# DearCaat/RRT-MIL

Measured on AMD Instinct MI355X. Metric: slides/sec RRTEncoder fwd, N=9000 D=512 region_num=8, higher is better.
Workload: dtype f32

## Files before the change

include/rrt_hip.h:

```cpp
#ifndef RRT_HIP_H
#define RRT_HIP_H
#include <stddef.h>
#include <stdint.h>

#ifdef __cplusplus
extern "C" {
#endif

#define RRT_ABI_VERSION 28
#define RRT_MAX_RMSA_LAYERS 8
#define RRT_MAX_CRMSA_K 8

enum {
  RRT_OK = 0,
  RRT_E_INVALID = -1,
  RRT_E_UNSUPPORTED = -2,
  RRT_E_WORKSPACE = -3,
  RRT_E_HANDOVER = -4
};

enum { RRT_COMPUTE_F32 = 0, RRT_COMPUTE_BF16 = 1, RRT_COMPUTE_F16 = 2, RRT_COMPUTE_F32X3 = 3 };
enum { RRT_POS_NONE = 0, RRT_POS_PEG = 1, RRT_POS_PPEG = 2 };
enum { RRT_EPEG_ATTN = 0, RRT_EPEG_VALUE_BF = 1, RRT_EPEG_VALUE_AF = 2 };

enum { RRT_ACT_NONE = 0, RRT_ACT_RELU = 1, RRT_ACT_GELU = 2, RRT_ACT_TANH = 3, RRT_ACT_SIGMOID = 4 };

typedef struct rrt_grid {
  int64_t L;
  int32_t H;
  int32_t s;
  int32_t regions_side;
  int64_t add;
} rrt_grid;

typedef struct rrt_encoder_desc {
  int32_t dim;
  int32_t n_heads;
  int32_t n_rmsa_layers;
  int32_t region_num;
  int32_t region_size;
  int32_t min_region_num;
  float   min_region_ratio;
  int32_t epeg;
  int32_t epeg_k;
  int32_t cr_msa;
  int32_t crmsa_k;
  int32_t crmsa_heads;
  int32_t crmsa_mlp;
  int32_t all_shortcut;
  int32_t compute;
  int32_t ffn;
  int32_t ffn_act;
  int32_t ffn_hidden;
  int32_t pos;
  int32_t pos_pos;
  int32_t peg_k;
  int32_t peg_1d;
  int32_t epeg_2d;
  int32_t epeg_type;
  int32_t weights16_valid;
  int32_t solo;
} rrt_encoder_desc;

typedef struct rrt_attn_weights {
  const float *norm_w, *norm_b;
  const float *qkv_w, *qkv_b;
  const float *proj_w, *proj_b;
  const float *pe_w, *pe_b;
  const float *norm2_w, *norm2_b;
  const float *fc1_w, *fc1_b;
  const float *fc2_w, *fc2_b;
} rrt_attn_weights;

typedef struct rrt_encoder_weights {
  rrt_attn_weights rmsa[RRT_MAX_RMSA_LAYERS];
  rrt_attn_weights crmsa;
  const float *phi;
  const float *phi0_w, *phi2_w;
  const float *norm_w, *norm_b;
  const float *pos_w[3], *pos_b[3];
  uint64_t version;
} rrt_encoder_weights;

int         rrt_abi_version(void);
const char *rrt_strerror(int code);

int rrt_region_grid(int64_t L, int32_t region_num, int32_t region_size,
                    int32_t min_region_num, float min_region_ratio, rrt_grid *out);

int rrt_encoder_workspace_size(const rrt_encoder_desc *desc, int64_t n_tokens, size_t *bytes);

#define RRT_PLAN_FUSED      1
#define RRT_PLAN_FUSED_PROJ 2
#define RRT_PLAN_FUSED16    4
#define RRT_PLAN_FUSED_X3   8
#define RRT_PLAN_CRMSA_PARTS 16
#define RRT_PLAN_ATTN_HD    32
int rrt_encoder_plan(const rrt_encoder_desc *desc, int64_t n_tokens, int32_t *flags);

int rrt_encoder_forward_f32(const rrt_encoder_desc *desc, const rrt_encoder_weights *w,
                            const float *x, float *y, int64_t n_tokens,
                            void *workspace, size_t workspace_bytes, void *stream);

enum {
  RRT_EV_START = 0,
  RRT_EV_LN_PARTITION,
  RRT_EV_QKV,
  RRT_EV_ATTN,
  RRT_EV_PROJ,
  RRT_EV_CR_COMBINE,
  RRT_EV_CR_INNER,
  RRT_EV_END,
  RRT_EV_COUNT
};
int rrt_encoder_forward_events_f32(const rrt_encoder_desc *desc, const rrt_encoder_weights *w,
                                   const float *x, float *y, int64_t n_tokens,
                                   void *workspace, size_t workspace_bytes, void *stream,
                                   void **events);

typedef struct rrt_phase_gate rrt_phase_gate;
int rrt_phase_gate_create(rrt_phase_gate **out);
int rrt_phase_gate_destroy(rrt_phase_gate *gate);
int rrt_encoder_forward_gated_f32(const rrt_encoder_desc *desc, const rrt_encoder_weights *w,
                                  const float *x, float *y, int64_t n_tokens,
                                  void *workspace, size_t workspace_bytes, void *stream,
                                  rrt_phase_gate *gate, void **events);

int rrt_encoder_batch_workspace_size(const rrt_encoder_desc *desc, int32_t batch, int64_t n_tokens, size_t *bytes);
int rrt_encoder_forward_batch_f32(const rrt_encoder_desc *desc, const rrt_encoder_weights *w,
                                  const float *x, float *y, int32_t batch, int64_t n_tokens,
                                  void *workspace, size_t workspace_bytes, void *stream);


int rrt_ln_partition_f32(const float *x, const float *gamma, const float *beta, float *u,
                         int64_t L, int32_t dim, const rrt_grid *g, void *stream);

int rrt_linear_f32(const float *A, const float *B, const float *bias, float *C,
                   int64_t M, int32_t N, int32_t K, int32_t q_cols, float q_scale,
                   int32_t compute , void *stream);

int rrt_linear_unpartition_residual_f32(const float *A, const float *B, const float *bias,
                                        const float *resid, float *out, int32_t N, int32_t K,
                                        const rrt_grid *g, int32_t compute, void *stream);

int rrt_region_attention_f32(const float *qkv, const float *pe_w, float *o,
                             int32_t n_regions, int32_t P, int32_t dim, int32_t heads,
                             int32_t epeg_k, void *stream);

int rrt_region_attention_hd_supported(int32_t P, int32_t dim, int32_t heads, int32_t epeg_k);
int rrt_region_attention_hd_f32(const float *qkv, const float *pe_w, float *o,
                                int32_t n_regions, int32_t P, int32_t dim, int32_t heads,
                                int32_t epeg_k, void *stream);

int rrt_rmsa_fused_f32(const float *u, const float *qkv_w, const float *qkv_b, const float *pe_w,
                       float *o, int32_t n_regions, int32_t P, int32_t dim, int32_t heads,
                       int32_t epeg_k, int32_t compute, void *stream);

int rrt_rmsa_fused_proj_f32(const float *u, const float *qkv_w, const float *qkv_b, const float *pe_w,
                            const float *proj_w, const float *proj_b, const float *resid, float *out,
                            float *o_scratch, int32_t *counters, int32_t dim, int32_t heads, int32_t epeg_k,
                            const rrt_grid *g, void *stream);
int rrt_rmsa_fused_proj_stats_f32(const float *u, const float *qkv_w, const float *qkv_b, const float *pe_w,
                                  const float *proj_w, const float *proj_b, const float *resid, float *out,
                                  float *o_scratch, int32_t *counters, const float *ln2_gamma, const float *phi,
                                  int32_t crmsa_k, float *part, int32_t dim, int32_t heads, int32_t epeg_k,
                                  const rrt_grid *g, void *stream);
int rrt_crmsa_combine_parts_f32(const float *x1, const float *part, const float *gamma, const float *beta,
                                const float *phi, float *wdisp, float *rep, int64_t n_tokens, int32_t dim, int32_t k,
                                const rrt_grid *g8, void *stream);
int rrt_device_error(int32_t clear);
int rrt_debug_rmsa_fused_proj_f32(const float *u, const float *qkv_w, const float *qkv_b, const float *pe_w,
                                  const float *proj_w, const float *proj_b, const float *resid, float *out,
                                  float *o_scratch, int32_t *counters, int32_t dim, int32_t heads, int32_t epeg_k,
                                  const rrt_grid *g, int32_t lag, int32_t spin_limit, int32_t wait_extra, void *stream);

int rrt_cast16(const float *src, uint16_t *dst, int64_t n, int32_t compute, void *stream);
int rrt_ln_partition16(const float *x, const float *gamma, const float *beta, uint16_t *u, int64_t L,
                       int32_t dim, const rrt_grid *g, int32_t compute, void *stream);
int rrt_linear16_f32(const uint16_t *A, const uint16_t *B, const float *bias, const float *resid, float *C,
                     int64_t M, int32_t N, int32_t K, const rrt_grid *g, int32_t compute, void *stream);
int rrt_rmsa_fused16(const uint16_t *u, const uint16_t *qkv_w, const float *qkv_b, const float *pe_w,
                     uint16_t *o, int32_t n_regions, int32_t P, int32_t dim, int32_t heads, int32_t epeg_k,
                     int32_t compute, void *stream);
int rrt_rmsa_pair16_proj(const uint16_t *u, const uint16_t *qkv_w, const float *qkv_b, const float *pe_w,
                         const uint16_t *proj_w, const float *proj_b, const float *resid, float *out, uint16_t *o,
                         int32_t *cnt, int32_t dim, int32_t heads, int32_t epeg_k, const rrt_grid *g, int32_t compute,
                         void *stream);

int rrt_cast_split(const float *src, void *dst, int64_t n, void *stream);
int rrt_ln_partition_split(const float *x, const float *gamma, const float *beta, void *u, int64_t L,
                           int32_t dim, const rrt_grid *g, void *stream);
int rrt_linear_split_f32(const void *A, const void *B, const float *bias, const float *resid, float *C,
                         int64_t M, int32_t N, int32_t K, const rrt_grid *g, void *stream);
int rrt_rmsa_fused_x3(const void *u, const void *qkv_w, const float *qkv_b, const float *pe_w, void *o,
                      int32_t n_regions, int32_t P, int32_t dim, int32_t heads, int32_t epeg_k, void *stream);

int rrt_crmsa_logits_f32(const float *x1, const float *gamma, const float *beta, const float *phi,
                         float *mean_rstd, float *logits, int64_t L, int32_t dim, int32_t k,
                         const rrt_grid *g8, void *stream);
int rrt_crmsa_combine_f32(const float *x1, const float *gamma, const float *beta,
                          const float *mean_rstd, const float *logits, float *wdisp, float *rep,
                          int64_t L, int32_t dim, int32_t k, const rrt_grid *g8, void *stream);
int rrt_crmsa_region_f32(const float *x1, const float *gamma, const float *beta, const float *phi,
                         float *mean_rstd, float *logits, float *wdisp, float *rep,
                         int64_t L, int32_t dim, int32_t k, const rrt_grid *g8, void *stream);
int rrt_crmsa_region4_f32(const float *x1, const float *gamma, const float *beta, const float *phi,
                          float *mean_rstd, float *logits, float *wdisp, float *rep,
                          int64_t L, int32_t dim, int32_t k, const rrt_grid *g8,
                          void *scratch, size_t scratch_bytes, void *stream);
int rrt_crmsa_stream4_f32(const float *x1, const float *gamma, const float *beta, const float *phi,
                          float *mean_rstd, float *logits, float *wdisp, float *rep,
                          int64_t L, int32_t dim, int32_t k, const rrt_grid *g8,
                          void *scratch, size_t scratch_bytes, void *stream);
int rrt_crmsa_dispatch_ln_f32(const float *x1, const float *x0, const float *wdisp,
                              const float *rep2, const float *gamma,
                              const float *beta, float *y, int64_t L, int32_t dim, int32_t k,
                              const rrt_grid *g8, void *stream);
int rrt_crmsa_mlp_logits_f32(const float *hid, const float *w2, float *logits, int64_t rows,
                             int32_t hdim, int32_t k, void *stream);
int rrt_layernorm_f32(const float *x1, const float *x0, const float *gamma, const float *beta,
                      float *y, int64_t L, int32_t dim, void *stream);

typedef struct rrt_mil_desc {
  rrt_encoder_desc enc;
  int32_t input_dim;
  int32_t emb_act;
  int32_t n_classes;
  int32_t pool_hidden;
  int32_t pool_act;
  int32_t pool_gated;
  int32_t input16;
} rrt_mil_desc;

typedef struct rrt_mil_weights {
  rrt_encoder_weights enc;
  const float *emb_w, *emb_b;
  const float *pool_a_w, *pool_a_b;
  const float *pool_b_w, *pool_b_b;
  const float *pool_c_w, *pool_c_b;
  const float *pred_w, *pred_b;
} rrt_mil_weights;

int rrt_attn_pool_workspace_size(int64_t n_tokens, int32_t dim, int32_t hidden, size_t *bytes);
int rrt_attn_pool_f32(const float *y, const float *hid_a, const float *hid_b, const float *c_w, const float *c_b,
                      float *pooled, float *attn, float *a_raw, int64_t n_tokens, int32_t dim, int32_t hidden,
                      void *workspace, size_t workspace_bytes, void *stream);
int rrt_attn_pool_backward_f32(const float *y, const float *hid_a, const float *hid_b, const float *c_w,
                               const float *attn, const float *pooled, const float *d_pooled,
                               const float *d_attn, const float *d_raw, const float *c_ext, float *dy,
                               float *dhid_a, float *dhid_b, float *dwcb, int64_t n_tokens, int32_t dim,
                               int32_t hidden, void *workspace, size_t workspace_bytes, void *stream);

int rrt_mil_workspace_size(const rrt_mil_desc *desc, int64_t n_tokens, size_t *bytes);

int rrt_mil_forward_f32(const rrt_mil_desc *desc, const rrt_mil_weights *w, const float *x,
                        float *logits, float *attn, int32_t no_norm, float *feat, int64_t n_tokens,
                        void *workspace, size_t workspace_bytes, void *stream);

int rrt_pool_workspace_size(int64_t n_tokens, int32_t dim, int32_t hidden, int32_t gated, size_t *bytes);
int rrt_pool_predict_f32(const float *y, const float *a_w, const float *a_b, const float *b_w,
                         const float *b_b, const float *c_w, const float *c_b, const float *pred_w,
                         const float *pred_b, float *pooled, float *logits, float *attn, int32_t no_norm,
                         int64_t n_tokens, int32_t dim, int32_t hidden, int32_t act, int32_t n_classes,
                         int32_t compute, void *workspace, size_t workspace_bytes, void *stream);

int rrt_linear_act_f32(const float *A, const float *B, const float *bias, float *C, int64_t M, int32_t N,
                       int32_t K, int32_t act, int32_t compute, void *stream);

typedef struct rrt_executor rrt_executor;
typedef struct rrt_bag {
  const float *x;
  float *y;
  int64_t n_tokens;
} rrt_bag;
int rrt_executor_create(const rrt_encoder_desc *desc, int32_t n_streams, int64_t max_tokens,
                        rrt_executor **out);
int rrt_executor_create_on_streams(const rrt_encoder_desc *desc, int32_t n_streams, void *const *streams,
                                   int64_t max_tokens, rrt_executor **out);
int rrt_executor_forward(rrt_executor *ex, const rrt_encoder_weights *w, const rrt_bag *bags,
                         int32_t n_bags, void *stream);
int rrt_executor_destroy(rrt_executor *ex);

int rrt_region_attention_backward_workspace_size(int32_t n_regions, int32_t P, int32_t dim, int32_t heads,
                                                 int32_t epeg_k, size_t *bytes);
int rrt_region_attention_backward_f32(const float *qkv, const float *pe_w, const float *o, const float *d_o,
                                      float *d_qkv, float *d_pe_w, int32_t n_regions, int32_t P, int32_t dim,
                                      int32_t heads, int32_t epeg_k, void *workspace, size_t workspace_bytes,
                                      void *stream);
int rrt_layernorm_backward_f32(const float *dy, const float *x, const float *gamma, const float *add,
                               float *dx, float *dgamma_dbeta, int64_t L, int32_t dim, const rrt_grid *g,
                               void *workspace, size_t workspace_bytes, void *stream);
int rrt_reduce_partials_f32(const float *part, float *out, float *out_tr, int32_t S, int64_t n, int64_t split,
                            int32_t tr_dim, int32_t tr_k, int32_t deferred, int32_t copies, void *stream);
int rrt_linear_backward_workspace_size(int64_t M, int32_t N, int32_t K, size_t *bytes);
int rrt_linear_backward_f32(const float *dY, const float *X, const float *W, float *dX, float *dW,
                            float *db, int64_t M, int32_t N, int32_t K, int32_t compute,
                            void *workspace, size_t workspace_bytes, void *stream);

typedef struct rrt_attn_grads {
  float *norm;
  float *qkv_w, *qkv_b;
  float *proj_w, *proj_b;
  float *pe_w;
  float *pe_b;
  float *norm2;
  float *fc1_w, *fc1_b;
  float *fc2_w, *fc2_b;
} rrt_attn_grads;
typedef struct rrt_encoder_grads {
  rrt_attn_grads rmsa[RRT_MAX_RMSA_LAYERS];
  rrt_attn_grads crmsa;
  float *phi;
  float *phi0_w, *phi2_w;
  float *norm;
  float *pos_w[3], *pos_b[3];
} rrt_encoder_grads;

int rrt_encoder_train_sizes(const rrt_encoder_desc *desc, int64_t n_tokens, size_t *stash_bytes,
                            size_t *backward_workspace_bytes);
int rrt_encoder_forward_train_f32(const rrt_encoder_desc *desc, const rrt_encoder_weights *w, const float *x,
                                  float *y, int64_t n_tokens, void *stash, size_t stash_bytes,
                                  float drop_p, uint64_t drop_seed, const float *branch_scale, void *stream);
// ... 11 lines not shown
```

rrt-mil_amd/_lib.py:

```python
import ctypes as C
import os

HERE = os.path.dirname(os.path.abspath(__file__))
LIB_PATH = os.path.join(HERE, "librrt_hip.so")

RRT_MAX_RMSA_LAYERS = 8
RRT_MAX_CRMSA_K = 8
ABI_VERSION = 28

_f32p = C.POINTER(C.c_float)


class Grid(C.Structure):
    _fields_ = [("L", C.c_int64), ("H", C.c_int32), ("s", C.c_int32),
                ("regions_side", C.c_int32), ("add", C.c_int64)]


class EncoderDesc(C.Structure):
    _fields_ = [("dim", C.c_int32), ("n_heads", C.c_int32), ("n_rmsa_layers", C.c_int32),
                ("region_num", C.c_int32), ("region_size", C.c_int32), ("min_region_num", C.c_int32),
                ("min_region_ratio", C.c_float), ("epeg", C.c_int32), ("epeg_k", C.c_int32),
                ("cr_msa", C.c_int32), ("crmsa_k", C.c_int32), ("crmsa_heads", C.c_int32),
                ("crmsa_mlp", C.c_int32), ("all_shortcut", C.c_int32), ("compute", C.c_int32),
                ("ffn", C.c_int32), ("ffn_act", C.c_int32), ("ffn_hidden", C.c_int32),
                ("pos", C.c_int32), ("pos_pos", C.c_int32), ("peg_k", C.c_int32), ("peg_1d", C.c_int32),
                ("epeg_2d", C.c_int32), ("epeg_type", C.c_int32), ("weights16_valid", C.c_int32),
                ("solo", C.c_int32)]


class AttnWeights(C.Structure):
    _fields_ = [(n, C.c_void_p) for n in ("norm_w", "norm_b", "qkv_w", "qkv_b", "proj_w", "proj_b",
                                          "pe_w", "pe_b", "norm2_w", "norm2_b", "fc1_w", "fc1_b",
                                          "fc2_w", "fc2_b")]


class EncoderWeights(C.Structure):
    _fields_ = [("rmsa", AttnWeights * RRT_MAX_RMSA_LAYERS), ("crmsa", AttnWeights),
                ("phi", C.c_void_p), ("phi0_w", C.c_void_p), ("phi2_w", C.c_void_p),
                ("norm_w", C.c_void_p), ("norm_b", C.c_void_p),
                ("pos_w", C.c_void_p * 3), ("pos_b", C.c_void_p * 3), ("version", C.c_uint64)]


class AttnGrads(C.Structure):
    _fields_ = [(n, C.c_void_p) for n in ("norm", "qkv_w", "qkv_b", "proj_w", "proj_b", "pe_w", "pe_b", "norm2",
                                          "fc1_w", "fc1_b", "fc2_w", "fc2_b")]


class EncoderGrads(C.Structure):
    _fields_ = [("rmsa", AttnGrads * RRT_MAX_RMSA_LAYERS), ("crmsa", AttnGrads), ("phi", C.c_void_p),
                ("phi0_w", C.c_void_p), ("phi2_w", C.c_void_p), ("norm", C.c_void_p),
                ("pos_w", C.c_void_p * 3), ("pos_b", C.c_void_p * 3)]


class MilDesc(C.Structure):
    _fields_ = [("enc", EncoderDesc), ("input_dim", C.c_int32), ("emb_act", C.c_int32),
                ("n_classes", C.c_int32), ("pool_hidden", C.c_int32), ("pool_act", C.c_int32),
                ("pool_gated", C.c_int32), ("input16", C.c_int32)]


class MilWeights(C.Structure):
    _fields_ = [("enc", EncoderWeights)] + [(n, C.c_void_p) for n in (
        "emb_w", "emb_b", "pool_a_w", "pool_a_b", "pool_b_w", "pool_b_b", "pool_c_w", "pool_c_b",
        "pred_w", "pred_b")]


class Bag(C.Structure):
    _fields_ = [("x", C.c_void_p), ("y", C.c_void_p), ("n_tokens", C.c_int64)]


ACT_NONE, ACT_RELU, ACT_GELU, ACT_TANH, ACT_SIGMOID = 0, 1, 2, 3, 4
ACT_BY_NAME = {"relu": ACT_RELU, "gelu": ACT_GELU, "tanh": ACT_TANH}

SIGNATURES = {
    "rrt_abi_version": (C.c_int, []),
    "rrt_strerror": (C.c_char_p, [C.c_int]),
    "rrt_region_grid": (C.c_int, [C.c_int64, C.c_int32, C.c_int32, C.c_int32, C.c_float, C.POINTER(Grid)]),
    "rrt_encoder_workspace_size": (C.c_int, [C.POINTER(EncoderDesc), C.c_int64, C.POINTER(C.c_size_t)]),
    "rrt_encoder_plan": (C.c_int, [C.POINTER(EncoderDesc), C.c_int64, C.POINTER(C.c_int32)]),
    "rrt_encoder_forward_f32": (C.c_int, [C.POINTER(EncoderDesc), C.POINTER(EncoderWeights), C.c_void_p,
                                          C.c_void_p, C.c_int64, C.c_void_p, C.c_size_t, C.c_void_p]),
    "rrt_encoder_forward_events_f32": (C.c_int, [C.POINTER(EncoderDesc), C.POINTER(EncoderWeights), C.c_void_p,
                                                 C.c_void_p, C.c_int64, C.c_void_p, C.c_size_t, C.c_void_p,
                                                 C.POINTER(C.c_void_p)]),
    "rrt_encoder_batch_workspace_size": (C.c_int, [C.POINTER(EncoderDesc), C.c_int32, C.c_int64, C.POINTER(C.c_size_t)]),
    "rrt_encoder_forward_batch_f32": (C.c_int, [C.POINTER(EncoderDesc), C.POINTER(EncoderWeights), C.c_void_p, C.c_void_p,
                                                C.c_int32, C.c_int64, C.c_void_p, C.c_size_t, C.c_void_p]),
    "rrt_phase_gate_create": (C.c_int, [C.POINTER(C.c_void_p)]),
    "rrt_phase_gate_destroy": (C.c_int, [C.c_void_p]),
    "rrt_encoder_forward_gated_f32": (C.c_int, [C.POINTER(EncoderDesc), C.POINTER(EncoderWeights), C.c_void_p,
                                                C.c_void_p, C.c_int64, C.c_void_p, C.c_size_t, C.c_void_p,
                                                C.c_void_p, C.POINTER(C.c_void_p)]),
    "rrt_ln_partition_f32": (C.c_int, [C.c_void_p, C.c_void_p, C.c_void_p, C.c_void_p, C.c_int64,
                                       C.c_int32, C.POINTER(Grid), C.c_void_p]),
    "rrt_linear_f32": (C.c_int, [C.c_void_p, C.c_void_p, C.c_void_p, C.c_void_p, C.c_int64, C.c_int32,
                                 C.c_int32, C.c_int32, C.c_float, C.c_int32, C.c_void_p]),
    "rrt_linear_unpartition_residual_f32": (C.c_int, [C.c_void_p, C.c_void_p, C.c_void_p, C.c_void_p,
                                                      C.c_void_p, C.c_int32, C.c_int32, C.POINTER(Grid),
                                                      C.c_int32, C.c_void_p]),
    "rrt_region_attention_f32": (C.c_int, [C.c_void_p, C.c_void_p, C.c_void_p, C.c_int32, C.c_int32,
                                           C.c_int32, C.c_int32, C.c_int32, C.c_void_p]),
    "rrt_region_attention_hd_supported": (C.c_int, [C.c_int32] * 4),
    "rrt_region_attention_hd_f32": (C.c_int, [C.c_void_p, C.c_void_p, C.c_void_p, C.c_int32, C.c_int32,
                                              C.c_int32, C.c_int32, C.c_int32, C.c_void_p]),
    "rrt_rmsa_fused_f32": (C.c_int, [C.c_void_p] * 5 + [C.c_int32] * 6 + [C.c_void_p]),
    "rrt_rmsa_fused_proj_f32": (C.c_int, [C.c_void_p] * 10 + [C.c_int32] * 3 + [C.c_void_p] * 2),
    "rrt_device_error": (C.c_int, [C.c_int32]),
    "rrt_rmsa_fused_proj_stats_f32": (C.c_int, [C.c_void_p] * 12 + [C.c_int32, C.c_void_p] + [C.c_int32] * 3 + [C.c_void_p] * 2),
    "rrt_crmsa_combine_parts_f32": (C.c_int, [C.c_void_p] * 7 + [C.c_int64, C.c_int32, C.c_int32, C.POINTER(Grid), C.c_void_p]),
    "rrt_debug_rmsa_fused_proj_f32": (C.c_int, [C.c_void_p] * 10 + [C.c_int32] * 3 + [C.c_void_p] + [C.c_int32] * 3 + [C.c_void_p]),
    "rrt_cast16": (C.c_int, [C.c_void_p, C.c_void_p, C.c_int64, C.c_int32, C.c_void_p]),
    "rrt_ln_partition16": (C.c_int, [C.c_void_p, C.c_void_p, C.c_void_p, C.c_void_p, C.c_int64, C.c_int32,
                                     C.POINTER(Grid), C.c_int32, C.c_void_p]),
    "rrt_linear16_f32": (C.c_int, [C.c_void_p] * 5 + [C.c_int64, C.c_int32, C.c_int32, C.POINTER(Grid), C.c_int32,
                                                      C.c_void_p]),
    "rrt_rmsa_fused16": (C.c_int, [C.c_void_p] * 5 + [C.c_int32] * 6 + [C.c_void_p]),
    "rrt_rmsa_pair16_proj": (C.c_int, [C.c_void_p] * 10 + [C.c_int32] * 3 + [C.POINTER(Grid), C.c_int32, C.c_void_p]),
    "rrt_cast_split": (C.c_int, [C.c_void_p, C.c_void_p, C.c_int64, C.c_void_p]),
    "rrt_ln_partition_split": (C.c_int, [C.c_void_p, C.c_void_p, C.c_void_p, C.c_void_p, C.c_int64, C.c_int32,
                                         C.POINTER(Grid), C.c_void_p]),
    "rrt_linear_split_f32": (C.c_int, [C.c_void_p] * 5 + [C.c_int64, C.c_int32, C.c_int32, C.POINTER(Grid), C.c_void_p]),
    "rrt_rmsa_fused_x3": (C.c_int, [C.c_void_p] * 5 + [C.c_int32] * 5 + [C.c_void_p]),
    "rrt_crmsa_logits_f32": (C.c_int, [C.c_void_p] * 6 + [C.c_int64, C.c_int32, C.c_int32,
                                                         C.POINTER(Grid), C.c_void_p]),
    "rrt_crmsa_combine_f32": (C.c_int, [C.c_void_p] * 7 + [C.c_int64, C.c_int32, C.c_int32,
                                                          C.POINTER(Grid), C.c_void_p]),
    "rrt_crmsa_region_f32": (C.c_int, [C.c_void_p] * 8 + [C.c_int64, C.c_int32, C.c_int32, C.POINTER(Grid), C.c_void_p]),
    "rrt_crmsa_region4_f32": (C.c_int, [C.c_void_p] * 8 + [C.c_int64, C.c_int32, C.c_int32, C.POINTER(Grid), C.c_void_p,
                                                         C.c_size_t, C.c_void_p]),
    "rrt_crmsa_stream4_f32": (C.c_int, [C.c_void_p] * 8 + [C.c_int64, C.c_int32, C.c_int32, C.POINTER(Grid), C.c_void_p,
                                                         C.c_size_t, C.c_void_p]),
    "rrt_crmsa_dispatch_ln_f32": (C.c_int, [C.c_void_p] * 7 + [C.c_int64, C.c_int32, C.c_int32,
                                                              C.POINTER(Grid), C.c_void_p]),
    "rrt_crmsa_mlp_logits_f32": (C.c_int, [C.c_void_p] * 3 + [C.c_int64, C.c_int32, C.c_int32, C.c_void_p]),
    "rrt_layernorm_f32": (C.c_int, [C.c_void_p] * 5 + [C.c_int64, C.c_int32, C.c_void_p]),
    "rrt_mil_workspace_size": (C.c_int, [C.POINTER(MilDesc), C.c_int64, C.POINTER(C.c_size_t)]),
    "rrt_mil_forward_f32": (C.c_int, [C.POINTER(MilDesc), C.POINTER(MilWeights), C.c_void_p, C.c_void_p,
                                      C.c_void_p, C.c_int32, C.c_void_p, C.c_int64, C.c_void_p, C.c_size_t,
                                      C.c_void_p]),
    "rrt_pool_workspace_size": (C.c_int, [C.c_int64, C.c_int32, C.c_int32, C.c_int32, C.POINTER(C.c_size_t)]),
    "rrt_pool_predict_f32": (C.c_int, [C.c_void_p] * 12 + [C.c_int32, C.c_int64] + [C.c_int32] * 5 +
                             [C.c_void_p, C.c_size_t, C.c_void_p]),
    "rrt_attn_pool_workspace_size": (C.c_int, [C.c_int64, C.c_int32, C.c_int32, C.POINTER(C.c_size_t)]),
    "rrt_attn_pool_f32": (C.c_int, [C.c_void_p] * 8 + [C.c_int64, C.c_int32, C.c_int32, C.c_void_p, C.c_size_t, C.c_void_p]),
    "rrt_attn_pool_backward_f32": (C.c_int, [C.c_void_p] * 14 + [C.c_int64, C.c_int32, C.c_int32, C.c_void_p, C.c_size_t,
                                                                 C.c_void_p]),
    "rrt_executor_create": (C.c_int, [C.POINTER(EncoderDesc), C.c_int32, C.c_int64, C.POINTER(C.c_void_p)]),
    "rrt_executor_create_on_streams": (C.c_int, [C.POINTER(EncoderDesc), C.c_int32, C.POINTER(C.c_void_p), C.c_int64,
                                                 C.POINTER(C.c_void_p)]),
    "rrt_executor_forward": (C.c_int, [C.c_void_p, C.POINTER(EncoderWeights), C.POINTER(Bag), C.c_int32,
                                       C.c_void_p]),
    "rrt_executor_destroy": (C.c_int, [C.c_void_p]),
    "rrt_region_attention_backward_workspace_size": (C.c_int, [C.c_int32] * 5 + [C.POINTER(C.c_size_t)]),
    "rrt_region_attention_backward_f32": (C.c_int, [C.c_void_p] * 6 + [C.c_int32] * 5 + [C.c_void_p, C.c_size_t,
                                                                                       C.c_void_p]),
    "rrt_layernorm_backward_f32": (C.c_int, [C.c_void_p] * 6 + [C.c_int64, C.c_int32, C.POINTER(Grid), C.c_void_p,
                                                                C.c_size_t, C.c_void_p]),
    "rrt_reduce_partials_f32": (C.c_int, [C.c_void_p] * 3 + [C.c_int32, C.c_int64, C.c_int64] + [C.c_int32] * 4 + [C.c_void_p]),
    "rrt_linear_backward_workspace_size": (C.c_int, [C.c_int64, C.c_int32, C.c_int32, C.POINTER(C.c_size_t)]),
    "rrt_linear_backward_f32": (C.c_int, [C.c_void_p] * 6 + [C.c_int64, C.c_int32, C.c_int32, C.c_int32,
                                                             C.c_void_p, C.c_size_t, C.c_void_p]),
    "rrt_encoder_train_sizes": (C.c_int, [C.POINTER(EncoderDesc), C.c_int64, C.POINTER(C.c_size_t),
                                          C.POINTER(C.c_size_t)]),
    "rrt_encoder_forward_train_f32": (C.c_int, [C.POINTER(EncoderDesc), C.POINTER(EncoderWeights), C.c_void_p,
                                                C.c_void_p, C.c_int64, C.c_void_p, C.c_size_t, C.c_float,
                                                C.c_uint64, C.POINTER(C.c_float), C.c_void_p]),
    "rrt_encoder_backward_f32": (C.c_int, [C.POINTER(EncoderDesc), C.POINTER(EncoderWeights), C.c_void_p, C.c_void_p,
                                           C.c_void_p, C.c_size_t, C.POINTER(EncoderGrads), C.c_void_p, C.c_int64,
                                           C.c_void_p, C.c_size_t, C.c_float, C.c_uint64, C.POINTER(C.c_float),
                                           C.c_void_p]),
    "rrt_linear_act_f32": (C.c_int, [C.c_void_p] * 4 + [C.c_int64, C.c_int32, C.c_int32, C.c_int32, C.c_int32,
                                                        C.c_void_p]),
}

COMPUTE_F32, COMPUTE_BF16, COMPUTE_F16, COMPUTE_F32X3 = 0, 1, 2, 3
POS_NONE, POS_PEG, POS_PPEG = 0, 1, 2
EPEG_ATTN, EPEG_VALUE_BF, EPEG_VALUE_AF = 0, 1, 2

PLAN_FUSED, PLAN_FUSED_PROJ, PLAN_FUSED16, PLAN_FUSED_X3, PLAN_CRMSA_PARTS, PLAN_ATTN_HD = 1, 2, 4, 8, 16, 32
EV_START, EV_LN_PARTITION, EV_QKV, EV_ATTN, EV_PROJ, EV_CR_COMBINE, EV_CR_INNER, EV_END, EV_COUNT = range(9)

_lib = None


class RRTHipError(RuntimeError):
    pass


def load(path=None):
    global _lib
    if _lib is not None and path is None:
        return _lib
    p = path or os.environ.get("RRT_HIP_LIB") or LIB_PATH
    if not os.path.exists(p):
        raise RRTHipError(
            f"{p} is missing: the HIP extension is the only compute path. Build it with "
            "`python rrt-mil_amd/build.py` (needs /opt/rocm/bin/hipcc).")
    lib = C.CDLL(p)
    for name, (res, args) in SIGNATURES.items():
        fn = getattr(lib, name)
        fn.restype = res
        fn.argtypes = args
    if lib.rrt_abi_version() != ABI_VERSION:
        raise RRTHipError(f"librrt_hip.so ABI {lib.rrt_abi_version()} != binding {ABI_VERSION}; rebuild")
    if path is None:
        _lib = lib
    return lib


E_HANDOVER = -4


def device_error(clear=False):
    return int(load().rrt_device_error(1 if clear else 0))


def check(rc, what=""):
    if rc != 0:
        msg = load().rrt_strerror(rc).decode()
        if rc == -2:
            raise NotImplementedError(f"rrt_hip {what}: {msg}")
        if rc == E_HANDOVER:
            msg += (" -- sticky until cleared: torch.cuda.synchronize(), discard the outputs of the forwards in flight, "
                    "rrt_mil_amd.device_error(clear=True), run them again")
        raise RRTHipError(f"rrt_hip {what} failed ({rc}): {msg}")


def region_grid(L, region_num=8, region_size=0, min_region_num=0, min_region_ratio=0.0):
    g = Grid()
    check(load().rrt_region_grid(L, region_num, region_size, min_region_num, min_region_ratio, C.byref(g)),
          "rrt_region_grid")
    return g
```

rrt-mil_amd/csrc/api.hip:

```cpp
#include <math.h>
#include <stdio.h>
#include <string.h>

#include "internal.h"

namespace {

thread_local char g_detail[256] = "";

int unsupported(const char* why) {
  snprintf(g_detail, sizeof(g_detail), "%s", why);
  return RRT_E_UNSUPPORTED;
}

int64_t ceil_sqrt(int64_t n) {
  int64_t r = (int64_t)floor(sqrt((double)n));
  while (r * r > n) --r;
  while ((r + 1) * (r + 1) <= n) ++r;
  return r * r == n ? r : r + 1;
}

inline size_t align_up(size_t v, size_t a) { return (v + a - 1) / a * a; }

struct Workspace {
  float *uo, *qkv, *xa, *xb, *mean_rstd, *logits, *wdisp, *rep, *rep_qkv, *rep_o, *rep2, *v8, *hid;
  float *ffn_ln, *ffn_hid, *xp;
  float* pe_out;
  float* smap;
  uint16_t* w16;
  uint16_t* wcr16;
  uint16_t *rep16, *repo16;
  float* cr_part;
  int* cr_cnt;
  int* proj_cnt;
  float* cr_pstat;
  size_t bytes;
};

Workspace carve(const rrt_encoder_desc& d, int64_t N, const rrt_grid& g, const rrt_grid& g8, char* base) {
  Workspace w{};
  size_t off = 0;
  auto take = [&](size_t nfloat) {
    float* p = base ? (float*)(base + off) : nullptr;
    off = align_up(off + nfloat * sizeof(float), 256);
    return p;
  };
  const size_t D = d.dim;
  const size_t Np = (size_t)g.H * g.H, Np8 = (size_t)g8.H * g8.H;
  const size_t R8 = (size_t)g8.regions_side * g8.regions_side;
  if (d.n_rmsa_layers > 0) w.w16 = (uint16_t*)take((size_t)d.n_rmsa_layers * 4 * D * D);
  if (d.cr_msa) w.wcr16 = (uint16_t*)take(2 * D * D);
  if (d.n_rmsa_layers > 0) {
    w.uo = take(Np * D);
    w.qkv = take(Np * 3 * D);
    w.xa = take((size_t)N * D);
    if (d.n_rmsa_layers > 1 || d.ffn) w.xb = take((size_t)N * D);
    w.proj_cnt = (int*)take((size_t)g.regions_side * g.regions_side);
    if (d.epeg && d.epeg_type != RRT_EPEG_ATTN) w.pe_out = take(Np * D);
    if (d.epeg && d.epeg_2d && d.epeg_type == RRT_EPEG_ATTN) {
      const size_t sm = attn_scoremap_scratch_floats(g.regions_side * g.regions_side, g.s * g.s, d.n_heads, d.epeg_k, 1);
      if (sm) w.smap = take(sm);
    }
  }
  if (d.ffn) {
    if (!w.xa) w.xa = take((size_t)N * D);
    if (!w.xb) w.xb = take((size_t)N * D);
    w.ffn_ln = take((size_t)N * D);
    w.ffn_hid = take((size_t)N * d.ffn_hidden);
  }
  if (d.cr_msa) {
    const size_t k = d.crmsa_k;
    w.mean_rstd = take((size_t)N * 2);
    w.logits = take(Np8 * k);
    w.wdisp = take(Np8 * k);
    w.rep = take(k * R8 * D);
    w.rep_qkv = take(k * R8 * 3 * D);
    w.rep_o = take(k * R8 * D);
    w.rep2 = take(k * R8 * D);
    w.rep16 = (uint16_t*)take(k * R8 * D / 2);
    w.repo16 = (uint16_t*)take(k * R8 * D / 2);
    if (d.n_rmsa_layers > 0) {
      w.cr_part = take(crmsa_region4_scratch_floats(to_dev(g8), d.crmsa_k));
      w.cr_cnt = (int*)take(64);
      if (D % 64 == 0) w.cr_pstat = take(crmsa_parts_floats(N, (int)D, d.crmsa_k));
    }
    if (d.crmsa_mlp) {
      w.v8 = take(Np8 * D);
      w.hid = take(Np8 * (D / 4));
    }
  }
  if (d.pos) w.xp = take((size_t)N * D);
  w.bytes = off ? off : 256;
  return w;
}

int check_desc(const rrt_encoder_desc* d, int64_t N) {
  if (!d || N <= 0) return RRT_E_INVALID;
  if (d->dim <= 0 || d->dim % 32 != 0) return unsupported("dim must be a positive multiple of 32");
  if (d->dim > 2048) return unsupported("dim > 2048");
  if (d->n_rmsa_layers < 0 || d->n_rmsa_layers > RRT_MAX_RMSA_LAYERS) return unsupported("n_layers-1 out of range");
  if (d->n_rmsa_layers > 0) {
    if (d->n_heads <= 0 || d->dim % d->n_heads != 0) return unsupported("n_heads must divide dim");
    if (d->epeg && (d->epeg_k <= 0 || d->epeg_k % 2 == 0)) return unsupported("epeg_k must be odd");
    if (d->epeg_type < RRT_EPEG_ATTN || d->epeg_type > RRT_EPEG_VALUE_AF) return unsupported("epeg_type must be attn / value_bf / value_af");
    if (d->epeg && (d->epeg_2d || d->epeg_type != RRT_EPEG_ATTN) && d->epeg_k > 63) return unsupported("epeg ablations: epeg_k <= 63");
    if (d->region_size <= 0 && d->region_num <= 0) return unsupported("region_num must be positive");
  }
  if (d->cr_msa) {
    if (d->crmsa_k <= 0 || d->crmsa_k > RRT_MAX_CRMSA_K) return unsupported("crmsa_k must be in [1,8]");
    if (d->crmsa_heads <= 0 || d->dim % d->crmsa_heads != 0) return unsupported("crmsa_heads must divide dim");
  }
  if (d->ffn) {
    if (d->ffn_hidden <= 0 || d->ffn_hidden % 32 != 0)
      return unsupported("ffn: hidden width int(dim * mlp_ratio) must be a positive multiple of 32");
    if (d->ffn_act != RRT_ACT_GELU && d->ffn_act != RRT_ACT_RELU) return unsupported("ffn_act must be gelu or relu");
  }
  if (d->pos) {
    if (d->pos != RRT_POS_PEG && d->pos != RRT_POS_PPEG) return unsupported("pos must be none / peg / ppeg");
    if (d->peg_k <= 0 || d->peg_k % 2 == 0 || d->peg_k > 11) return unsupported("peg_k must be odd and <= 11");
    if (d->pos_pos != -1 && d->pos_pos != 0) return unsupported("pos_pos must be -1 or 0");
  }
  if (N > (int64_t)4000000) return unsupported("bag larger than 4e6 tokens");
  if (d->compute < 0 || d->compute > RRT_COMPUTE_F32X3) return unsupported("compute must be RRT_COMPUTE_F32/BF16/F16/F32X3");
  return RRT_OK;
}

hipError_t inner_attention(const float* u, int n_regions, int P, const rrt_attn_weights& w, int dim,
                           int heads, int epeg_k, float* qkv, float* o, int prec, bool solo, hipStream_t st) {
  const int M = n_regions * P;
  LinearEpilogue ep{};
  ep.prec = prec;
  ep.solo = solo;
  ep.bias = w.qkv_b;
  ep.q_cols = dim;
  ep.q_scale = 1.0f / sqrtf((float)(dim / heads));
  hipError_t e = launch_linear(u, w.qkv_w, qkv, M, 3 * dim, dim, ep, st);
  if (e != hipSuccess) return e;
  return launch_region_attention(qkv, epeg_k > 0 ? w.pe_w : nullptr, o, n_regions, P, dim, heads,
                                 epeg_k, st);
}

}

GridDev to_dev(const rrt_grid& g) {
  GridDev d;
  d.L = (int)g.L;
  d.H = g.H;
  d.s = g.s;
  d.rs = g.regions_side;
  d.P = g.s * g.s;
  d.Np = g.H * g.H;
  d.inv_H = 1.0f / (float)d.H;
  d.inv_s = 1.0f / (float)d.s;
  d.inv_rs = 1.0f / (float)d.rs;
  d.inv_P = 1.0f / (float)d.P;
  d.Rt = d.rs * d.rs;
  return d;
}

extern "C" {

int rrt_abi_version(void) { return RRT_ABI_VERSION; }

const char* rrt_strerror(int code) {
  switch (code) {
    case RRT_OK: return "ok";
    case RRT_E_INVALID: return "invalid argument (null pointer or non-positive size)";
    case RRT_E_UNSUPPORTED: return g_detail[0] ? g_detail : "unsupported configuration";
    case RRT_E_WORKSPACE: return "workspace too small (see rrt_encoder_workspace_size)";
    case RRT_E_HANDOVER: return "an earlier merged R-MSA launch gave up its in-launch hand-over wait; outputs in flight are invalid "
                                "(synchronise, then rrt_device_error(1) to clear)";
    default: return code > 0 ? hipGetErrorString((hipError_t)code) : "unknown error";
  }
}

int rrt_region_grid(int64_t L, int32_t region_num, int32_t region_size, int32_t min_region_num,
                    float min_region_ratio, rrt_grid* out) {
  if (!out || L <= 0) return RRT_E_INVALID;
  if (region_size <= 0 && region_num <= 0) return RRT_E_INVALID;
  int64_t H = ceil_sqrt(L), s;
  if (region_size > 0) {
    H += ((-H) % region_size + region_size) % region_size;
    s = region_size;
  } else {
    H += ((-H) % region_num + region_num) % region_num;
    s = H / region_num;
  }
  int64_t add = H * H - L;
  if ((double)add > (double)L / ((double)min_region_ratio + 1e-8) || L < min_region_num) {
    H = ceil_sqrt(L);
    H += H % 2;
    add = H * H - L;
    s = H;
  }
  if (H > 46340) return RRT_E_INVALID;
  out->L = L;
  out->H = (int32_t)H;
  out->s = (int32_t)s;
  out->regions_side = (int32_t)(H / s);
  out->add = add;
  return RRT_OK;
}

int rrt_encoder_workspace_size(const rrt_encoder_desc* desc, int64_t n_tokens, size_t* bytes) {
  if (!bytes) return RRT_E_INVALID;
  int rc = check_desc(desc, n_tokens);
  if (rc) return rc;
  rrt_grid g{}, g8{};
  if (desc->n_rmsa_layers > 0) {
    rc = rrt_region_grid(n_tokens, desc->region_num, desc->region_size, desc->min_region_num,
                         desc->min_region_ratio, &g);
    if (rc) return rc;
  }
  rc = rrt_region_grid(n_tokens, 8, 0, 0, 0.f, &g8);
  if (rc) return rc;
  *bytes = carve(*desc, n_tokens, g, g8, nullptr).bytes;
  return RRT_OK;
}

int rrt_encoder_plan(const rrt_encoder_desc* desc, int64_t n_tokens, int32_t* flags) {
  if (!flags) return RRT_E_INVALID;
  *flags = 0;
  int rc = check_desc(desc, n_tokens);
  if (rc) return rc;
  if (desc->n_rmsa_layers <= 0) return RRT_OK;
  rrt_grid g{};
  rc = rrt_region_grid(n_tokens, desc->region_num, desc->region_size, desc->min_region_num, desc->min_region_ratio, &g);
  if (rc) return rc;
  const GridDev gd = to_dev(g);
  const int D = desc->dim, ek = desc->epeg ? desc->epeg_k : 0;
  const bool want_x3 = desc->compute == RRT_COMPUTE_F32X3;
  const int compute = want_x3 ? RRT_COMPUTE_F32 : desc->compute;
  const bool epeg_variant = desc->epeg && (desc->epeg_2d || desc->epeg_type != RRT_EPEG_ATTN);
  if (epeg_variant) return RRT_OK;
  const bool rows_ok = rmsa_fused_supported_rows(gd.Np, D);
  if (compute != RRT_COMPUTE_F32 && D % 64 == 0 && rmsa_fused16_supported(gd.P, D, desc->n_heads, ek) && rows_ok) {
    *flags = RRT_PLAN_FUSED16;
    return RRT_OK;
  }
  if (want_x3 && D % 256 == 0 && rmsa_fused_x3_supported(gd.P, D, desc->n_heads, ek) && rows_ok) {
    *flags = RRT_PLAN_FUSED_X3;
    return RRT_OK;
  }
  if (rmsa_fused_supported(gd.P, D, desc->n_heads, ek) && rows_ok) {
    *flags = RRT_PLAN_FUSED;
    if (compute == RRT_COMPUTE_F32 && rmsa_fused_proj_supported(gd.rs * gd.rs, gd.P, D, desc->n_heads, ek, compute)) {
      *flags |= RRT_PLAN_FUSED_PROJ;
      rrt_grid g8{};
      if (rrt_region_grid(n_tokens, 8, 0, 0, 0.f, &g8) == RRT_OK && desc->solo != 0 && desc->crmsa_k <= 4 && desc->cr_msa &&
          !desc->crmsa_mlp && !desc->ffn && D % 64 == 0 &&
          crmsa_combine_parts_supported(D, desc->crmsa_k, to_dev(g8)))
        *flags |= RRT_PLAN_CRMSA_PARTS;
    }
    return RRT_OK;
  }
  if (region_attention_hd_supported(gd.P, D, desc->n_heads, ek)) *flags = RRT_PLAN_ATTN_HD;
  return RRT_OK;
}

struct rrt_phase_gate {
  hipEvent_t done;
  bool armed;
};

static int ffn_apply(const rrt_encoder_desc* desc, const rrt_attn_weights& lw, const float* xi, float* xo,
                     const Workspace& ws, int64_t N, hipStream_t st) {
  if (!lw.norm2_w || !lw.norm2_b || !lw.fc1_w || !lw.fc1_b || !lw.fc2_w || !lw.fc2_b) return RRT_E_INVALID;
  const int D = desc->dim;
  GridDev gid{};
  const int Hs = (int)ceil_sqrt(N);
  gid.L = (int)N;
  gid.H = gid.s = Hs;
  gid.rs = 1;
  gid.P = gid.Np = Hs * Hs;
  gid.inv_H = gid.inv_s = 1.0f / (float)Hs;
  gid.inv_rs = 1.0f;
  gid.inv_P = 1.0f / (float)gid.P;
  gid.Rt = 1;
  hipError_t fe = launch_layernorm(xi, nullptr, lw.norm2_w, lw.norm2_b, ws.ffn_ln, (int)N, D, st);
  if (fe != hipSuccess) return (int)fe;
  LinearEpilogue e1{};
  e1.prec = desc->compute;
  e1.bias = lw.fc1_b;
  e1.act = desc->ffn_act;
  fe = launch_linear(ws.ffn_ln, lw.fc1_w, ws.ffn_hid, (int)N, desc->ffn_hidden, D, e1, st);
  if (fe != hipSuccess) return (int)fe;
  LinearEpilogue e2{};
  e2.prec = desc->compute;
  e2.bias = lw.fc2_b;
  e2.resid = xi;
  e2.g = gid;
  return (int)launch_linear(ws.ffn_hid, lw.fc2_w, xo, (int)N, D, desc->ffn_hidden, e2, st);
}

#ifndef RRT_STREAM4_MIN_P
#define RRT_STREAM4_MIN_P 145
#endif
static bool crmsa_parts_wanted(const rrt_encoder_desc& d, const Workspace& ws, const GridDev& g8, bool stops_before_crmsa) {
  return d.solo != 0 && d.cr_msa && !d.crmsa_mlp && !d.ffn && d.crmsa_k <= 4 && !stops_before_crmsa && ws.cr_pstat != nullptr &&
         crmsa_combine_parts_supported(d.dim, d.crmsa_k, g8);
}

static int encoder_forward(const rrt_encoder_desc* desc_in, const rrt_encoder_weights* w, const float* x,
                           float* y, int64_t n_tokens, void* workspace, size_t workspace_bytes,
                           void* stream, void** events, rrt_phase_gate* gate = nullptr, float* rmsa_out = nullptr,
                           uint16_t* y16 = nullptr, bool* y16_done = nullptr) {
  if (y16_done) *y16_done = false;
  if (!desc_in || !w || !x || !y || x == y) return RRT_E_INVALID;
  int rc = check_desc(desc_in, n_tokens);
  if (rc) return rc;
  if (handover_err_peek(false)) return RRT_E_HANDOVER;
  rrt_encoder_desc dloc = *desc_in;
  const bool want_x3 = dloc.compute == RRT_COMPUTE_F32X3;
  if (want_x3) dloc.compute = RRT_COMPUTE_F32;
  const rrt_encoder_desc* const desc = &dloc;
  hipStream_t st = (hipStream_t)stream;
  const int D = desc->dim;
  const int64_t N = n_tokens;
  rrt_grid g{}, g8{};
  if (desc->n_rmsa_layers > 0) {
    rc = rrt_region_grid(N, desc->region_num, desc->region_size, desc->min_region_num,
                         desc->min_region_ratio, &g);
    if (rc) return rc;
  }
  rc = rrt_region_grid(N, 8, 0, 0, 0.f, &g8);
  if (rc) return rc;
  Workspace ws = carve(*desc, N, g, g8, nullptr);
  if (!workspace || workspace_bytes < ws.bytes) return RRT_E_WORKSPACE;
  ws = carve(*desc, N, g, g8, (char*)workspace);

  hipError_t e = hipSuccess;
#define RRT_TRY(call)            \
  do {                           \
    e = (call);                  \
    if (e != hipSuccess) return (int)e; \
  } while (0)
#define RRT_MARK(i)                                                          \
  do {                                                                       \
    if (events && events[i]) RRT_TRY(hipEventRecord((hipEvent_t)events[i], st)); \
  } while (0)
  RRT_MARK(RRT_EV_START);

  auto ffn_block = [&](const rrt_attn_weights& lw, const float* xi, float* xo) -> int {
    return ffn_apply(desc, lw, xi, xo, ws, N, st);
  };

  const float* xin = x;
  auto pos_embed = [&]() -> int {
    if (!w->pos_w[0] || (desc->pos == RRT_POS_PPEG && (!w->pos_w[1] || !w->pos_w[2]))) return RRT_E_INVALID;
    hipError_t pe = launch_peg(xin, w->pos_w, w->pos_b, ws.xp, (int)N, D, desc->peg_k, desc->peg_1d,
                               desc->pos == RRT_POS_PPEG, st);
    if (pe != hipSuccess) return (int)pe;
    xin = ws.xp;
    return RRT_OK;
  };
  if (desc->pos && desc->pos_pos == -1) {
    rc = pos_embed();
    if (rc) return rc;
  }
  const bool epeg_variant = desc->epeg && (desc->epeg_2d || desc->epeg_type != RRT_EPEG_ATTN);
  bool lowp16 = false;
  const bool inner16 = desc->cr_msa && desc->compute != RRT_COMPUTE_F32 && D % 64 == 0 &&
                       rmsa_fused16_supported(64, D, desc->crmsa_heads, 0);
  if (desc->compute != RRT_COMPUTE_F32 && D % 64 == 0) {
    Cast16Jobs jobs{};
    if (desc->n_rmsa_layers > 0 && !epeg_variant) {
      const GridDev gd = to_dev(g);
      lowp16 = rmsa_fused16_supported(gd.P, D, desc->n_heads, desc->epeg ? desc->epeg_k : 0) &&
               rmsa_fused_supported_rows(gd.Np, D);
      for (int li = 0; li < desc->n_rmsa_layers; ++li) {
        const rrt_attn_weights& lw = w->rmsa[li];
        if (!lw.qkv_w || !lw.proj_w) return RRT_E_INVALID;
        uint16_t* base = ws.w16 + (size_t)li * 4 * D * D;
        jobs.src[jobs.count] = lw.qkv_w; jobs.dst[jobs.count] = base; jobs.n4[jobs.count++] = (size_t)3 * D * D / 4;
        jobs.src[jobs.count] = lw.proj_w; jobs.dst[jobs.count] = base + (size_t)3 * D * D; jobs.n4[jobs.count++] = (size_t)D * D / 4;
      }
    }
    if (inner16) {
      if (!w->crmsa.qkv_w || !w->crmsa.proj_w) return RRT_E_INVALID;
      jobs.src[jobs.count] = w->crmsa.qkv_w; jobs.dst[jobs.count] = ws.wcr16; jobs.n4[jobs.count++] = (size_t)3 * D * D / 4;
      jobs.src[jobs.count] = w->crmsa.proj_w; jobs.dst[jobs.count] = ws.wcr16 + (size_t)3 * D * D; jobs.n4[jobs.count++] = (size_t)D * D / 4;
    }
    if (jobs.count && !desc->weights16_valid) RRT_TRY(launch_cast16(jobs, desc->compute, st));
  }
  bool x3 = false;
  if (want_x3 && desc->n_rmsa_layers > 0 && !epeg_variant) {
    const GridDev gd = to_dev(g);
    x3 = D % 256 == 0 && rmsa_fused_x3_supported(gd.P, D, desc->n_heads, desc->epeg ? desc->epeg_k : 0) &&
         rmsa_fused_supported_rows(gd.Np, D);
    Cast16Jobs jobs{};
    for (int li = 0; li < desc->n_rmsa_layers; ++li) {
      const rrt_attn_weights& lw = w->rmsa[li];
      if (!lw.qkv_w || !lw.proj_w) return RRT_E_INVALID;
      uint16_t* base = ws.w16 + (size_t)li * 8 * D * D;
      jobs.src[jobs.count] = lw.qkv_w; jobs.dst[jobs.count] = base; jobs.n4[jobs.count++] = (size_t)3 * D * D / 4;
      jobs.src[jobs.count] = lw.proj_w; jobs.dst[jobs.count] = base + (size_t)6 * D * D; jobs.n4[jobs.count++] = (size_t)D * D / 4;
    }
    if (!desc->weights16_valid) RRT_TRY(launch_cast_split(jobs, st));
  }
  bool parts_done = false;
  for (int li = 0; li < desc->n_rmsa_layers; ++li) {
    if (li == 1 && desc->pos && desc->pos_pos == 0) {
      rc = pos_embed();
      if (rc) return rc;
    }
    const rrt_attn_weights& lw = w->rmsa[li];
    if (!lw.norm_w || !lw.norm_b || !lw.qkv_w || !lw.proj_w || !lw.proj_b) return RRT_E_INVALID;
    if (desc->epeg && !lw.pe_w) return RRT_E_INVALID;
    const GridDev gd = to_dev(g);
    const bool to_out = rmsa_out != nullptr && li == desc->n_rmsa_layers - 1;
    float* xout = desc->ffn ? ws.xa : (to_out ? rmsa_out : ((li & 1) ? ws.xb : ws.xa));
    float* const fout = to_out ? rmsa_out : ws.xb;
    const int ek = desc->epeg ? desc->epeg_k : 0;
    if (lowp16) {
      uint16_t* u16 = (uint16_t*)ws.uo;
      uint16_t* o16 = (uint16_t*)ws.qkv;
      const uint16_t* wq16 = ws.w16 + (size_t)li * 4 * D * D;
      static const bool want_merged16 = rrt_tune_env("RRT_PAIR16_PROJ") != nullptr;
      const bool merged16 = want_merged16 && ws.proj_cnt != nullptr &&
                            rmsa_pair16_proj_supported(gd.rs * gd.rs, gd.P, D, desc->n_heads, ek);
      RRT_TRY(launch_ln_partition16(xin, lw.norm_w, lw.norm_b, u16, D, gd, desc->compute, st, merged16 ? ws.proj_cnt : nullptr,
                                    merged16 ? gd.rs * gd.rs / 2 : 0));
      rrt_phase_gate* const gt16 = (gate && gd.P > 112) ? gate : nullptr;
      if (gt16 && gt16->armed) RRT_TRY(hipStreamWaitEvent(st, gt16->done, 0));
      if (li == 0) RRT_MARK(RRT_EV_LN_PARTITION);
      if (merged16) {
        PairProj pj{};
        pj.Wp = wq16 + (size_t)3 * D * D;
        pj.bias = lw.proj_b;
        pj.resid = xin;
        pj.out = xout;
        pj.cnt = ws.proj_cnt;
        pj.zero64 = ws.cr_cnt;
        pj.g = gd;
        RRT_TRY(launch_rmsa_pair16_proj(u16, wq16, lw.qkv_b, desc->epeg ? lw.pe_w : nullptr, o16, gd.rs * gd.rs, gd.P, D,
                                        desc->n_heads, ek, desc->compute, pj, st));
        if (gt16) { RRT_TRY(hipEventRecord(gt16->done, st)); gt16->armed = true; }
        if (li == 0) { RRT_MARK(RRT_EV_QKV); RRT_MARK(RRT_EV_ATTN); RRT_MARK(RRT_EV_PROJ); }
        xin = xout;
        if (desc->ffn) {
          rc = ffn_block(lw, xout, fout);
          if (rc) return rc;
          xin = fout;
        }
        continue;
      }
      RRT_TRY(launch_rmsa_fused16(u16, wq16, lw.qkv_b, desc->epeg ? lw.pe_w : nullptr, o16, gd.rs * gd.rs, gd.P, D,
                                  desc->n_heads, ek, desc->compute, st));
      if (gt16) { RRT_TRY(hipEventRecord(gt16->done, st)); gt16->armed = true; }
      if (li == 0) { RRT_MARK(RRT_EV_QKV); RRT_MARK(RRT_EV_ATTN); }
      LinearEpilogue ep{};
      ep.prec = desc->compute;
      ep.bias = lw.proj_b;
      ep.resid = xin;
      ep.g = gd;
      ep.zero64 = ws.cr_cnt;
      ep.solo = desc->solo != 0;
      RRT_TRY(launch_linear16(o16, wq16 + (size_t)3 * D * D, xout, gd.Np, D, D, ep, st));
      if (li == 0) RRT_MARK(RRT_EV_PROJ);
      xin = xout;
      if (desc->ffn) {
        rc = ffn_block(lw, xout, fout);
        if (rc) return rc;
        xin = fout;
      }
      continue;
    }
    if (x3) {
      const uint16_t* wq = ws.w16 + (size_t)li * 8 * D * D;
      RRT_TRY(launch_ln_partition_split(xin, lw.norm_w, lw.norm_b, ws.uo, D, gd, st));
      rrt_phase_gate* const gt3 = (gate && gd.P > 112) ? gate : nullptr;
      if (gt3 && gt3->armed) RRT_TRY(hipStreamWaitEvent(st, gt3->done, 0));
      if (li == 0) RRT_MARK(RRT_EV_LN_PARTITION);
      RRT_TRY(launch_rmsa_fused_x3(ws.uo, wq, lw.qkv_b, desc->epeg ? lw.pe_w : nullptr, ws.qkv, gd.rs * gd.rs, gd.P, D,
                                   desc->n_heads, ek, st));
      if (gt3) { RRT_TRY(hipEventRecord(gt3->done, st)); gt3->armed = true; }
      if (li == 0) { RRT_MARK(RRT_EV_QKV); RRT_MARK(RRT_EV_ATTN); }
      LinearEpilogue ep{};
      ep.bias = lw.proj_b;
      ep.resid = xin;
      ep.g = gd;
      ep.zero64 = ws.cr_cnt;
      RRT_TRY(launch_linear_split(ws.qkv, wq + (size_t)6 * D * D, xout, gd.Np, D, D, ep, st));
      if (li == 0) RRT_MARK(RRT_EV_PROJ);
      xin = xout;
      if (desc->ffn) {
        rc = ffn_block(lw, xout, fout);
        if (rc) return rc;
        xin = fout;
      }
      continue;
    }
    const bool merged = !epeg_variant && desc->compute == RRT_COMPUTE_F32 && ws.proj_cnt != nullptr &&
                        rmsa_fused_supported_rows(gd.Np, D) &&
                        rmsa_fused_proj_supported(gd.rs * gd.rs, gd.P, D, desc->n_heads, ek, desc->compute);
    const bool parts = merged && li == desc->n_rmsa_layers - 1 && !epeg_variant &&
                       rmsa_fused_supported(gd.P, D, desc->n_heads, ek) &&
                       crmsa_parts_wanted(*desc, ws, to_dev(g8), rmsa_out != nullptr);
    if (parts && (!w->crmsa.norm_w || !w->crmsa.norm_b || !w->phi)) return RRT_E_INVALID;
    RRT_TRY(launch_ln_partition(xin, lw.norm_w, lw.norm_b, ws.uo, D, gd, st, merged ? ws.proj_cnt : nullptr,
                                merged ? gd.rs * gd.rs : 0));
    if (epeg_variant) {
      if (!lw.pe_w) return RRT_E_INVALID;
      const int nreg = gd.rs * gd.rs;
      {
        LinearEpilogue ep{};
        ep.prec = desc->compute;
        ep.bias = lw.qkv_b;
        ep.q_cols = D;
        ep.q_scale = 1.0f / sqrtf((float)(D / desc->n_heads));
        RRT_TRY(launch_linear(ws.uo, lw.qkv_w, ws.qkv, gd.Np, 3 * D, D, ep, st));
      }
      if (desc->epeg_type == RRT_EPEG_ATTN) {
        RRT_TRY(launch_attn_scoremap(ws.qkv, lw.pe_w, ws.uo, ws.smap, nreg, gd.P, D, desc->n_heads, desc->epeg_k, st));
      } else {
        RRT_TRY(launch_value_pe(ws.qkv, lw.pe_w, lw.pe_b, ws.pe_out, nreg, gd.P, gd.s, D, desc->n_heads, desc->epeg_k,
                                desc->epeg_2d, st));
        if (desc->epeg_type == RRT_EPEG_VALUE_BF)
          RRT_TRY(launch_add_cols(ws.qkv + 2 * D, ws.pe_out, (size_t)gd.Np, D, 3 * D, st));
        RRT_TRY(launch_region_attention(ws.qkv, nullptr, ws.uo, nreg, gd.P, D, desc->n_heads, 0, st));
        if (desc->epeg_type == RRT_EPEG_VALUE_AF)
          RRT_TRY(launch_add_cols(ws.uo, ws.pe_out, (size_t)gd.Np, D, D, st));
      }
      LinearEpilogue ep{};
      ep.prec = desc->compute;
      ep.bias = lw.proj_b;
      ep.resid = xin;
      ep.g = gd;
      ep.zero64 = ws.cr_cnt;
      RRT_TRY(launch_linear(ws.uo, lw.proj_w, xout, gd.Np, D, D, ep, st));
      xin = xout;
      if (desc->ffn) {
        rc = ffn_block(lw, xout, fout);
        if (rc) return rc;
        xin = fout;
      }
      continue;
    }
    const bool fused = rmsa_fused_supported(gd.P, D, desc->n_heads, ek) && rmsa_fused_supported_rows(gd.Np, D);
    rrt_phase_gate* const gt = (gate && fused && gd.P > 112) ? gate : nullptr;
    if (gt && gt->armed) RRT_TRY(hipStreamWaitEvent(st, gt->done, 0));
    if (li == 0) RRT_MARK(RRT_EV_LN_PARTITION);
    if (fused && merged) {
      FusedProj pj{};
      pj.Wp = lw.proj_w;
      pj.bias = lw.proj_b;
      pj.resid = xin;
      pj.out = xout;
      pj.cnt = ws.proj_cnt;
      pj.zero64 = ws.cr_cnt;
      pj.g = gd;
      if (parts) {
        pj.part = ws.cr_pstat;
        pj.ln_g = w->crmsa.norm_w;
        pj.phi = w->phi;
        pj.k = desc->crmsa_k;
        parts_done = true;
      }
      RRT_TRY(launch_rmsa_fused(ws.uo, lw.qkv_w, lw.qkv_b, desc->epeg ? lw.pe_w : nullptr, ws.qkv,
                                gd.rs * gd.rs, gd.P, D, desc->n_heads, ek, desc->compute, st, nullptr, &pj));
      if (gt) { RRT_TRY(hipEventRecord(gt->done, st)); gt->armed = true; }
      if (li == 0) { RRT_MARK(RRT_EV_QKV); RRT_MARK(RRT_EV_ATTN); RRT_MARK(RRT_EV_PROJ); }
      xin = xout;
      if (desc->ffn) {
        rc = ffn_block(lw, xout, fout);
        if (rc) return rc;
        xin = fout;
      }
      continue;
    }
    if (fused) {
      RRT_TRY(launch_rmsa_fused(ws.uo, lw.qkv_w, lw.qkv_b, desc->epeg ? lw.pe_w : nullptr, ws.qkv,
                                gd.rs * gd.rs, gd.P, D, desc->n_heads, ek, desc->compute, st));
      static const bool gate_proj = rrt_tune_env("RRT_GATE_PROJ") != nullptr;
      if (gt && !gate_proj) { RRT_TRY(hipEventRecord(gt->done, st)); gt->armed = true; }
      if (li == 0) { RRT_MARK(RRT_EV_QKV); RRT_MARK(RRT_EV_ATTN); }
      LinearEpilogue ep{};
      ep.prec = desc->compute;
      ep.bias = lw.proj_b;
      ep.resid = xin;
      ep.g = gd;
      ep.zero64 = ws.cr_cnt;
      RRT_TRY(launch_linear(ws.qkv, lw.proj_w, xout, gd.Np, D, D, ep, st));
      if (gt && gate_proj) { RRT_TRY(hipEventRecord(gt->done, st)); gt->armed = true; }
      if (li == 0) RRT_MARK(RRT_EV_PROJ);
      xin = xout;
      if (desc->ffn) {
        rc = ffn_block(lw, xout, fout);
        if (rc) return rc;
        xin = fout;
      }
      continue;
    }
    {
      LinearEpilogue ep{};
      ep.prec = desc->compute;
      ep.bias = lw.qkv_b;
      ep.q_cols = D;
      ep.q_scale = 1.0f / sqrtf((float)(D / desc->n_heads));
      RRT_TRY(launch_linear(ws.uo, lw.qkv_w, ws.qkv, gd.Np, 3 * D, D, ep, st));
    }
    if (li == 0) RRT_MARK(RRT_EV_QKV);
    RRT_TRY(launch_region_attention(ws.qkv, desc->epeg ? lw.pe_w : nullptr, ws.uo, gd.rs * gd.rs, gd.P, D,
                                    desc->n_heads, desc->epeg ? desc->epeg_k : 0, st));
    if (li == 0) RRT_MARK(RRT_EV_ATTN);
    LinearEpilogue ep{};
    ep.prec = desc->compute;
    ep.bias = lw.proj_b;
    ep.resid = xin;
    ep.g = gd;
    ep.zero64 = ws.cr_cnt;
    RRT_TRY(launch_linear(ws.uo, lw.proj_w, xout, gd.Np, D, D, ep, st));
    if (li == 0) RRT_MARK(RRT_EV_PROJ);
    xin = xout;
    if (desc->ffn) {
      rc = ffn_block(lw, xout, fout);
      if (rc) return rc;
      xin = fout;
    }
  }
  if (rmsa_out != nullptr) {
    if (xin != rmsa_out) RRT_TRY(hipMemcpyAsync(rmsa_out, xin, (size_t)N * D * sizeof(float), hipMemcpyDeviceToDevice, st));
    return RRT_OK;
  }
  const float* x0 = desc->all_shortcut ? x : nullptr;
  if (!w->norm_w || !w->norm_b) return RRT_E_INVALID;
  if (!desc->cr_msa) {
    RRT_TRY(launch_layernorm(xin, x0, w->norm_w, w->norm_b, y, (int)N, D, st));
    RRT_MARK(RRT_EV_END);
    return RRT_OK;
  }
  const rrt_attn_weights& cw = w->crmsa;
  if (!cw.norm_w || !cw.norm_b || !cw.qkv_w || !cw.proj_w || !cw.proj_b) return RRT_E_INVALID;
  if (desc->crmsa_mlp ? (!w->phi0_w || !w->phi2_w) : !w->phi) return RRT_E_INVALID;
  const GridDev gd8 = to_dev(g8);
  const int k = desc->crmsa_k, R8 = gd8.rs * gd8.rs;
  bool rep16_done = false;
  static const bool no_region_inflight = rrt_tune_env("RRT_NO_REGION_INFLIGHT") != nullptr;
  static const bool region_lowp = rrt_tune_env("RRT_REGION_INFLIGHT_LOWP") != nullptr;
  const bool region_inflight = !no_region_inflight && !desc->solo && !desc->crmsa_mlp && !parts_done && !x3 &&
                               (desc->compute == RRT_COMPUTE_F32 || region_lowp) && crmsa_region_supported(D, k, gd8);
  if (desc->crmsa_mlp) {
    RRT_TRY(launch_ln_partition(xin, cw.norm_w, cw.norm_b, ws.v8, D, gd8, st));
    LinearEpilogue ep{};
    ep.prec = desc->compute;
    RRT_TRY(launch_linear(ws.v8, w->phi0_w, ws.hid, gd8.Np, D / 4, D, ep, st));
    RRT_TRY(launch_crmsa_mlp_logits(ws.hid, w->phi2_w, ws.logits, gd8.Np, D / 4, k, st));
    RRT_TRY(launch_crmsa_combine(ws.v8, nullptr, nullptr, nullptr, ws.logits, ws.wdisp, ws.rep, inner16 ? ws.rep16 : nullptr,
                                 desc->compute, D, k, gd8, st));
    rep16_done = inner16;
  } else if (parts_done) {
    RRT_TRY(launch_crmsa_combine_parts(xin, ws.cr_pstat, cw.norm_w, cw.norm_b, w->phi, ws.wdisp, ws.rep,
                                       inner16 ? ws.rep16 : nullptr, desc->compute, D, k, gd8, st));
    rep16_done = inner16;
  } else if (region_inflight) {
    RRT_TRY(launch_crmsa_region(xin, cw.norm_w, cw.norm_b, w->phi, nullptr, nullptr, ws.wdisp, ws.rep, k, gd8, st,
                                inner16 ? ws.rep16 : nullptr, desc->compute));
    rep16_done = inner16;
  } else if (ws.cr_cnt && desc->n_rmsa_layers > 0 && crmsa_region4_supported(D, k, gd8) && gd8.P < RRT_STREAM4_MIN_P) {
    RRT_TRY(launch_crmsa_region4(xin, cw.norm_w, cw.norm_b, w->phi, nullptr, ws.logits, ws.wdisp, ws.rep,
                                 inner16 ? ws.rep16 : nullptr, desc->compute, ws.cr_part, ws.cr_cnt, k, gd8, st));
    rep16_done = inner16;
  } else if (crmsa_region_enabled() && crmsa_region_supported(D, k, gd8)) {
    RRT_TRY(launch_crmsa_region(xin, cw.norm_w, cw.norm_b, w->phi, nullptr, nullptr, ws.wdisp, ws.rep, k, gd8, st));
  } else if (ws.cr_cnt && desc->n_rmsa_layers > 0 && gd8.P >= RRT_STREAM4_MIN_P && crmsa_stream4_supported(D, k, gd8)) {
    RRT_TRY(launch_crmsa_stream4(xin, cw.norm_w, cw.norm_b, w->phi, nullptr, ws.logits, ws.wdisp, ws.rep,
                                 inner16 ? ws.rep16 : nullptr, desc->compute, ws.cr_part, ws.cr_cnt, k, gd8, st));
    rep16_done = inner16;
  } else {
    RRT_TRY(launch_crmsa_logits(xin, cw.norm_w, cw.norm_b, w->phi, ws.mean_rstd, ws.logits, D, k, gd8, st));
    RRT_TRY(launch_crmsa_combine(xin, cw.norm_w, cw.norm_b, ws.mean_rstd, ws.logits, ws.wdisp, ws.rep,
                                 inner16 ? ws.rep16 : nullptr, desc->compute, D, k, gd8, st));
    rep16_done = inner16;
  }
  RRT_MARK(RRT_EV_CR_COMBINE);
  if (inner16) {
    if (!rep16_done) {
      Cast16Jobs cj{};
      cj.src[0] = ws.rep; cj.dst[0] = ws.rep16; cj.n4[0] = (size_t)k * R8 * D / 4; cj.count = 1;
      RRT_TRY(launch_cast16(cj, desc->compute, st));
    }
    RRT_TRY(launch_rmsa_fused16(ws.rep16, ws.wcr16, cw.qkv_b, nullptr, ws.repo16, k, R8, D, desc->crmsa_heads, 0,
                                desc->compute, st));
    LinearEpilogue ep{};
    ep.prec = desc->compute;
    ep.bias = cw.proj_b;
    RRT_TRY(launch_linear16(ws.repo16, ws.wcr16 + (size_t)3 * D * D, ws.rep2, k * R8, D, D, ep, st));
  } else {
    static const bool inner_solo = rrt_tune_env("RRT_INNER_SOLO") != nullptr;
    RRT_TRY(inner_attention(ws.rep, k, R8, cw, D, desc->crmsa_heads, 0, ws.rep_qkv, ws.rep_o, desc->compute, desc->solo != 0 || inner_solo, st));
    LinearEpilogue ep{};
    ep.prec = desc->compute;
    ep.bias = cw.proj_b;
    ep.solo = desc->solo != 0 || inner_solo;
    RRT_TRY(launch_linear(ws.rep_o, cw.proj_w, ws.rep2, k * R8, D, D, ep, st));
  }
  RRT_MARK(RRT_EV_CR_INNER);
  if (desc->ffn) {
    RRT_TRY(launch_crmsa_dispatch_ln(xin, nullptr, ws.wdisp, ws.rep2, nullptr, nullptr, ws.xa, D, k, gd8, st));
    rc = ffn_block(cw, ws.xa, ws.xb);
    if (rc) return rc;
    RRT_TRY(launch_layernorm(ws.xb, x0, w->norm_w, w->norm_b, y, (int)N, D, st));
    RRT_MARK(RRT_EV_END);
    return RRT_OK;
  }
  const bool want16 = y16 != nullptr && (desc->compute == RRT_COMPUTE_BF16 || desc->compute == RRT_COMPUTE_F16) && D % 4 == 0;
  RRT_TRY(launch_crmsa_dispatch_ln(xin, x0, ws.wdisp, ws.rep2, w->norm_w, w->norm_b, y, D, k,
                                   gd8, st, want16 ? y16 : nullptr, want16 ? desc->compute : 0));
  if (want16 && y16_done) *y16_done = true;
  RRT_MARK(RRT_EV_END);
#undef RRT_TRY
#undef RRT_MARK
  return RRT_OK;
// ... 131 lines not shown
  if (!cw.norm_w || !cw.norm_b || !cw.qkv_w || !cw.proj_w || !cw.proj_b) return RRT_E_INVALID;
  if (desc->crmsa_mlp ? (!w->phi0_w || !w->phi2_w) : !w->phi) return RRT_E_INVALID;
  GridDev gd8 = to_dev(g8);
  const int k = desc->crmsa_k, R8 = gd8.rs * gd8.rs;
  gd8.Rt = R8 * (int)B;
  const size_t Np8 = (size_t)gd8.Np;
  const int prec = desc->compute == RRT_COMPUTE_F32X3 ? RRT_COMPUTE_F32 : desc->compute;
  for (int64_t b = 0; b < B; ++b) {
    const float* xb1 = bw.x1 + (size_t)b * N * D;
    float* lg = bw.logits + (size_t)b * Np8 * k;
    float* wd = bw.wdisp + (size_t)b * Np8 * k;
    float* repb = bw.rep + (size_t)b * R8 * D;
    if (desc->crmsa_mlp) {
      RRT_TRY(launch_ln_partition(xb1, cw.norm_w, cw.norm_b, bw.one.v8, D, gd8, st));
      LinearEpilogue ep{};
      ep.prec = prec;
      RRT_TRY(launch_linear(bw.one.v8, w->phi0_w, bw.one.hid, gd8.Np, D / 4, D, ep, st));
      RRT_TRY(launch_crmsa_mlp_logits(bw.one.hid, w->phi2_w, lg, gd8.Np, D / 4, k, st));
      RRT_TRY(launch_crmsa_combine(bw.one.v8, nullptr, nullptr, nullptr, lg, wd, repb, nullptr, 0, D, k, gd8, st));
    } else {
      float* mr = bw.mean_rstd + (size_t)b * N * 2;
      RRT_TRY(launch_crmsa_logits(xb1, cw.norm_w, cw.norm_b, w->phi, mr, lg, D, k, gd8, st));
      RRT_TRY(launch_crmsa_combine(xb1, cw.norm_w, cw.norm_b, mr, lg, wd, repb, nullptr, 0, D, k, gd8, st));
    }
  }
  RRT_TRY(inner_attention(bw.rep, k, R8 * (int)B, cw, D, desc->crmsa_heads, 0, bw.rep_qkv, bw.rep_o, prec, false, st));
  {
    LinearEpilogue ep{};
    ep.prec = prec;
    ep.bias = cw.proj_b;
    RRT_TRY(launch_linear(bw.rep_o, cw.proj_w, bw.rep2, k * R8 * (int)B, D, D, ep, st));
  }
  for (int64_t b = 0; b < B; ++b) {
    const float* xb1 = bw.x1 + (size_t)b * N * D;
    const float* x0 = desc->all_shortcut ? x + (size_t)b * N * D : nullptr;
    const float* wd = bw.wdisp + (size_t)b * Np8 * k;
    const float* rep2b = bw.rep2 + (size_t)b * R8 * D;
    float* yb = y + (size_t)b * N * D;
    if (desc->ffn) {
      RRT_TRY(launch_crmsa_dispatch_ln(xb1, nullptr, wd, rep2b, nullptr, nullptr, bw.one.xa, D, k, gd8, st));
      rc = ffn_apply(desc, cw, bw.one.xa, bw.one.xb, bw.one, N, st);
      if (rc) return rc;
      RRT_TRY(launch_layernorm(bw.one.xb, x0, w->norm_w, w->norm_b, yb, (int)N, D, st));
    } else {
      RRT_TRY(launch_crmsa_dispatch_ln(xb1, x0, wd, rep2b, w->norm_w, w->norm_b, yb, D, k, gd8, st));
    }
  }
#undef RRT_TRY
  return RRT_OK;
}

int rrt_ln_partition_f32(const float* x, const float* gamma, const float* beta, float* u, int64_t L,
                         int32_t dim, const rrt_grid* g, void* stream) {
  if (!x || !gamma || !beta || !u || !g || L != g->L || dim <= 0 || dim % 4) return RRT_E_INVALID;
  if (dim > 2048) return unsupported("dim > 2048");
  return (int)launch_ln_partition(x, gamma, beta, u, dim, to_dev(*g), (hipStream_t)stream);
}

int rrt_linear_f32(const float* A, const float* B, const float* bias, float* C, int64_t M, int32_t N,
                   int32_t K, int32_t q_cols, float q_scale, int32_t compute, void* stream) {
  if (!A || !B || !C || M <= 0 || N <= 0 || K <= 0) return RRT_E_INVALID;
  if (K % 32) return unsupported("linear: K must be a multiple of 32");
  if (compute < 0 || compute > 2) return unsupported("compute must be RRT_COMPUTE_F32/BF16/F16");
  LinearEpilogue ep{};
  ep.prec = compute;
  ep.bias = bias;
  ep.q_cols = q_cols;
  ep.q_scale = q_scale;
  return (int)launch_linear(A, B, C, (int)M, N, K, ep, (hipStream_t)stream);
}

int rrt_linear_unpartition_residual_f32(const float* A, const float* B, const float* bias,
                                        const float* resid, float* out, int32_t N, int32_t K,
                                        const rrt_grid* g, int32_t compute, void* stream) {
  if (!A || !B || !resid || !out || !g || N <= 0 || K <= 0) return RRT_E_INVALID;
  if (K % 32) return unsupported("linear: K must be a multiple of 32");
  if (compute < 0 || compute > 2) return unsupported("compute must be RRT_COMPUTE_F32/BF16/F16");
  LinearEpilogue ep{};
  ep.prec = compute;
  ep.bias = bias;
  ep.resid = resid;
  ep.g = to_dev(*g);
  return (int)launch_linear(A, B, out, ep.g.Np, N, K, ep, (hipStream_t)stream);
}

int rrt_region_attention_f32(const float* qkv, const float* pe_w, float* o, int32_t n_regions, int32_t P,
                             int32_t dim, int32_t heads, int32_t epeg_k, void* stream) {
  if (!qkv || !o || n_regions <= 0 || P <= 0 || dim <= 0 || heads <= 0 || dim % heads) return RRT_E_INVALID;
  if (pe_w && epeg_k > 0 && epeg_k % 2 == 0) return unsupported("epeg_k must be odd");
  return (int)launch_region_attention(qkv, pe_w, o, n_regions, P, dim, heads, epeg_k, (hipStream_t)stream);
}

int rrt_region_attention_hd_supported(int32_t P, int32_t dim, int32_t heads, int32_t epeg_k) {
  return region_attention_hd_supported(P, dim, heads, epeg_k) ? 1 : 0;
}

int rrt_region_attention_hd_f32(const float* qkv, const float* pe_w, float* o, int32_t n_regions, int32_t P, int32_t dim,
                                int32_t heads, int32_t epeg_k, void* stream) {
  if (n_regions <= 0 || P <= 0 || dim <= 0 || heads <= 0 || dim % heads) return RRT_E_INVALID;
  const int ek = pe_w ? epeg_k : 0;
  if (!region_attention_hd_supported(P, dim, heads, ek))
    return unsupported("region_attention_hd: needs a head dim that is a multiple of 16 in [16, 256] other than 64 and "
                       "epeg_k <= 63 (use rrt_region_attention_f32)");
  if (!qkv || !o) return RRT_E_INVALID;
  if (ek > 0 && ek % 2 == 0) return unsupported("epeg_k must be odd");
  if (n_regions > 65535) return unsupported("region_attention_hd: more than 65535 regions in one call");
  return (int)launch_region_attention_hd(qkv, pe_w, o, n_regions, P, dim, heads, ek, (hipStream_t)stream);
}

int rrt_rmsa_fused_f32(const float* u, const float* qkv_w, const float* qkv_b, const float* pe_w, float* o,
                       int32_t n_regions, int32_t P, int32_t dim, int32_t heads, int32_t epeg_k,
                       int32_t compute, void* stream) {
  if (!u || !qkv_w || !o || n_regions <= 0 || P <= 0 || dim <= 0 || heads <= 0) return RRT_E_INVALID;
  if (compute < 0 || compute > 2) return unsupported("compute must be RRT_COMPUTE_F32/BF16/F16");
  const int ek = pe_w ? epeg_k : 0;
  if (!rmsa_fused_supported(P, dim, heads, ek) || !rmsa_fused_supported_rows((long)n_regions * P, dim))
    return unsupported("rmsa_fused: needs head dim 64, 48 < P <= 208, epeg_k <= 63 (use linear + region_attention)");
  return (int)launch_rmsa_fused(u, qkv_w, qkv_b, pe_w, o, n_regions, P, dim, heads, ek, compute,
                                (hipStream_t)stream);
}

int rrt_device_error(int32_t clear) { return handover_err_peek(clear != 0); }

int rrt_rmsa_fused_proj_f32(const float* u, const float* qkv_w, const float* qkv_b, const float* pe_w,
                            const float* proj_w, const float* proj_b, const float* resid, float* out, float* o_scratch,
                            int32_t* counters, int32_t dim, int32_t heads, int32_t epeg_k, const rrt_grid* g,
                            void* stream) {
  return rrt_debug_rmsa_fused_proj_f32(u, qkv_w, qkv_b, pe_w, proj_w, proj_b, resid, out, o_scratch, counters, dim, heads,
                                       epeg_k, g, 0, 0, 0, stream);
}

}
static int fused_proj_stage(const float* u, const float* qkv_w, const float* qkv_b, const float* pe_w,
                            const float* proj_w, const float* proj_b, const float* resid, float* out, float* o_scratch,
                            int32_t* counters, int32_t dim, int32_t heads, int32_t epeg_k, const rrt_grid* g,
                            int32_t lag, int32_t spin_limit, int32_t wait_extra, const float* ln2_gamma, const float* phi,
                            int32_t crmsa_k, float* part, void* stream);
extern "C" {
int rrt_debug_rmsa_fused_proj_f32(const float* u, const float* qkv_w, const float* qkv_b, const float* pe_w,
                                  const float* proj_w, const float* proj_b, const float* resid, float* out, float* o_scratch,
                                  int32_t* counters, int32_t dim, int32_t heads, int32_t epeg_k, const rrt_grid* g,
                                  int32_t lag, int32_t spin_limit, int32_t wait_extra, void* stream) {
  return fused_proj_stage(u, qkv_w, qkv_b, pe_w, proj_w, proj_b, resid, out, o_scratch, counters, dim, heads, epeg_k, g, lag,
                          spin_limit, wait_extra, nullptr, nullptr, 0, nullptr, stream);
}

int rrt_rmsa_fused_proj_stats_f32(const float* u, const float* qkv_w, const float* qkv_b, const float* pe_w,
                                  const float* proj_w, const float* proj_b, const float* resid, float* out, float* o_scratch,
                                  int32_t* counters, const float* ln2_gamma, const float* phi, int32_t crmsa_k, float* part,
                                  int32_t dim, int32_t heads, int32_t epeg_k, const rrt_grid* g, void* stream) {
  if (!ln2_gamma || !phi || !part || crmsa_k < 1 || crmsa_k > RRT_MAX_CRMSA_K) return RRT_E_INVALID;
  return fused_proj_stage(u, qkv_w, qkv_b, pe_w, proj_w, proj_b, resid, out, o_scratch, counters, dim, heads, epeg_k, g, 0, 0, 0,
                          ln2_gamma, phi, crmsa_k, part, stream);
}

int rrt_crmsa_combine_parts_f32(const float* x1, const float* part, const float* gamma, const float* beta, const float* phi,
                                float* wdisp, float* rep, int64_t n_tokens, int32_t dim, int32_t k, const rrt_grid* g8,
                                void* stream) {
  if (!x1 || !part || !gamma || !beta || !phi || !wdisp || !rep || !g8 || n_tokens <= 0 || g8->L != n_tokens) return RRT_E_INVALID;
  const GridDev gd = to_dev(*g8);
  if (!crmsa_combine_parts_supported(dim, k, gd)) return unsupported("crmsa_combine_parts: dim % 64 == 0, dim <= 512, 1 <= k <= 8");
  return (int)launch_crmsa_combine_parts(x1, part, gamma, beta, phi, wdisp, rep, nullptr, 0, dim, k, gd, (hipStream_t)stream);
}
}

static int fused_proj_stage(const float* u, const float* qkv_w, const float* qkv_b, const float* pe_w,
                            const float* proj_w, const float* proj_b, const float* resid, float* out, float* o_scratch,
                            int32_t* counters, int32_t dim, int32_t heads, int32_t epeg_k, const rrt_grid* g,
                            int32_t lag, int32_t spin_limit, int32_t wait_extra, const float* ln2_gamma, const float* phi,
                            int32_t crmsa_k, float* part, void* stream) {
  if (!u || !qkv_w || !proj_w || !resid || !out || !o_scratch || !counters || !g || dim <= 0 || heads <= 0 || out == resid ||
      lag < 0 || spin_limit < 0 || wait_extra < 0)
    return RRT_E_INVALID;
  if (handover_err_peek(false)) return RRT_E_HANDOVER;
  const GridDev gd = to_dev(*g);
  const int ek = pe_w ? epeg_k : 0, R = gd.rs * gd.rs;
  if (!rmsa_fused_proj_supported(R, gd.P, dim, heads, ek, RRT_COMPUTE_F32) || !rmsa_fused_supported_rows(gd.Np, dim))
    return unsupported("rmsa_fused_proj: needs what rmsa_fused needs (head dim 64, 64 < P <= 208, epeg_k <= 63) and at "
                       "least two rounds of (region, head) items (heads * regions >= 2 x the CU count)");
  hipError_t e = hipMemsetAsync(counters, 0, (size_t)R * sizeof(int32_t), (hipStream_t)stream);
  if (e != hipSuccess) return (int)e;
  FusedProj pj{};
  pj.Wp = proj_w;
  pj.bias = proj_b;
  pj.resid = resid;
  pj.out = out;
  pj.cnt = counters;
  pj.g = gd;
  pj.lag = lag;
  pj.spin_limit = spin_limit;
  pj.wait_for = wait_extra > 0 ? heads + wait_extra : 0;
  pj.part = part;
  pj.ln_g = ln2_gamma;
  pj.phi = phi;
  pj.k = crmsa_k;
  if (lag > 0 && (lag < 8 * heads || lag > heads * R)) return unsupported("rmsa_fused_proj: lag must be in [8 * heads, heads * regions]");
  return (int)launch_rmsa_fused(u, qkv_w, qkv_b, pe_w, o_scratch, R, gd.P, dim, heads, ek, RRT_COMPUTE_F32,
                                (hipStream_t)stream, nullptr, &pj);
}
extern "C" {

int rrt_cast16(const float* src, uint16_t* dst, int64_t n, int32_t compute, void* stream) {
  if (!src || !dst || n <= 0 || n % 4) return RRT_E_INVALID;
  if (compute != RRT_COMPUTE_BF16 && compute != RRT_COMPUTE_F16) return unsupported("cast16: compute must be BF16 or F16");
  Cast16Jobs jobs{};
  jobs.src[0] = src; jobs.dst[0] = dst; jobs.n4[0] = (size_t)n / 4; jobs.count = 1;
  return (int)launch_cast16(jobs, compute, (hipStream_t)stream);
}

int rrt_ln_partition16(const float* x, const float* gamma, const float* beta, uint16_t* u, int64_t L, int32_t dim,
                       const rrt_grid* g, int32_t compute, void* stream) {
  if (!x || !gamma || !beta || !u || !g || L != g->L || dim <= 0 || dim % 4) return RRT_E_INVALID;
  if (dim > 2048) return unsupported("dim > 2048");
  if (compute != RRT_COMPUTE_BF16 && compute != RRT_COMPUTE_F16) return unsupported("compute must be BF16 or F16");
  return (int)launch_ln_partition16(x, gamma, beta, u, dim, to_dev(*g), compute, (hipStream_t)stream);
}

int rrt_linear16_f32(const uint16_t* A, const uint16_t* B, const float* bias, const float* resid, float* C, int64_t M,
                     int32_t N, int32_t K, const rrt_grid* g, int32_t compute, void* stream) {
  if (!A || !B || !C || M <= 0 || N <= 0 || K <= 0 || (resid && !g)) return RRT_E_INVALID;
  if (K % 64) return unsupported("linear16: K must be a multiple of 64");
  if (compute != RRT_COMPUTE_BF16 && compute != RRT_COMPUTE_F16) return unsupported("compute must be BF16 or F16");
  LinearEpilogue ep{};
  ep.prec = compute;
  ep.bias = bias;
  if (resid) {
    ep.resid = resid;
    ep.g = to_dev(*g);
    if (M != ep.g.Np) return RRT_E_INVALID;
  }
  return (int)launch_linear16(A, B, C, (int)M, N, K, ep, (hipStream_t)stream);
}

int rrt_rmsa_fused16(const uint16_t* u, const uint16_t* qkv_w, const float* qkv_b, const float* pe_w, uint16_t* o,
                     int32_t n_regions, int32_t P, int32_t dim, int32_t heads, int32_t epeg_k, int32_t compute,
                     void* stream) {
  if (!u || !qkv_w || !o || n_regions <= 0 || P <= 0 || dim <= 0 || heads <= 0) return RRT_E_INVALID;
  if (compute != RRT_COMPUTE_BF16 && compute != RRT_COMPUTE_F16) return unsupported("compute must be BF16 or F16");
  const int ek = pe_w ? epeg_k : 0;
  if (!rmsa_fused16_supported(P, dim, heads, ek) || !rmsa_fused_supported_rows((long)n_regions * P, dim))
    return unsupported("rmsa_fused16: needs head dim 64, 16 < P <= 256, epeg_k <= 63");
  return (int)launch_rmsa_fused16(u, qkv_w, qkv_b, pe_w, o, n_regions, P, dim, heads, ek, compute, (hipStream_t)stream);
}

int rrt_rmsa_pair16_proj(const uint16_t* u, const uint16_t* qkv_w, const float* qkv_b, const float* pe_w, const uint16_t* proj_w,
                         const float* proj_b, const float* resid, float* out, uint16_t* o, int32_t* cnt, int32_t dim,
                         int32_t heads, int32_t epeg_k, const rrt_grid* g, int32_t compute, void* stream) {
  if (!u || !qkv_w || !proj_w || !resid || !out || !o || !cnt || !g || dim <= 0 || heads <= 0) return RRT_E_INVALID;
  if (compute != RRT_COMPUTE_BF16 && compute != RRT_COMPUTE_F16) return unsupported("compute must be BF16 or F16");
  if (handover_err_peek(false)) return RRT_E_HANDOVER;
  const GridDev gd = to_dev(*g);
  const int ek = pe_w ? epeg_k : 0, R = gd.rs * gd.rs;
  if (!rmsa_pair16_proj_supported(R, gd.P, dim, heads, ek))
    return unsupported("rmsa_pair16_proj: head dim 64, regions of 65..96 or 113..128 tokens, a multiple of 16 regions, "
                       "at least two rounds of (pair, head) items");
  hipError_t e = hipMemsetAsync(cnt, 0, (size_t)(R / 2) * sizeof(int), (hipStream_t)stream);
  if (e != hipSuccess) return (int)e;
  PairProj pj{};
  pj.Wp = proj_w;
  pj.bias = proj_b;
  pj.resid = resid;
  pj.out = out;
  pj.cnt = cnt;
  pj.g = gd;
  return (int)launch_rmsa_pair16_proj(u, qkv_w, qkv_b, pe_w, o, R, gd.P, dim, heads, ek, compute, pj, (hipStream_t)stream);
}

int rrt_cast_split(const float* src, void* dst, int64_t n, void* stream) {
  if (!src || !dst || n <= 0 || n % 32) return RRT_E_INVALID;
  Cast16Jobs jobs{};
  jobs.src[0] = src; jobs.dst[0] = (uint16_t*)dst; jobs.n4[0] = (size_t)n / 4; jobs.count = 1;
  return (int)launch_cast_split(jobs, (hipStream_t)stream);
}

int rrt_ln_partition_split(const float* x, const float* gamma, const float* beta, void* u, int64_t L, int32_t dim,
                           const rrt_grid* g, void* stream) {
  if (!x || !gamma || !beta || !u || !g || L != g->L || dim <= 0 || dim % 32) return RRT_E_INVALID;
  if (dim > 2048) return unsupported("dim > 2048");
  return (int)launch_ln_partition_split(x, gamma, beta, u, dim, to_dev(*g), (hipStream_t)stream);
}

int rrt_linear_split_f32(const void* A, const void* B, const float* bias, const float* resid, float* C, int64_t M,
                         int32_t N, int32_t K, const rrt_grid* g, void* stream) {
  if (!A || !B || !C || M <= 0 || N <= 0 || K <= 0 || (resid && !g)) return RRT_E_INVALID;
  if (K % 32) return unsupported("linear_split: K must be a multiple of 32");
  LinearEpilogue ep{};
  ep.bias = bias;
  if (resid) {
    ep.resid = resid;
    ep.g = to_dev(*g);
    if (M != ep.g.Np) return RRT_E_INVALID;
  }
  return (int)launch_linear_split(A, B, C, (int)M, N, K, ep, (hipStream_t)stream);
}

int rrt_rmsa_fused_x3(const void* u, const void* qkv_w, const float* qkv_b, const float* pe_w, void* o,
                      int32_t n_regions, int32_t P, int32_t dim, int32_t heads, int32_t epeg_k, void* stream) {
  if (!u || !qkv_w || !o || n_regions <= 0 || P <= 0 || dim <= 0 || heads <= 0) return RRT_E_INVALID;
  const int ek = pe_w ? epeg_k : 0;
  if (!rmsa_fused_x3_supported(P, dim, heads, ek) || !rmsa_fused_supported_rows((long)n_regions * P, dim))
    return unsupported("rmsa_fused_x3: needs head dim 64, 48 < P <= 144, epeg_k <= 63");
  return (int)launch_rmsa_fused_x3(u, qkv_w, qkv_b, pe_w, o, n_regions, P, dim, heads, ek, (hipStream_t)stream);
}

int rrt_crmsa_logits_f32(const float* x1, const float* gamma, const float* beta, const float* phi,
                         float* mean_rstd, float* logits, int64_t L, int32_t dim, int32_t k,
// ... 1178 lines not shown
```

rrt-mil_amd/csrc/cast16.hip:

```cpp
#include "internal.h"

namespace {

template <int PREC>
__device__ __forceinline__ uint2 pack4(float a, float b, float c, float d) {
  if constexpr (PREC == 1) {
    typedef __bf16 v4 __attribute__((ext_vector_type(4)));
    v4 r;
    r[0] = (__bf16)a; r[1] = (__bf16)b; r[2] = (__bf16)c; r[3] = (__bf16)d;
    return __builtin_bit_cast(uint2, r);
  } else {
    typedef _Float16 v4 __attribute__((ext_vector_type(4)));
    v4 r;
    r[0] = (_Float16)a; r[1] = (_Float16)b; r[2] = (_Float16)c; r[3] = (_Float16)d;
    return __builtin_bit_cast(uint2, r);
  }
}

template <int PREC>
__global__ __launch_bounds__(256) void cast16_kernel(Cast16Jobs jobs) {
  const int j = blockIdx.y;
  const float4* src = (const float4*)jobs.src[j];
  uint2* dst = (uint2*)jobs.dst[j];
  const size_t n4 = jobs.n4[j];
  const size_t stride = (size_t)gridDim.x * 256;
  for (size_t i = (size_t)blockIdx.x * 256 + threadIdx.x; i < n4; i += 4 * stride) {
    float4 v[4];
#pragma unroll
    for (int u = 0; u < 4; ++u)
      if (i + u * stride < n4) {
#ifdef RRT_NO_NT_CAST
        v[u] = src[i + u * stride];
#else
        v[u] = ld_nt((const float*)(src + i + u * stride));
#endif
      }
#pragma unroll
    for (int u = 0; u < 4; ++u)
      if (i + u * stride < n4) dst[i + u * stride] = pack4<PREC>(v[u].x, v[u].y, v[u].z, v[u].w);
  }
}

template <int NV, int PREC, bool FULL>
__global__ __launch_bounds__(256) void ln_partition16_kernel(const float* __restrict__ x,
                                                             const float* __restrict__ gamma,
                                                             const float* __restrict__ beta,
                                                             uint16_t* __restrict__ u, int dim, GridDev g,
                                                             int* __restrict__ zero, int n_zero) {
  if (zero != nullptr && blockIdx.x == 0)
    for (int i = threadIdx.x; i < n_zero; i += 256) zero[i] = 0;
  const int lane = threadIdx.x & 63;
  const int t = blockIdx.x * 4 + (threadIdx.x >> 6);
  if (t >= g.Np) return;
  uint16_t* dst = u + (size_t)token_to_slot(t, g) * dim;
  if (t >= g.L) {
#pragma unroll
    for (int v = 0; v < NV; ++v) {
      int c = (v * 64 + lane) * 4;
      if (FULL || c < dim) *(uint2*)(dst + c) = make_uint2(0u, 0u);
    }
    return;
  }
  const float* src = x + (size_t)t * dim;
  float4 r[NV];
  float sum = 0.f;
#pragma unroll
  for (int v = 0; v < NV; ++v) {
    int c = (v * 64 + lane) * 4;
    r[v] = (FULL || c < dim) ? ld_row<NT_LN1>(src + c) : make_float4(0.f, 0.f, 0.f, 0.f);
    sum += (r[v].x + r[v].y) + (r[v].z + r[v].w);
  }
  const float inv_d = 1.0f / (float)dim;
  const float mean = wave_sum(sum) * inv_d;
  float sq = 0.f;
#pragma unroll
  for (int v = 0; v < NV; ++v) {
    int c = (v * 64 + lane) * 4;
    if (FULL || c < dim) {
      float a = r[v].x - mean, b = r[v].y - mean, cc = r[v].z - mean, d = r[v].w - mean;
      sq += (a * a + b * b) + (cc * cc + d * d);
    }
  }
  const float rstd = 1.0f / sqrtf(wave_sum(sq) * inv_d + LN_EPS);
#pragma unroll
  for (int v = 0; v < NV; ++v) {
    int c = (v * 64 + lane) * 4;
    if (FULL || c < dim) {
      float4 gm = *(const float4*)(gamma + c), bt = *(const float4*)(beta + c);
      *(uint2*)(dst + c) = pack4<PREC>((r[v].x - mean) * rstd * gm.x + bt.x, (r[v].y - mean) * rstd * gm.y + bt.y,
                                       (r[v].z - mean) * rstd * gm.z + bt.z, (r[v].w - mean) * rstd * gm.w + bt.w);
    }
  }
}

__device__ __forceinline__ void split4(float a, float b, float c, float d, uint2& hi, uint2& lo) {
  typedef __bf16 v4 __attribute__((ext_vector_type(4)));
  v4 h, l;
  h[0] = (__bf16)a; h[1] = (__bf16)b; h[2] = (__bf16)c; h[3] = (__bf16)d;
  l[0] = (__bf16)(a - (float)h[0]); l[1] = (__bf16)(b - (float)h[1]);
  l[2] = (__bf16)(c - (float)h[2]); l[3] = (__bf16)(d - (float)h[3]);
  hi = __builtin_bit_cast(uint2, h);
  lo = __builtin_bit_cast(uint2, l);
}
__device__ __forceinline__ size_t split_off(size_t e) { return (e >> 5) * 128 + (e & 31) * 2; }

__global__ __launch_bounds__(256) void cast_split_kernel(Cast16Jobs jobs) {
  const int j = blockIdx.y;
  const float4* src = (const float4*)jobs.src[j];
  char* dst = (char*)jobs.dst[j];
  const size_t n4 = jobs.n4[j];
  for (size_t i = (size_t)blockIdx.x * 256 + threadIdx.x; i < n4; i += (size_t)gridDim.x * 256) {
    const float4 v = src[i];
    uint2 hi, lo;
    split4(v.x, v.y, v.z, v.w, hi, lo);
    const size_t off = split_off(i * 4);
    *(uint2*)(dst + off) = hi;
    *(uint2*)(dst + off + 64) = lo;
  }
}

template <int NV, bool FULL>
__global__ __launch_bounds__(256) void ln_partition_split_kernel(const float* __restrict__ x,
                                                                 const float* __restrict__ gamma,
                                                                 const float* __restrict__ beta,
                                                                 char* __restrict__ u, int dim, GridDev g) {
  const int lane = threadIdx.x & 63;
  const int t = blockIdx.x * 4 + (threadIdx.x >> 6);
  if (t >= g.Np) return;
  char* dst = u + (size_t)token_to_slot(t, g) * dim * 4;
  if (t >= g.L) {
#pragma unroll
    for (int v = 0; v < NV; ++v) {
      int c = (v * 64 + lane) * 4;
      if (FULL || c < dim) *(float4*)(dst + (size_t)c * 4) = make_float4(0.f, 0.f, 0.f, 0.f);
    }
    return;
  }
  const float* src = x + (size_t)t * dim;
  float4 r[NV];
  float sum = 0.f;
#pragma unroll
  for (int v = 0; v < NV; ++v) {
    int c = (v * 64 + lane) * 4;
    r[v] = (FULL || c < dim) ? ld_row<NT_LN1>(src + c) : make_float4(0.f, 0.f, 0.f, 0.f);
    sum += (r[v].x + r[v].y) + (r[v].z + r[v].w);
  }
  const float inv_d = 1.0f / (float)dim;
  const float mean = wave_sum(sum) * inv_d;
  float sq = 0.f;
#pragma unroll
  for (int v = 0; v < NV; ++v) {
    int c = (v * 64 + lane) * 4;
    if (FULL || c < dim) {
      float a = r[v].x - mean, b = r[v].y - mean, cc = r[v].z - mean, d = r[v].w - mean;
      sq += (a * a + b * b) + (cc * cc + d * d);
    }
  }
  const float rstd = 1.0f / sqrtf(wave_sum(sq) * inv_d + LN_EPS);
#pragma unroll
  for (int v = 0; v < NV; ++v) {
    int c = (v * 64 + lane) * 4;
    if (FULL || c < dim) {
      float4 gm = *(const float4*)(gamma + c), bt = *(const float4*)(beta + c);
      uint2 hi, lo;
      split4((r[v].x - mean) * rstd * gm.x + bt.x, (r[v].y - mean) * rstd * gm.y + bt.y,
             (r[v].z - mean) * rstd * gm.z + bt.z, (r[v].w - mean) * rstd * gm.w + bt.w, hi, lo);
      const size_t off = split_off((size_t)c);
      *(uint2*)(dst + off) = hi;
      *(uint2*)(dst + off + 64) = lo;
    }
  }
}

}

hipError_t launch_cast_split(const Cast16Jobs& jobs, hipStream_t st) {
  if (jobs.count <= 0) return hipSuccess;
  size_t mx = 0;
  for (int j = 0; j < jobs.count; ++j) mx = jobs.n4[j] > mx ? jobs.n4[j] : mx;
  size_t blocks = (mx + 256 * 4 - 1) / (256 * 4);
  if (blocks < 1) blocks = 1;
  if (blocks > 512) blocks = 512;
  cast_split_kernel<<<dim3((unsigned)blocks, jobs.count), 256, 0, st>>>(jobs);
  return hipGetLastError();
}

hipError_t launch_ln_partition_split(const float* x, const float* gamma, const float* beta, void* u, int dim,
                                     const GridDev& g, hipStream_t st) {
  if (dim % 32) return hipErrorInvalidValue;
  dim3 grid((g.Np + 3) / 4), block(256);
#define RRT_LNPS(NV)                                                                                          \
  do {                                                                                                      \
    if (RRT_ALLOW_FULL && dim == NV * 256) ln_partition_split_kernel<NV, true><<<grid, block, 0, st>>>(x, gamma, beta, (char*)u, dim, g);  \
    else ln_partition_split_kernel<NV, false><<<grid, block, 0, st>>>(x, gamma, beta, (char*)u, dim, g);                 \
  } while (0)
  if (dim <= 256) RRT_LNPS(1);
  else if (dim <= 512) RRT_LNPS(2);
  else if (dim <= 1024) RRT_LNPS(4);
  else RRT_LNPS(8);
#undef RRT_LNPS
  return hipGetLastError();
}

hipError_t launch_cast16(const Cast16Jobs& jobs, int prec, hipStream_t st) {
  if (jobs.count <= 0) return hipSuccess;
  if (prec != 1 && prec != 2) return hipErrorInvalidValue;
  size_t mx = 0;
  for (int j = 0; j < jobs.count; ++j) mx = jobs.n4[j] > mx ? jobs.n4[j] : mx;
  size_t blocks = (mx + 256 * 4 - 1) / (256 * 4);
  if (blocks < 1) blocks = 1;
  if (blocks > 4096) blocks = 4096;
  dim3 grid((unsigned)blocks, jobs.count);
  if (prec == 1) cast16_kernel<1><<<grid, 256, 0, st>>>(jobs);
  else cast16_kernel<2><<<grid, 256, 0, st>>>(jobs);
  return hipGetLastError();
}

hipError_t launch_ln_partition16(const float* x, const float* gamma, const float* beta, uint16_t* u, int dim,
                                 const GridDev& g, int prec, hipStream_t st, int* zero, int n_zero) {
  if (prec != 1 && prec != 2) return hipErrorInvalidValue;
  dim3 grid((g.Np + 3) / 4), block(256);
#define RRT_LNP16(NV)                                                                               \
  do {                                                                                              \
    if (RRT_ALLOW_FULL && dim == NV * 256) {                                                                          \
      if (prec == 1) ln_partition16_kernel<NV, 1, true><<<grid, block, 0, st>>>(x, gamma, beta, u, dim, g, zero, n_zero);  \
      else ln_partition16_kernel<NV, 2, true><<<grid, block, 0, st>>>(x, gamma, beta, u, dim, g, zero, n_zero);           \
    } else {                                                                                        \
      if (prec == 1) ln_partition16_kernel<NV, 1, false><<<grid, block, 0, st>>>(x, gamma, beta, u, dim, g, zero, n_zero); \
      else ln_partition16_kernel<NV, 2, false><<<grid, block, 0, st>>>(x, gamma, beta, u, dim, g, zero, n_zero);          \
    }                                                                                               \
  } while (0)
  if (dim <= 256) RRT_LNP16(1);
  else if (dim <= 512) RRT_LNP16(2);
  else if (dim <= 1024) RRT_LNP16(4);
  else RRT_LNP16(8);
#undef RRT_LNP16
  return hipGetLastError();
}
```

rrt-mil_amd/csrc/internal.h:

```cpp
#pragma once
#include <hip/hip_runtime.h>
#include "common.h"
#include "../../include/rrt_hip.h"

GridDev to_dev(const rrt_grid& g);

#ifdef RRT_TUNING
#include <stdlib.h>
inline const char* rrt_tune_env(const char* name) { return getenv(name); }
#else
inline const char* rrt_tune_env(const char*) { return nullptr; }
#endif

struct OncePerDevice {
  bool seen[64] = {};
  bool first() {
    int d = 0;
    (void)hipGetDevice(&d);
    d &= 63;
    if (seen[d]) return false;
    seen[d] = true;
    return true;
  }
};

hipError_t launch_ln_partition(const float* x, const float* gamma, const float* beta, float* u,
                               int dim, const GridDev& g, hipStream_t st, int* zero = nullptr, int n_zero = 0);

struct LinearEpilogue {
  int prec;
  const float* bias;
  int q_cols;
  float q_scale;
  int act;
  unsigned drop_thresh, drop_seed;
  float drop_scale;
  bool drop_on;
  const float* resid;
  GridDev g;
  int* zero64;
  bool solo;
};
hipError_t launch_linear(const float* A, const float* B, float* C, int M, int N, int K,
                         const LinearEpilogue& ep, hipStream_t st);

constexpr int CAST16_MAX_JOBS = 2 * RRT_MAX_RMSA_LAYERS + 2;
struct Cast16Jobs {
  const float* src[CAST16_MAX_JOBS];
  uint16_t* dst[CAST16_MAX_JOBS];
  size_t n4[CAST16_MAX_JOBS];
  int count;
};
hipError_t launch_cast16(const Cast16Jobs& jobs, int prec, hipStream_t st);
hipError_t launch_ln_partition16(const float* x, const float* gamma, const float* beta, uint16_t* u, int dim,
                                 const GridDev& g, int prec, hipStream_t st, int* zero = nullptr, int n_zero = 0);
hipError_t launch_cast_split(const Cast16Jobs& jobs, hipStream_t st);
hipError_t launch_ln_partition_split(const float* x, const float* gamma, const float* beta, void* u, int dim,
                                     const GridDev& g, hipStream_t st);
hipError_t launch_linear_split(const void* Asplit, const void* Bsplit, float* C, int M, int N, int K,
                               const LinearEpilogue& ep, hipStream_t st);
bool rmsa_pair16_supported(int n_regions, int P, int D, int heads, int epeg_k);
hipError_t launch_rmsa_pair16(const uint16_t* U, const uint16_t* W, const float* bqkv, const float* pe_w, uint16_t* O,
                              int n_regions, int P, int D, int heads, int epeg_k, int prec, hipStream_t st);
struct PairProj {
  const uint16_t* Wp;
  const float* bias;
  const float* resid;
  float* out;
  int* cnt;
  int* zero64;
  int lag;
  int n_items;
  GridDev g;
  int* err;
  int spin_limit;
  int wait_for;
};
bool rmsa_pair16_proj_supported(int n_regions, int P, int D, int heads, int epeg_k);
hipError_t launch_rmsa_pair16_proj(const uint16_t* U, const uint16_t* W, const float* bqkv, const float* pe_w, uint16_t* O,
                                   int n_regions, int P, int D, int heads, int epeg_k, int prec, const PairProj& proj,
                                   hipStream_t st);
bool rmsa_fused_x3_supported(int P, int D, int heads, int epeg_k);
hipError_t launch_rmsa_fused_x3(const void* Usplit, const void* Wsplit, const float* bqkv, const float* pe_w,
                                void* Osplit, int n_regions, int P, int D, int heads, int epeg_k, hipStream_t st);
hipError_t launch_linear16(const void* A16, const void* B16, float* C, int M, int N, int K, const LinearEpilogue& ep,
                           hipStream_t st);
bool rmsa_fused16_supported(int P, int D, int heads, int epeg_k);
hipError_t launch_rmsa_fused16(const uint16_t* U16, const uint16_t* Wqkv16, const float* bqkv, const float* pe_w,
                               uint16_t* O16, int n_regions, int P, int D, int heads, int epeg_k, int prec,
                               hipStream_t st);

hipError_t launch_region_attention(const float* qkv, const float* pe_w, float* o, int n_regions,
                                   int P, int dim, int heads, int epeg_k, hipStream_t st);
bool region_attention_hd_supported(int P, int dim, int heads, int epeg_k);
hipError_t launch_region_attention_hd(const float* qkv, const float* pe_w, float* o, int n_regions, int P, int dim,
                                      int heads, int epeg_k, hipStream_t st);

bool rmsa_fused_supported(int P, int D, int heads, int epeg_k);
bool rmsa_fused_supported_rows(long n_rows, int D);
struct FusedProj {
  const float* Wp;
  const float* bias;
  const float* resid;
  float* out;
  int* cnt;
  int* zero64;
  int lag;
  int n_items;
  GridDev g;
  int* err;
  int spin_limit;
  int wait_for;
  float* part;
  const float* ln_g;
  const float* phi;
  int k;
  int n_slabs;
};
int* handover_err_device();
int handover_err_peek(bool clear);
bool rmsa_fused_proj_supported(int n_regions, int P, int D, int heads, int epeg_k, int prec);
hipError_t launch_rmsa_fused(const float* U, const float* Wqkv, const float* bqkv, const float* pe_w,
                             float* O, int n_regions, int P, int D, int heads, int epeg_k, int prec,
                             hipStream_t st, float* stash = nullptr,
                             const FusedProj* proj = nullptr);

size_t attn_scoremap_lds(int P, int k);
size_t attn_scoremap_scratch_floats(int n_regions, int P, int heads, int k, int maps);
hipError_t launch_attn_scoremap(const float* qkv, const float* pe_w, float* o, float* smap, int n_regions, int P, int dim,
                                int heads, int k, hipStream_t st);
hipError_t launch_value_pe(const float* qkv, const float* w, const float* bias, float* pe, int n_regions, int P, int s,
                           int dim, int heads, int k, int two_d, hipStream_t st);
hipError_t launch_add_cols(float* dst, const float* src, size_t rows, int dim, int ld, hipStream_t st);
hipError_t launch_value_pe_backward(const float* dpe, const float* qkv, const float* vsub, const float* w, float* dqkv, float* dw,
                                    float* db, int n_regions, int P, int s, int dim, int heads, int k, int two_d,
                                    hipStream_t st);
hipError_t launch_copy_cols(float* dst, const float* src, size_t rows, int dim, int ld, int off, hipStream_t st);
hipError_t launch_sub(float* dst, const float* a, const float* b, size_t n, hipStream_t st);
hipError_t launch_small_k_matmul(const float* A, const float* W, float* Cm, int M, int N, int Kd, hipStream_t st);
hipError_t launch_attn_scoremap_backward(const float* qkv, const float* pe_w, const float* dO, float* dqkv, float* dpe_w,
                                         float* scratch, int n_regions, int P, int dim, int heads, int k, hipStream_t st);

hipError_t launch_crmsa_logits(const float* x1, const float* gamma, const float* beta,
                               const float* phi, float* mean_rstd, float* logits, int dim, int k,
                               const GridDev& g8, hipStream_t st);
bool crmsa_region_supported(int dim, int k, const GridDev& g8);
bool crmsa_region_enabled();
bool crmsa_region4_supported(int dim, int k, const GridDev& g8);
size_t crmsa_region4_scratch_floats(const GridDev& g8, int k);
hipError_t launch_crmsa_region4(const float* x1, const float* gamma, const float* beta, const float* phi,
                                float* mean_rstd, float* logits, float* wdisp, float* rep, uint16_t* rep16, int prec16,
                                float* part_g, int* counters, int k, const GridDev& g8, hipStream_t st);
hipError_t launch_crmsa_region(const float* x1, const float* gamma, const float* beta, const float* phi,
                               float* mean_rstd, float* logits, float* wdisp, float* rep, int k, const GridDev& g8,
                               hipStream_t st, uint16_t* rep16 = nullptr, int prec16 = 0);
bool crmsa_stream4_supported(int dim, int k, const GridDev& g8);
hipError_t launch_crmsa_stream4(const float* x1, const float* gamma, const float* beta, const float* phi,
                                float* mean_rstd, float* logits, float* wdisp, float* rep, uint16_t* rep16, int prec16,
                                float* part_g, int* counters, int k, const GridDev& g8, hipStream_t st);
hipError_t launch_crmsa_combine(const float* x1, const float* gamma, const float* beta,
                                const float* mean_rstd, const float* logits, float* wdisp,
                                float* rep, uint16_t* rep16, int prec16, int dim, int k, const GridDev& g8, hipStream_t st);
bool crmsa_combine_parts_supported(int dim, int k, const GridDev& g8);
size_t crmsa_parts_floats(long n_tokens, int dim, int k);
hipError_t launch_crmsa_combine_parts(const float* x1, const float* part, const float* gamma, const float* beta,
                                      const float* phi, float* wdisp, float* rep, uint16_t* rep16, int prec16, int dim,
                                      int k, const GridDev& g8, hipStream_t st);
hipError_t launch_crmsa_mlp_logits(const float* hid, const float* w2, float* logits, int rows, int hdim,
                                   int k, hipStream_t st);
hipError_t launch_crmsa_dispatch_ln(const float* x1, const float* x0, const float* wdisp,
                                    const float* rep2, const float* gamma,
                                    const float* beta, float* y, int dim, int k, const GridDev& g8,
                                    hipStream_t st, uint16_t* y16 = nullptr, int prec16 = 0);
hipError_t launch_layernorm(const float* x1, const float* x0, const float* gamma,
                            const float* beta, float* y, int L, int dim, hipStream_t st);

constexpr int POOL_CHUNK = 32;
hipError_t launch_pool_partial(const float* y, const float* hid_a, const float* hid_b, const float* wc,
                               const float* bc, float* a_raw, float* part, int N, int dim, int hid,
                               hipStream_t st);
hipError_t launch_pool_merge(const float* part, const float* a_raw, const float* pred_w, const float* pred_b,
                             float* pooled, float* logits, float* attn, int no_norm, int N, int dim,
                             int n_classes, hipStream_t st);

size_t pool_backward_part_floats(int N, int hid);
hipError_t launch_pool_backward(const float* y, const float* hid_a, const float* hid_b, const float* wc, const float* attn,
                                const float* pooled, const float* d_pooled, const float* d_attn, const float* d_raw,
                                const float* c_ext, float* dy, float* dhid_a, float* dhid_b, float* dwcb, float* part, int N,
                                int dim, int hid, hipStream_t st);

size_t linear_bwd_workspace(int M, int N, int K);
hipError_t launch_linear_backward(const float* dY, const float* X, const float* W, float* dX, float* dW, float* db,
                                  int M, int N, int K, int prec, void* ws, hipStream_t st, const float* WT_ready = nullptr);
hipError_t launch_transpose(const float* in, float* out, int R, int C, hipStream_t st);
constexpr int TRANSPOSE_MAX_JOBS = 2 * RRT_MAX_RMSA_LAYERS + 2;
struct TransposeJobs {
  const float* in[TRANSPOSE_MAX_JOBS];
  float* out[TRANSPOSE_MAX_JOBS];
  int R[TRANSPOSE_MAX_JOBS], C[TRANSPOSE_MAX_JOBS], blk0[TRANSPOSE_MAX_JOBS];
  int n;
};
hipError_t launch_transpose_batch(TransposeJobs& jobs, hipStream_t st);
hipError_t launch_reduce_partials(const float* part, float* out, int S, size_t n, hipStream_t st);
constexpr int REDUCE_MAX_JOBS = 16;
struct ReduceJobs {
  const float* part[REDUCE_MAX_JOBS];
  float* out[REDUCE_MAX_JOBS];
  float* out_tr[REDUCE_MAX_JOBS];
  unsigned long long n[REDUCE_MAX_JOBS], split[REDUCE_MAX_JOBS];
  int S[REDUCE_MAX_JOBS], tr_dim[REDUCE_MAX_JOBS], tr_k[REDUCE_MAX_JOBS];
  unsigned blk0[REDUCE_MAX_JOBS + 1];
  int count;
};
hipError_t reduce_or_defer(ReduceJobs* defer, const float* part, float* out, int S, size_t n, hipStream_t st,
                           size_t split = 0, float* out_tr = nullptr, int tr_dim = 0, int tr_k = 0);
hipError_t launch_reduce_jobs(ReduceJobs& jobs, hipStream_t st);
hipError_t launch_reduce_partials_scatter(const float* part, float* out, int S, size_t n, size_t split, float* out_tr,
                                          int tr_dim, int tr_k, hipStream_t st);
hipError_t launch_gemm_tn(const float* dY, const float* X, float* dW, float* scratch, int M, int N, int K,
                          hipStream_t st);
hipError_t launch_colsum(const float* Y, float* out, float* scratch, int M, int N, hipStream_t st);
size_t ln_bwd_workspace(int dim);
hipError_t launch_ln_backward(const float* dy, const float* x, const float* gamma, const float* add, float* dx,
                              float* dgb, float* part, int L, int dim, const GridDev* g, hipStream_t st,
                              ReduceJobs* defer = nullptr);
bool attn_bwd_supported(int P, int D, int heads, int epeg_k);
size_t attn_bwd_workspace(int n_regions, int P, int D, int heads, int epeg_k);
hipError_t launch_attention_backward(const float* qkv, const float* pe_w, const float* O, const float* dO,
                                     float* dqkv, float* dpe, float* dpe_part, int n_regions, int P, int D,
                                     int heads, int epeg_k, hipStream_t st, ReduceJobs* defer = nullptr,
                                     float* defer_part = nullptr);
hipError_t launch_partition_rows(const float* src, float* dst, int dim, const GridDev& g, unsigned drop_thresh,
                                 unsigned drop_seed, float drop_scale, hipStream_t st);
hipError_t launch_apply_drop_mask(float* buf, int rows, int cols, unsigned drop_thresh, unsigned drop_seed,
                                  float drop_scale, hipStream_t st);
hipError_t launch_crmsa_tokdot(const float* x, const float* mean_rstd, const float* gamma, const float* beta,
                               const float* vec, float* out, int dim, int k, const GridDev& g, hipStream_t st);
hipError_t launch_crmsa_wsum(const float* X, const float* W, float* out, int dim, int k, const GridDev& g,
                             hipStream_t st);
hipError_t launch_crmsa_bwd_region(const float* lg, const float* dC, const float* dWd, float* dlg, float* Cw, int k,
                                   const GridDev& g, hipStream_t st);
size_t crmsa_bwd_dx_workspace(int dim, int k);
hipError_t launch_crmsa_bwd_dx(const float* x1, const float* dx2, const float* mean_rstd, const float* gamma,
                               const float* beta, const float* phi, const float* Cw, const float* dlg,
                               const float* drep, float* dx1, float* out_rows, float* part, int dim, int k,
                               const GridDev& g, bool mlp, hipStream_t st, float* dphi_t = nullptr,
                               ReduceJobs* defer = nullptr);
hipError_t launch_crmsa_mlp_bwd_hidden(const float* hid, const float* dlg, const float* w2, float* th, float* dhid,
                                       size_t rows, int hdim, int k, hipStream_t st);
hipError_t launch_act_forward(const float* hpre, float* h, size_t n, int act, unsigned thresh, unsigned seed,
                              float scale, hipStream_t st);
hipError_t launch_act_backward(float* dh, const float* hpre, size_t n, int act, unsigned thresh, unsigned seed,
                               float scale, hipStream_t st);
hipError_t launch_copy_drop_mask(const float* src, float* dst, size_t n, unsigned drop_thresh, unsigned drop_seed,
                                 float drop_scale, hipStream_t st);
hipError_t launch_peg(const float* x, const float* const* w, const float* const* b, float* y, int N, int C, int k,
                      int conv_1d, int ppeg, hipStream_t st);
size_t peg_bwd_workspace(int N, int C, int k, int ppeg);
hipError_t launch_peg_backward(const float* x, const float* dy, const float* const* w, float* dx, float* const* dw,
                               float* const* db, int N, int C, int k, int conv_1d, int ppeg, void* ws, hipStream_t st);
```

rrt-mil_amd/csrc/rmsa_fused.hip:

```cpp
#include <stdio.h>
#include <stdlib.h>
#include <string.h>
#include <mutex>

#include "internal.h"

namespace {

constexpr int BK = 32;
constexpr int HD = 64;
constexpr int BN = 3 * HD;
constexpr float NEG_BIG = -3.0e38f;
constexpr float LOG2E = 1.4426950408889634f;

typedef float f32x2 __attribute__((ext_vector_type(2)));
template <bool WT>
__device__ __forceinline__ void store_o(f32x2* p, f32x2 v) {
  if constexpr (WT) asm volatile("global_store_dwordx2 %0, %1, off sc0 sc1" ::"v"(p), "v"(v) : "memory");
  else *p = v;
}
#define RRT_STORE_O(ptr, val) store_o<PROJ>((ptr), (val))

template <bool WT>
__device__ __forceinline__ void store_o(f32x4* p, f32x4 v) {
// ... 172 lines not shown
#pragma unroll
  for (int i = 0; i < MT; ++i) {
    const int t = token_of(i);
    toff[i] = t < 0 ? -1 : t * D + ncol;
  }
  float4 rq[PREF ? MT : 1];
  const float4 bias = pj.bias ? *(const float4*)(pj.bias + ncol) : make_float4(0.f, 0.f, 0.f, 0.f);
  f32x4 acc[MT];
#pragma unroll
  for (int i = 0; i < MT; ++i) acc[i] = (f32x4){0.f, 0.f, 0.f, 0.f};
  float4 af[2][MT], bfr[2];
  auto frags = [&](const float* As, const int kk, float4 (&a)[MT], float4& bb) {
    {
      const int row = wave * 16 + lr;
      bb = *(const float4*)(As + BM * BK + row * BK + (((4 * kk + lg) ^ ((row >> 1) & 7)) << 2));
    }
#pragma unroll
    for (int i = 0; i < MT; ++i) {
      const int row = i * 16 + lr;
      a[i] = *(const float4*)(As + row * BK + (((4 * kk + lg) ^ ((row >> 1) & 7)) << 2));
    }
  };
  auto half = [&](const float4 (&a)[MT], const float4& bb, const bool load, const float* nAs, const int nkk,
                  float4 (&na)[MT], float4& nb) {
    if (load) frags(nAs, nkk, na, nb);
#pragma unroll
    for (int comp = 0; comp < 4; ++comp) {
      const float bv = comp == 0 ? bb.x : comp == 1 ? bb.y : comp == 2 ? bb.z : bb.w;
#pragma unroll
      for (int i = 0; i < MT; ++i) {
        const float av = comp == 0 ? a[i].x : comp == 1 ? a[i].y : comp == 2 ? a[i].z : a[i].w;
        acc[i] = __builtin_amdgcn_mfma_f32_16x16x4f32(bv, av, acc[i], 0, 0, 0);
      }
    }
    if (load) {
#pragma unroll
      for (int r = 0; r < MT + 1; ++r) {
        __builtin_amdgcn_sched_group_barrier(0x008, 3, 0);
        __builtin_amdgcn_sched_group_barrier(0x100, 1, 0);
      }
      __builtin_amdgcn_sched_group_barrier(0x008, 4 * MT - 3 * (MT + 1), 0);
    }
    __builtin_amdgcn_sched_barrier(0);
  };
  auto lds_barrier = [] { asm volatile("s_waitcnt lgkmcnt(0)\n\ts_barrier" ::: "memory"); };
  RRT_TRACE_MARK();
  lds_barrier();
  RRT_TRACE_MARK();
  frags(lds, 0, af[0], bfr[0]);
  __builtin_amdgcn_sched_barrier(0);
  auto tile = [&](const int kt) {
    half(af[0], bfr[0], true, lds + (kt % NS) * SST, 1, af[1], bfr[1]);
    lds_barrier();
    if (kt == 0 || kt == 7 || kt == 14) RRT_TRACE_MARK();
    half(af[1], bfr[1], true, lds + ((kt + 1) % NS) * SST, 0, af[0], bfr[0]);
  };
  constexpr int RQA = PREF ? (RRT_PROJ_RQA < MT ? RRT_PROJ_RQA : MT) : 0;
  for (int kt = 0; kt + 2 < nk; ++kt) tile(kt);
  if constexpr (PREF) {
#pragma unroll
    for (int i = 0; i < RQA; ++i) rq[i] = ld_row<NT_RESID>(pj.resid + (toff[i] < 0 ? ncol : toff[i]));
  }
  if (nk >= 2) tile(nk - 2);
  if constexpr (PREF) {
#pragma unroll
    for (int i = RQA; i < MT; ++i) rq[i] = ld_row<NT_RESID>(pj.resid + (toff[i] < 0 ? ncol : toff[i]));
  }
  half(af[0], bfr[0], true, lds + ((nk - 1) % NS) * SST, 1, af[1], bfr[1]);
  lds_barrier();
  half(af[1], bfr[1], false, nullptr, 0, af[0], bfr[0]);
  RRT_TRACE_MARK();
  if constexpr (PREF) {
#pragma unroll
    for (int i = 0; i < MT; ++i) asm volatile("" : "+v"(rq[i].x), "+v"(rq[i].y), "+v"(rq[i].z), "+v"(rq[i].w));
  }
  if constexpr (KM == 0) {
#pragma unroll
    for (int i = 0; i < MT; ++i) {
      float4 q;
      if constexpr (PREF) q = rq[i];
      else q = ld_row<NT_RESID>(pj.resid + (toff[i] < 0 ? ncol : toff[i]));
      const float4 v = make_float4(acc[i][0] + bias.x + q.x, acc[i][1] + bias.y + q.y, acc[i][2] + bias.z + q.z, acc[i][3] + bias.w + q.w);
      if (toff[i] >= 0) *(float4*)(pj.out + toff[i]) = v;
    }
    RRT_TRACE_MARK();
  } else {
    constexpr int NF = KM <= 2 ? 1 : KM <= 6 ? 2 : 3;
    float4* const rec = (float4*)lds;
    const float* gpl = (const float*)(smem + LDS_MAIN_F * 4);
    float4 gp[KM];
#pragma unroll
    for (int n = 0; n < KM; ++n) gp[n] = *(const float4*)(gpl + n * 64 + wave * 16 + 4 * lg);
#pragma unroll
    for (int i = 0; i < MT; ++i) {
      float4 q;
      if constexpr (PREF) q = rq[i];
      else q = ld_row<NT_RESID>(pj.resid + (toff[i] < 0 ? ncol : toff[i]));
      const float4 v = make_float4(acc[i][0] + bias.x + q.x, acc[i][1] + bias.y + q.y, acc[i][2] + bias.z + q.z, acc[i][3] + bias.w + q.w);
      if (toff[i] >= 0) *(float4*)(pj.out + toff[i]) = v;
      const float m = ((v.x + v.y) + (v.z + v.w)) * 0.25f;
      const float a = v.x - m, b = v.y - m, c = v.z - m, d = v.w - m;
      float o[4 * NF];
      o[0] = m;
      o[1] = (a * a + b * b) + (c * c + d * d);
#pragma unroll
      for (int n = 0; n < 4 * NF - 2; ++n)
        o[2 + n] = n < KM ? (v.x * gp[n < KM ? n : 0].x + v.y * gp[n < KM ? n : 0].y) + (v.z * gp[n < KM ? n : 0].z + v.w * gp[n < KM ? n : 0].w) : 0.f;
      float4* const r = rec + ((size_t)(wave * 4 + lg) * BM + i * 16 + lr) * NF;
#pragma unroll
      for (int f = 0; f < NF; ++f) r[f] = make_float4(o[4 * f], o[4 * f + 1], o[4 * f + 2], o[4 * f + 3]);
    }
    RRT_TRACE_MARK();
    lds_barrier();
    const int m_ = tid;
    if (m_ < P) {
      const int pi = fdiv(m_, pj.g.s, pj.g.inv_s), pjj = m_ - pi * pj.g.s;
      const int t = tbase + pi * pj.g.H + pjj;
      if (t < pj.g.L) {
        float o[4 * NF];
        {
          const float4* r0 = rec + (size_t)m_ * NF;
#pragma unroll
          for (int f = 0; f < NF; ++f) {
            const float4 x = r0[f];
            o[4 * f] = x.x; o[4 * f + 1] = x.y; o[4 * f + 2] = x.z; o[4 * f + 3] = x.w;
          }
        }
#pragma unroll
        for (int j = 1; j < 16; ++j) {
          const float4* rj = rec + ((size_t)j * BM + m_) * NF;
          float x[4 * NF];
#pragma unroll
          for (int f = 0; f < NF; ++f) {
            const float4 y = rj[f];
            x[4 * f] = y.x; x[4 * f + 1] = y.y; x[4 * f + 2] = y.z; x[4 * f + 3] = y.w;
          }
          const float dl = x[0] - o[0], w = 1.0f / (float)(j + 1);
          o[0] += dl * w;
          o[1] += x[1] + dl * dl * (4.0f * (float)j * w);
#pragma unroll
          for (int n = 2; n < 4 * NF; ++n) o[n] += x[n];
        }
        const int nf = (2 + pj.k + 3) >> 2;
        float4* dst = (float4*)(pj.part + ((size_t)t * pj.n_slabs + col) * (4 * nf));
        dst[0] = make_float4(o[0], o[1], o[2], o[3]);
        if constexpr (NF > 1) if (nf > 1) dst[1] = make_float4(o[4], o[5], o[6], o[7]);
        if constexpr (NF > 2) if (nf > 2) dst[2] = make_float4(o[8], o[9], o[10], o[11]);
      }
    }
    RRT_TRACE_MARK();
  }
}

template <int MT, int PREC, bool PROJ, int KM = 0>
__global__ __launch_bounds__(512, 1) void rmsa_fused_kernel(const float* __restrict__ U,
                                                            const float* __restrict__ Wqkv,
                                                            const float* __restrict__ bqkv,
                                                            const float* __restrict__ pe_w,
                                                            float* __restrict__ O, int n_rows, int P,
                                                            int D, int heads_rt, int epeg_k, float q_scale,
                                                            float* __restrict__ stash, FusedProj pj) {
  static_assert(!PROJ || PREC == PREC_F32, "the projection phase is fp32 only");
  constexpr int BM = 16 * MT;
  constexpr int STAGE = (BM + BN) * BK;
  constexpr int TILE = BM * HD;
  constexpr int NA = BM / 8, NB = BN / 8;
  constexpr int LA = (NA + 3) / 4, LB = NB / 4;
  constexpr int NT = 3;
  constexpr int LDS_MAIN = (2 * STAGE > 3 * TILE ? 2 * STAGE : 3 * TILE) * 4;
  constexpr bool PIPE = PREC == PREC_F32 && MT <= 11;
  constexpr bool SPLIT_LAST = MT == 9;
  constexpr int RUN = (BM * 16 + 511) / 512;
  constexpr int TAP_OFF = 12 + RUN - 1;
  extern __shared__ __attribute__((aligned(16))) char smem[];
  float* lds = (float*)smem;
  float* Qs = lds;
  float* Ks = lds + TILE;
  float* Vs = lds + 2 * TILE;
  float* Qt = Qs;

  const int tid = threadIdx.x;
  const int lane = tid & 63;
  const int wave = __builtin_amdgcn_readfirstlane(tid >> 6);
  const int lr = lane & 15, lg = lane >> 4;
  const unsigned lds_b = lds_addr_of(lds);
#ifndef RRT_FUSED_PRIO
#define RRT_FUSED_PRIO 3
#endif
  if (RRT_FUSED_PRIO > 0) __builtin_amdgcn_s_setprio(RRT_FUSED_PRIO);
  const int n_items = PROJ ? pj.n_items : (int)gridDim.x;
  auto item_of = [&](const int b, int& reg_, int& head_) { map_item(b, n_items, heads_rt, reg_, head_); };
  const bool has_item = !PROJ || (int)blockIdx.x < n_items;
  int head = 0, reg = 0;
  if (has_item) item_of(blockIdx.x, reg, head);
  if constexpr (PROJ) {
    if (pj.zero64 != nullptr && blockIdx.x == 0 && threadIdx.x < 64) pj.zero64[threadIdx.x] = 0;
  }
  const int row0 = reg * P;
  const int nk = D / BK;
  RRT_TRACE_INIT(blockIdx.x * 8 + wave);
  if (has_item) {
  float* const taps = (float*)(smem + LDS_MAIN);
  float* const bias_l = taps + 128;
  if (tid >= 128 && tid < 128 + BN) {
    const int n = tid - 128;
    bias_l[n] = bqkv ? bqkv[(n >> 6) * D + head * HD + (n & 63)] : 0.f;
  }
  if (tid < 128) {
    const int t = tid - TAP_OFF;
    float wt = (pe_w != nullptr && t >= 0 && t < epeg_k) ? pe_w[head * epeg_k + t] : 0.f;
    if (t == (epeg_k >> 1)) wt += 1.0f;
    taps[tid] = wt * LOG2E;
  }
  RRT_TRACE_MARK();

  if (wave >= 4) {
    const int lw = wave - 4;
    unsigned aoff[LA], boff[LB];
#pragma unroll
    for (int qi = 0; qi < LA; ++qi) {
      int S = (qi * 4 + lw) * 64 + lane;
      int row = S >> 3, p = S & 7;
      int gr = row0 + row;
      gr = gr < n_rows ? gr : n_rows - 1;
      aoff[qi] = (unsigned)gr * (unsigned)D * 4u + (unsigned)((p ^ ((row >> 1) & 7)) << 4);
    }
#pragma unroll
    for (int qi = 0; qi < LB; ++qi) {
      int S = (qi * 4 + lw) * 64 + lane;
      int row = S >> 3, p = S & 7;
      int wr = (row >> 6) * D + head * HD + (row & 63);
      boff[qi] = (unsigned)wr * (unsigned)D * 4u + (unsigned)((p ^ ((row >> 1) & 7)) << 4);
    }
    auto stage = [&](int kt, unsigned buf) {
#pragma unroll
      for (int qi = 0; qi < LA; ++qi)
        if (qi * 4 + lw < NA) dma16s(U + kt * BK, aoff[qi], buf + (qi * 4 + lw) * 1024);
#pragma unroll
      for (int qi = 0; qi < LB; ++qi) dma16s(Wqkv + kt * BK, boff[qi], buf + BM * BK * 4 + (qi * 4 + lw) * 1024);
    };
    stage(0, lds_b);
    if constexpr (PIPE) {
      wait_vm0();
      __syncthreads();
      if (nk > 1) stage(1, lds_b + STAGE * 4);
      for (int kt = 0; kt < nk; ++kt) {
        wait_vm0();
        __syncthreads();
        if (kt + 2 < nk) stage(kt + 2, lds_b + (kt & 1) * STAGE * 4);
      }
    } else {
      for (int kt = 0; kt < nk; ++kt) {
        wait_vm0();
        __syncthreads();
        if (kt + 1 < nk) stage(kt + 1, lds_b + ((kt + 1) & 1) * STAGE * 4);
      }
    }
  } else {
    f32x4 acc[MT][NT];
#pragma unroll
    for (int i = 0; i < MT; ++i)
#pragma unroll
      for (int j = 0; j < NT; ++j) acc[i][j] = (f32x4){0.f, 0.f, 0.f, 0.f};
    if constexpr (PIPE) {
      float4 af[MT], bfr[2][NT];
      auto a_frag = [&](const float* As, int kk, int i) {
        const int row = i * 16 + lr;
        return *(const float4*)(As + row * BK + (((4 * kk + lg) ^ ((row >> 1) & 7)) << 2));
      };
      auto b_frag = [&](const float* As, int kk, int j) {
        const int row = wave * (16 * NT) + j * 16 + lr;
        return *(const float4*)(As + BM * BK + row * BK + (((4 * kk + lg) ^ ((row >> 1) & 7)) << 2));
      };
      auto mm = [&](const int i, const float4 (&bc)[NT]) {
#pragma unroll
        for (int comp = 0; comp < 4; ++comp)
#pragma unroll
          for (int j = 0; j < NT; ++j) {
            const float a = comp == 0 ? af[i].x : comp == 1 ? af[i].y : comp == 2 ? af[i].z : af[i].w;
            const float b = comp == 0 ? bc[j].x : comp == 1 ? bc[j].y : comp == 2 ? bc[j].z : bc[j].w;
            acc[i][j] = __builtin_amdgcn_mfma_f32_16x16x4f32(b, a, acc[i][j], 0, 0, 0);
          }
        __builtin_amdgcn_sched_barrier(0);
      };
      auto first_half = [&](const float* As, const bool owe) {
        mm(0, bfr[0]);
        if (owe) af[MT - 1] = a_frag(As, 0, MT - 1);
        __builtin_amdgcn_sched_barrier(0);
#pragma unroll
        for (int i = 1; i < MT; ++i) {
          mm(i, bfr[0]);
          af[i - 1] = a_frag(As, 1, i - 1);
          if (i <= NT) bfr[1][i - 1] = b_frag(As, 1, i - 1);
          __builtin_amdgcn_sched_barrier(0);
        }
      };
      auto second_head = [&](const float* As) {
        mm(0, bfr[1]);
        af[MT - 1] = a_frag(As, 1, MT - 1);
        __builtin_amdgcn_sched_barrier(0);
        mm(1, bfr[1]);
      };
      auto second_tail = [&](const float* nAs, const bool refill) {
        if (refill) {
          af[0] = a_frag(nAs, 0, 0);
          bfr[0][0] = b_frag(nAs, 0, 0);
          __builtin_amdgcn_sched_barrier(0);
        }
#pragma unroll
        for (int i = 2; i < MT; ++i) {
          mm(i, bfr[1]);
          if (refill) {
            af[i - 1] = a_frag(nAs, 0, i - 1);
            if (i <= NT) bfr[0][i - 1] = b_frag(nAs, 0, i - 1);
            __builtin_amdgcn_sched_barrier(0);
          }
        }
      };
      static_assert(MT > NT, "the refill schedule needs more row tiles than column tiles");
      __syncthreads();
      RRT_TRACE_MARK();
#pragma unroll
      for (int i = 0; i < MT; ++i) af[i] = a_frag(lds, 0, i);
#pragma unroll
      for (int j = 0; j < NT; ++j) bfr[0][j] = b_frag(lds, 0, j);
      first_half(lds, false);
      second_head(lds);
      __syncthreads();
      RRT_TRACE_MARK();
      for (int kt = 1; kt < nk; ++kt) {
        const float* As = lds + (kt & 1) * STAGE;
        __builtin_amdgcn_sched_barrier(0);
        second_tail(As, true);
        first_half(As, true);
        second_head(As);
        __syncthreads();
        if (kt == 7) RRT_TRACE_MARK();
      }
      second_tail(nullptr, false);
    } else {
    for (int kt = 0; kt < nk; ++kt) {
      __syncthreads();
      if (kt == 0 || kt == 1 || kt == 8) RRT_TRACE_MARK();
      const float* As = lds + (kt & 1) * STAGE;
      const float* Bs = As + BM * BK;
      if constexpr (PREC == PREC_F32) {
#pragma unroll
        for (int kk = 0; kk < 2; ++kk) {
          float4 af[MT], bf[NT];
          const int cslot = 4 * kk + lg;
#pragma unroll
          for (int j = 0; j < NT; ++j) {
            int row = wave * (16 * NT) + j * 16 + lr;
            bf[j] = *(const float4*)(Bs + row * BK + ((cslot ^ ((row >> 1) & 7)) << 2));
          }
#pragma unroll
          for (int i = 0; i < MT; ++i) {
            int row = i * 16 + lr;
            af[i] = *(const float4*)(As + row * BK + ((cslot ^ ((row >> 1) & 7)) << 2));
          }
#pragma unroll
          for (int comp = 0; comp < 4; ++comp)
#pragma unroll
            for (int i = 0; i < MT; ++i)
#pragma unroll
              for (int j = 0; j < NT; ++j) {
                const float a = comp == 0 ? af[i].x : comp == 1 ? af[i].y : comp == 2 ? af[i].z : af[i].w;
                const float b = comp == 0 ? bf[j].x : comp == 1 ? bf[j].y : comp == 2 ? bf[j].z : bf[j].w;
                acc[i][j] = __builtin_amdgcn_mfma_f32_16x16x4f32(b, a, acc[i][j], 0, 0, 0);
              }
        }
      } else {
        using F = Frag8<PREC>;
        typename F::type a8[MT], b8[NT];
#pragma unroll
        for (int j = 0; j < NT; ++j) {
          const int row = wave * (16 * NT) + j * 16 + lr, f = (row >> 1) & 7;
          b8[j] = F::pack(*(const float4*)(Bs + row * BK + (((2 * lg) ^ f) << 2)),
                          *(const float4*)(Bs + row * BK + (((2 * lg + 1) ^ f) << 2)));
        }
#pragma unroll
        for (int i = 0; i < MT; ++i) {
          const int row = i * 16 + lr, f = (row >> 1) & 7;
          a8[i] = F::pack(*(const float4*)(As + row * BK + (((2 * lg) ^ f) << 2)),
                          *(const float4*)(As + row * BK + (((2 * lg + 1) ^ f) << 2)));
        }
#pragma unroll
        for (int i = 0; i < MT; ++i)
#pragma unroll
          for (int j = 0; j < NT; ++j) acc[i][j] = F::mfma(b8[j], a8[i], acc[i][j]);
      }
    }
    }
    RRT_TRACE_MARK();
    __syncthreads();
#pragma unroll
    for (int j = 0; j < NT; ++j) {
      const int n = wave * (16 * NT) + j * 16 + 4 * lg;
      const int c = n >> 6, d = n & 63;
      const float4 b = *(const float4*)(bias_l + n);
      const float sc = c == 0 ? q_scale : 1.0f;
      float* dstm = c == 0 ? Qs : (c == 1 ? Ks : Vs);
#pragma unroll
      for (int i = 0; i < MT; ++i) {
        const int m = i * 16 + lr;
        const int slot = (d >> 2) ^ (m & 15);
        float4 v = make_float4((acc[i][j][0] + b.x) * sc, (acc[i][j][1] + b.y) * sc,
                               (acc[i][j][2] + b.z) * sc, (acc[i][j][3] + b.w) * sc);
        *(float4*)(dstm + m * HD + (slot << 2)) = v;
      }
    }
  }
  if (wave >= 4) __syncthreads();
  __syncthreads();
  RRT_TRACE_MARK();
  if (stash != nullptr) {
    for (int idx = tid; idx < BM * 16 * 3; idx += 512) {
      const int c = idx / (BM * 16), rem = idx - c * (BM * 16);
      const int m = rem >> 4, sl = rem & 15;
      if (m < P) {
        const float4 v = *(const float4*)(lds + c * TILE + m * HD + ((sl ^ (m & 15)) << 2));
        *(float4*)(stash + (size_t)(row0 + m) * (3 * D) + c * D + head * HD + 4 * sl) = v;
      }
    }
  }

  {
    static_assert(RUN - 1 <= TAP_OFF && (TAP_OFF - (RUN - 1)) % 4 == 0 && 2 * RUN + 90 < 128, "tap table range / alignment");
    const int half = epeg_k >> 1;
    const int s = tid & 15, g = tid >> 4;
    const int r0 = g * RUN;
    f32x2 out[RUN][2];
#pragma unroll
    for (int o = 0; o < RUN; ++o) out[o][0] = out[o][1] = (f32x2){0.f, 0.f};
    if (r0 < BM) {
      const int nsrc = RUN + 2 * half;
      constexpr int NTV = (RUN + 3 + 3) / 4;
      const float4* tp4 = (const float4*)(taps + TAP_OFF - (RUN - 1));
      constexpr int NFAST = RUN + 14;
      if (nsrc <= NFAST) {
        constexpr int NTT = (NFAST + RUN - 1 + 3) / 4;
        float4 v[NFAST];
        float T[4 * NTT];
#pragma unroll
        for (int u = 0; u < NFAST; ++u) {
          const int rr = r0 - half + u;
          const bool ok = rr >= 0 && rr < P;
          const int rc = ok ? rr : 0;
          v[u] = *(const float4*)(Qs + rc * HD + ((s ^ (rc & 15)) << 2));
          if (!ok) v[u] = make_float4(0.f, 0.f, 0.f, 0.f);
        }
#pragma unroll
        for (int q = 0; q < NTT; ++q) {
          const float4 t4 = tp4[q];
          T[4 * q] = t4.x; T[4 * q + 1] = t4.y; T[4 * q + 2] = t4.z; T[4 * q + 3] = t4.w;
        }
#pragma unroll
        for (int u = 0; u < NFAST; ++u) {
          const f32x2 lo = {v[u].x, v[u].y}, hi = {v[u].z, v[u].w};
#pragma unroll
          for (int o = 0; o < RUN; ++o) {
            const float wt = T[u + RUN - 1 - o];
            const f32x2 w2 = {wt, wt};
            out[o][0] = __builtin_elementwise_fma(w2, lo, out[o][0]);
            out[o][1] = __builtin_elementwise_fma(w2, hi, out[o][1]);
          }
        }
      } else
      for (int j0 = 0; j0 < nsrc; j0 += 4) {
        float4 v[4];
        float T[4 * NTV];
#pragma unroll
        for (int q = 0; q < NTV; ++q) {
          const float4 t4 = tp4[(j0 >> 2) + q];
          T[4 * q] = t4.x; T[4 * q + 1] = t4.y; T[4 * q + 2] = t4.z; T[4 * q + 3] = t4.w;
        }
#pragma unroll
        for (int u = 0; u < 4; ++u) {
          const int rr = r0 - half + j0 + u;
          const bool ok = rr >= 0 && rr < P;
          const int rc = ok ? rr : 0;
          v[u] = *(const float4*)(Qs + rc * HD + ((s ^ (rc & 15)) << 2));
          if (!ok) v[u] = make_float4(0.f, 0.f, 0.f, 0.f);
        }
#pragma unroll
        for (int u = 0; u < 4; ++u) {
          const f32x2 lo = {v[u].x, v[u].y}, hi = {v[u].z, v[u].w};
#pragma unroll
          for (int o = 0; o < RUN; ++o) {
            const float wt = T[u + RUN - 1 - o];
            const f32x2 w2 = {wt, wt};
            out[o][0] = __builtin_elementwise_fma(w2, lo, out[o][0]);
            out[o][1] = __builtin_elementwise_fma(w2, hi, out[o][1]);
          }
        }
      }
    }
    __syncthreads();
    if (r0 < BM) {
#pragma unroll
      for (int o = 0; o < RUN; ++o) {
        const int m = r0 + o;
        if (m < BM)
          *(float4*)(Qt + m * HD + ((s ^ (m & 15)) << 2)) = make_float4(out[o][0][0], out[o][0][1], out[o][1][0], out[o][1][1]);
      }
    }
  }
  __syncthreads();
  RRT_TRACE_MARK();

  if constexpr (SPLIT_LAST) {
    constexpr int XT = MT - 1;
    float* const pstat = (float*)(smem + LDS_MAIN + 1280);
    float* const plast = pstat + MT * 32;
    const int i0 = wave * 16;
    int tk[MT];
#pragma unroll
    for (int j = 0; j < MT; ++j) tk[j] = j + wave < MT ? j + wave : j + wave - MT;
    float4 bq[4], bx[4];
    {
      const int m = i0 + lr, mx = XT * 16 + lr;
#pragma unroll
      for (int c = 0; c < 4; ++c) {
        bq[c] = *(const float4*)(Qt + m * HD + (((4 * c + lg) ^ lr) << 2));
        bx[c] = *(const float4*)(Qt + mx * HD + (((4 * c + lg) ^ lr) << 2));
      }
    }
    f32x4 s[MT], sx = {0.f, 0.f, 0.f, 0.f}, sy = {0.f, 0.f, 0.f, 0.f};
#pragma unroll
    for (int j = 0; j < MT; ++j) s[j] = (f32x4){0.f, 0.f, 0.f, 0.f};
#pragma unroll
    for (int c = 0; c < 4; ++c) {
      float4 a[MT];
#pragma unroll
      for (int j = 0; j < MT; ++j) a[j] = *(const float4*)(Ks + (tk[j] * 16 + lr) * HD + (((4 * c + lg) ^ lr) << 2));
#pragma unroll
      for (int comp = 0; comp < 4; ++comp) {
        const float qb = comp == 0 ? bq[c].x : comp == 1 ? bq[c].y : comp == 2 ? bq[c].z : bq[c].w;
        const float xb = comp == 0 ? bx[c].x : comp == 1 ? bx[c].y : comp == 2 ? bx[c].z : bx[c].w;
#pragma unroll
        for (int j = 0; j < MT; ++j) {
          const float ka = comp == 0 ? a[j].x : comp == 1 ? a[j].y : comp == 2 ? a[j].z : a[j].w;
          s[j] = __builtin_amdgcn_mfma_f32_16x16x4f32(ka, qb, s[j], 0, 0, 0);
          if (j == 0) sx = __builtin_amdgcn_mfma_f32_16x16x4f32(ka, xb, sx, 0, 0, 0);
        }
      }
    }
    if (wave == 0) {
#pragma unroll
      for (int c = 0; c < 4; ++c) {
        const float4 a8 = *(const float4*)(Ks + (XT * 16 + lr) * HD + (((4 * c + lg) ^ lr) << 2));
        sy = __builtin_amdgcn_mfma_f32_16x16x4f32(a8.x, bx[c].x, sy, 0, 0, 0);
        sy = __builtin_amdgcn_mfma_f32_16x16x4f32(a8.y, bx[c].y, sy, 0, 0, 0);
        sy = __builtin_amdgcn_mfma_f32_16x16x4f32(a8.z, bx[c].z, sy, 0, 0, 0);
        sy = __builtin_amdgcn_mfma_f32_16x16x4f32(a8.w, bx[c].w, sy, 0, 0, 0);
      }
    }
    RRT_TRACE_MARK();
    float cmax = NEG_BIG, xmax = NEG_BIG, ymax = NEG_BIG;
    if (P < BM) {
#pragma unroll
// ... 112 lines not shown
        for (int r = 0; r < 4; ++r)
          *(float4*)(plast + (4 * lg + r) * HD + 4 * lr) = make_float4(oy[0][r], oy[1][r], oy[2][r], oy[3][r]);
        if (lg == 0) {
          pstat[XT * 32 + lr] = ymax;
          pstat[XT * 32 + 16 + lr] = ysum;
        }
      }
    }
    RRT_TRACE_MARK();
    __syncthreads();
    RRT_TRACE_MARK();
    {
      const int q = tid >> 5, col = (tid & 31) * 2;
      float mw[MT], M = NEG_BIG;
#pragma unroll
      for (int w = 0; w < MT; ++w) {
        mw[w] = pstat[w * 32 + q];
        M = fmaxf(M, mw[w]);
      }
      float L = 0.f, o0 = 0.f, o1 = 0.f;
#pragma unroll
      for (int w = 0; w < MT; ++w) {
        const float sc = __builtin_amdgcn_exp2f(mw[w] - M);
        L += sc * pstat[w * 32 + 16 + q];
        const float2 a = *(const float2*)((w < XT ? Qt + w * 16 * HD : plast) + q * HD + col);
        o0 += sc * a.x;
        o1 += sc * a.y;
      }
      const float invL = 1.0f / L;
      if (XT * 16 + q < P)
        RRT_STORE_O((f32x2*)(O + (size_t)(row0 + XT * 16 + q) * D + head * HD + col), ((f32x2){o0 * invL, o1 * invL}));
      RRT_TRACE_MARK();
    }
  } else {
  for (int t = wave; t < MT; t += 8) {
    const int i0 = t * 16;
    if (i0 >= P) break;
    float4 bq[4];
    {
      const int m = i0 + lr;
#pragma unroll
      for (int c = 0; c < 4; ++c) bq[c] = *(const float4*)(Qt + m * HD + (((4 * c + lg) ^ (m & 15)) << 2));
    }
    f32x4 s[MT];
#pragma unroll
    for (int jt = 0; jt < MT; ++jt) s[jt] = (f32x4){0.f, 0.f, 0.f, 0.f};
#pragma unroll
    for (int c = 0; c < 4; ++c) {
      float4 a[MT];
#pragma unroll
      for (int jt = 0; jt < MT; ++jt) {
        const int row = jt * 16 + lr;
        a[jt] = *(const float4*)(Ks + row * HD + (((4 * c + lg) ^ (row & 15)) << 2));
      }
#pragma unroll
      for (int jt = 0; jt < MT; ++jt) s[jt] = __builtin_amdgcn_mfma_f32_16x16x4f32(a[jt].x, bq[c].x, s[jt], 0, 0, 0);
#pragma unroll
      for (int jt = 0; jt < MT; ++jt) s[jt] = __builtin_amdgcn_mfma_f32_16x16x4f32(a[jt].y, bq[c].y, s[jt], 0, 0, 0);
#pragma unroll
      for (int jt = 0; jt < MT; ++jt) s[jt] = __builtin_amdgcn_mfma_f32_16x16x4f32(a[jt].z, bq[c].z, s[jt], 0, 0, 0);
#pragma unroll
      for (int jt = 0; jt < MT; ++jt) s[jt] = __builtin_amdgcn_mfma_f32_16x16x4f32(a[jt].w, bq[c].w, s[jt], 0, 0, 0);
    }
    RRT_TRACE_MARK();
    float cmax = NEG_BIG;
    if (P < BM) {
#pragma unroll
      for (int jt = 0; jt < MT; ++jt)
#pragma unroll
        for (int r = 0; r < 4; ++r)
          if (jt * 16 + 4 * lg + r >= P) s[jt][r] = NEG_BIG;
    }
#pragma unroll
    for (int jt = 0; jt < MT; ++jt)
#pragma unroll
      for (int r = 0; r < 4; ++r) cmax = fmaxf(cmax, s[jt][r]);
    cmax = max_xor32(max_xor16(cmax));
    float a4[4] = {0.f, 0.f, 0.f, 0.f};
#pragma unroll
    for (int jt = 0; jt < MT; ++jt)
#pragma unroll
      for (int r = 0; r < 4; ++r) {
        const float e = __builtin_amdgcn_exp2f(s[jt][r] - cmax);
        s[jt][r] = e;
        a4[r] += e;
      }
    const float psum = sum_xor32(sum_xor16((a4[0] + a4[1]) + (a4[2] + a4[3])));
    float ir[4];
    {
      const float inv = 1.0f / psum;
#pragma unroll
      for (int r = 0; r < 4; ++r) ir[r] = __shfl(inv, 4 * lg + r);
    }
    RRT_TRACE_MARK();
    f32x4 oacc[4];
#pragma unroll
    for (int c = 0; c < 4; ++c) oacc[c] = (f32x4){0.f, 0.f, 0.f, 0.f};
#pragma unroll
    for (int jt = 0; jt < MT; ++jt)
#pragma unroll
      for (int r = 0; r < 4; ++r) {
        const int row = jt * 16 + 4 * lg + r;
        const float4 v = *(const float4*)(Vs + row * HD + ((lr ^ (row & 15)) << 2));
        const float p = s[jt][r];
        oacc[0] = __builtin_amdgcn_mfma_f32_16x16x4f32(p, v.x, oacc[0], 0, 0, 0);
        oacc[1] = __builtin_amdgcn_mfma_f32_16x16x4f32(p, v.y, oacc[1], 0, 0, 0);
        oacc[2] = __builtin_amdgcn_mfma_f32_16x16x4f32(p, v.z, oacc[2], 0, 0, 0);
        oacc[3] = __builtin_amdgcn_mfma_f32_16x16x4f32(p, v.w, oacc[3], 0, 0, 0);
      }
    RRT_TRACE_MARK();
#pragma unroll
    for (int r = 0; r < 4; ++r) {
      const int i = i0 + 4 * lg + r;
      if (i < P)
        RRT_STORE_O((f32x4*)(O + (size_t)(row0 + i) * D + head * HD + (lr << 2)),
                    ((f32x4){oacc[0][r] * ir[r], oacc[1][r] * ir[r], oacc[2][r] * ir[r], oacc[3][r] * ir[r]}));
    }
    RRT_TRACE_MARK();
  }
  }
  if constexpr (PROJ) {
    wait_vm0();
    __syncthreads();
    RRT_TRACE_MARK();
    if (tid == 0) __hip_atomic_fetch_add(pj.cnt + reg, 1, __ATOMIC_RELAXED, __HIP_MEMORY_SCOPE_AGENT);
  }
  }
  if constexpr (PROJ) proj_slab<MT, KM>(U, O, n_rows, P, D, heads_rt, pj, smem RRT_SLAB_TRACE_PASS);
}

int proj_lag(int n_items) {
  static int cus[64] = {};
  int d = 0;
  (void)hipGetDevice(&d);
  d &= 63;
  if (cus[d] == 0) {
    int n = 0;
    if (hipDeviceGetAttribute(&n, hipDeviceAttributeMultiprocessorCount, d) != hipSuccess || n <= 0) n = 256;
    cus[d] = n;
  }
  int lag = cus[d] & ~7;
  if (lag > n_items) lag = n_items & ~7;
  static const char* force = rrt_tune_env("RRT_PROJ_LAG");
  if (force != nullptr && atoi(force) > 0) lag = atoi(force);
  return lag;
}

template <int MT, int PREC>
hipError_t launch_mt(const float* U, const float* Wqkv, const float* bqkv, const float* pe_w, float* O,
                     int n_regions, int P, int D, int heads, int epeg_k, float* stash, hipStream_t st,
                     const FusedProj* proj) {
  constexpr int BM = 16 * MT;
  constexpr size_t STG = (size_t)2 * (BM + BN) * BK * 4, QKV = (size_t)3 * BM * HD * 4;
  constexpr size_t LDS = (STG > QKV ? STG : QKV) + (MT == 9 ? 1280 + MT * 32 * 4 + 16 * HD * 4 : 2064);
  static_assert(LDS <= 160 * 1024, "LDS budget");
  const float q_scale = 1.0f / sqrtf((float)HD);
  if constexpr (PREC == PREC_F32) {
    if (proj != nullptr) {
      FusedProj pj = *proj;
      pj.n_items = heads * n_regions;
      if (pj.lag <= 0) pj.lag = proj_lag(pj.n_items);
      if (pj.wait_for <= 0) pj.wait_for = heads;
      pj.n_slabs = D / HD;
      if (pj.part != nullptr && (pj.ln_g == nullptr || pj.phi == nullptr || pj.k < 1 || pj.k > RRT_MAX_CRMSA_K))
        return hipErrorInvalidValue;
      if (pj.spin_limit <= 0) pj.spin_limit = 1 << 22;
      if (pj.err == nullptr) pj.err = handover_err_device();
#define RRT_LAUNCH_PROJ(KM_)                                                                                    \
  do {                                                                                                           \
    auto kern = rmsa_fused_kernel<MT, PREC_F32, true, KM_>;                                                      \
    static OncePerDevice once;                                                                                   \
    if (once.first())                                                                                            \
      (void)hipFuncSetAttribute((const void*)kern, hipFuncAttributeMaxDynamicSharedMemorySize, (int)LDS);        \
    kern<<<dim3(pj.n_items + pj.lag), dim3(512), LDS, st>>>(U, Wqkv, bqkv, pe_w, O, n_regions * P, P, D, heads,  \
                                                            pe_w ? epeg_k : 0, q_scale, nullptr, pj);            \
  } while (0)
      if constexpr (MT >= 6) {
        if (pj.part != nullptr && pj.k <= 4) RRT_LAUNCH_PROJ(4);
        else if (pj.part != nullptr) RRT_LAUNCH_PROJ(8);
        else RRT_LAUNCH_PROJ(0);
      } else {
        if (pj.part != nullptr) return hipErrorInvalidValue;
        RRT_LAUNCH_PROJ(0);
      }
#undef RRT_LAUNCH_PROJ
      return hipGetLastError();
    }
  }
  auto kern = rmsa_fused_kernel<MT, PREC, false>;
  static OncePerDevice once;
  if (once.first())
    (void)hipFuncSetAttribute((const void*)kern, hipFuncAttributeMaxDynamicSharedMemorySize, (int)LDS);
  kern<<<dim3(heads * n_regions), dim3(512), LDS, st>>>(U, Wqkv, bqkv, pe_w, O, n_regions * P, P, D, heads,
                                                      pe_w ? epeg_k : 0, q_scale, stash, FusedProj{});
  return hipGetLastError();
}

}

#ifdef RRT_TRACE
RRT_TRACE_DEFINE_READER(rrt_debug_trace_fused)
#endif

namespace {
int* g_err_host = nullptr;
int* g_err_dev = nullptr;
std::once_flag g_err_once;
void handover_err_init() {
  void* h = nullptr;
  if (hipHostMalloc(&h, 64, hipHostMallocMapped | hipHostMallocPortable) == hipSuccess && h != nullptr) {
    memset(h, 0, 64);
    void* d = nullptr;
    if (hipHostGetDevicePointer(&d, h, 0) == hipSuccess && d != nullptr) {
      g_err_dev = (int*)d;
      __atomic_store_n(&g_err_host, (int*)h, __ATOMIC_RELEASE);
    }
  } else {
    (void)hipGetLastError();
  }
}
}
int* handover_err_device() {
  std::call_once(g_err_once, handover_err_init);
  return g_err_dev;
}
int handover_err_peek(bool clear) {
  int* const eh = __atomic_load_n(&g_err_host, __ATOMIC_ACQUIRE);
  if (eh == nullptr) return 0;
  const int v = __atomic_load_n(eh, __ATOMIC_RELAXED);
  if (clear && v != 0) __atomic_store_n(eh, 0, __ATOMIC_RELAXED);
  return v;
}

bool rmsa_fused_supported(int P, int D, int heads, int epeg_k) {
  static const bool off = rrt_tune_env("RRT_NO_FUSED") != nullptr;
  if (off) return false;
  return heads > 0 && D == heads * HD && D % BK == 0 && P > 48 && P <= 208 && epeg_k >= 0 && epeg_k <= 63;
}

bool rmsa_fused_supported_rows(long n_rows, int D) {
  return n_rows * (long)D * 4 < 4000000000L;
}

bool rmsa_fused_proj_supported(int n_regions, int P, int D, int heads, int epeg_k, int prec) {
  static const bool off = rrt_tune_env("RRT_NO_FUSED_PROJ") != nullptr;
  if (off || prec != PREC_F32 || !rmsa_fused_supported(P, D, heads, epeg_k)) return false;
  const int n_items = n_regions * heads, lag = proj_lag(n_items);
  return D % 4 == 0 && P > 64 && n_items >= 2 * lag && lag >= 8 * heads;
}

hipError_t launch_rmsa_fused(const float* U, const float* Wqkv, const float* bqkv, const float* pe_w,
                             float* O, int n_regions, int P, int D, int heads, int epeg_k, int prec,
                             hipStream_t st, float* stash, const FusedProj* proj) {
  if (proj != nullptr && (stash != nullptr || !rmsa_fused_proj_supported(n_regions, P, D, heads, epeg_k, prec)))
    return hipErrorInvalidValue;
  if (proj != nullptr && proj->lag > 0 && (proj->lag < 8 * heads || proj->lag > n_regions * heads)) return hipErrorInvalidValue;
#define RRT_FUSED(MT_)                                                                              \
  switch (prec) {                                                                                   \
    case 1: return launch_mt<MT_, PREC_BF16>(U, Wqkv, bqkv, pe_w, O, n_regions, P, D, heads, epeg_k, stash, st, proj); \
    case 2: return launch_mt<MT_, PREC_F16>(U, Wqkv, bqkv, pe_w, O, n_regions, P, D, heads, epeg_k, stash, st, proj);  \
    default: return launch_mt<MT_, PREC_F32>(U, Wqkv, bqkv, pe_w, O, n_regions, P, D, heads, epeg_k, stash, st, proj); \
  }
  if (P > 176) { RRT_FUSED(13) }
  if (P > 144) { RRT_FUSED(11) }
  if (P > 128) { RRT_FUSED(9) }
  if (P > 112) { RRT_FUSED(8) }
  if (P > 96) { RRT_FUSED(7) }
  if (P > 64) { RRT_FUSED(6) }
  RRT_FUSED(4)
#undef RRT_FUSED
}
```

rrt-mil_amd/encoder.py:

```python
import os
import warnings
import contextlib
import ctypes as C
import math

import numpy as np

import torch
from torch import nn

from . import _lib


def initialize_weights(module):
    for m in module.modules():
        if isinstance(m, (nn.Conv2d, nn.Linear)):
            nn.init.xavier_normal_(m.weight)
            if m.bias is not None:
                m.bias.data.zero_()
        elif isinstance(m, nn.LayerNorm):
            nn.init.constant_(m.bias, 0)
            nn.init.constant_(m.weight, 1.0)


# ... 303 lines not shown

    def _apply(self, fn, *a, **kw):
        r = super()._apply(fn, *a, **kw)
        self.__dict__["_plist"] = None
        self.__dict__["_w_struct"] = None
        return r

    def _weights(self):
        ver = self._weights_version()
        w = self.__dict__.get("_w_struct")
        if w is not None:
            return w
        w = _lib.EncoderWeights()
        w.version = ver
        for i, layer in enumerate(self.layers.children()):
            w.rmsa[i] = self._attn_weights(layer)
        if self._desc.cr_msa:
            w.crmsa = self._attn_weights(self.cr_msa)
            if self._desc.crmsa_mlp:
                w.phi0_w = self._ptr(self.cr_msa.attn.phi[0].weight)
                w.phi2_w = self._ptr(self.cr_msa.attn.phi[2].weight)
            else:
                w.phi = self._ptr(self.cr_msa.attn.phi)
        w.norm_w, w.norm_b = self._ptr(self.norm.weight), self._ptr(self.norm.bias)
        if self._desc.pos:
            for i, name in enumerate(("proj", "proj1", "proj2")):
                conv = getattr(self.pos_embedding, name, None)
                if conv is not None:
                    w.pos_w[i], w.pos_b[i] = self._ptr(conv.weight), self._ptr(conv.bias)
        self.__dict__["_w_struct"] = w
        return w

    def _grad_buffers(self, device):
        D = self.final_dim
        gs = _lib.EncoderGrads()
        by_name = {}

        def ln(prefix):
            t = torch.empty((2, D), dtype=torch.float32, device=device)
            by_name[prefix + ".weight"], by_name[prefix + ".bias"] = t[0], t[1]
            return t.data_ptr()

        def attn(prefix, layer, ag):
            ia = layer.attn.attn
            ag.norm = ln(prefix + "norm")
            for nm, mod in (("qkv", ia.qkv), ("proj", ia.proj)):
                gw = torch.empty_like(mod.weight)
                by_name[f"{prefix}attn.attn.{nm}.weight"] = gw
                setattr(ag, nm + "_w", gw.data_ptr())
                if mod.bias is not None:
                    gb = torch.empty_like(mod.bias)
                    by_name[f"{prefix}attn.attn.{nm}.bias"] = gb
                    setattr(ag, nm + "_b", gb.data_ptr())
            if ia.pe is not None:
                gw = torch.empty_like(ia.pe.weight)
                by_name[prefix + "attn.attn.pe.weight"] = gw
                ag.pe_w = gw.data_ptr()
                if ia.pe.bias is not None:
                    if ia.epeg_type == 'attn':
                        by_name[prefix + "attn.attn.pe.bias"] = torch.zeros_like(ia.pe.bias)
                    else:
                        gb = torch.empty_like(ia.pe.bias)
                        by_name[prefix + "attn.attn.pe.bias"] = gb
                        ag.pe_b = gb.data_ptr()
            if layer.ffn:
                ag.norm2 = ln(prefix + "norm2")
                for nm in ("fc1", "fc2"):
                    mod = getattr(layer.mlp, nm)
                    gw, gb = torch.empty_like(mod.weight), torch.empty_like(mod.bias)
                    by_name[f"{prefix}mlp.{nm}.weight"], by_name[f"{prefix}mlp.{nm}.bias"] = gw, gb
                    setattr(ag, nm + "_w", gw.data_ptr())
                    setattr(ag, nm + "_b", gb.data_ptr())

        gs.norm = ln("norm")
        for i, layer in enumerate(self.layers.children()):
            attn(f"layers.{i}.", layer, gs.rmsa[i])
        if self._desc.cr_msa:
            attn("cr_msa.", self.cr_msa, gs.crmsa)
            if self._desc.crmsa_mlp:
                g0 = torch.empty_like(self.cr_msa.attn.phi[0].weight)
                g2 = torch.empty_like(self.cr_msa.attn.phi[2].weight)
                by_name["cr_msa.attn.phi.0.weight"], by_name["cr_msa.attn.phi.2.weight"] = g0, g2
                gs.phi0_w, gs.phi2_w = g0.data_ptr(), g2.data_ptr()
            else:
                gphi = torch.empty_like(self.cr_msa.attn.phi)
                by_name["cr_msa.attn.phi"] = gphi
                gs.phi = gphi.data_ptr()
        if self._desc.pos:
            for i, name in enumerate(("proj", "proj1", "proj2")):
                conv = getattr(self.pos_embedding, name, None)
                if conv is None:
                    continue
                gw = torch.empty_like(conv.weight)
                by_name[f"pos_embedding.{name}.weight"] = gw
                gs.pos_w[i] = gw.data_ptr()
                if conv.bias is not None:
                    gb = torch.empty_like(conv.bias)
                    by_name[f"pos_embedding.{name}.bias"] = gb
                    gs.pos_b[i] = gb.data_ptr()
        elif not isinstance(self.pos_embedding, nn.Identity):
            for name, _ in self.pos_embedding.named_parameters():
                by_name["pos_embedding." + name] = None
        grads = [by_name[name] for name, _ in self.named_parameters()]
        return grads, gs

    def _workspace(self, n_tokens, device):
        cache = self.__dict__.setdefault("_ws_need", {})
        key = (int(n_tokens), int(self._desc.compute))
        need = cache.get(key)
        if need is None:
            lib = _lib.load()
            c_need = C.c_size_t()
            _lib.check(lib.rrt_encoder_workspace_size(C.byref(self._desc), n_tokens, C.byref(c_need)),
                       "rrt_encoder_workspace_size")
            need = cache[key] = int(c_need.value)
            if len(cache) > 4096:
                cache.clear()
        ws = self._ws
        if ws is None or ws.device != device or ws.numel() < need:
            ws = self._ws = torch.empty(need, dtype=torch.uint8, device=device)
        return ws

    def _compute_mode(self):
        dt = self.compute_dtype
        if dt is None and torch.is_autocast_enabled("cuda"):
            dt = torch.get_autocast_dtype("cuda")
        return {None: _lib.COMPUTE_F32, torch.float32: _lib.COMPUTE_F32, torch.bfloat16: _lib.COMPUTE_BF16,
                torch.float16: _lib.COMPUTE_F16, "f32x3": _lib.COMPUTE_F32X3}[dt]

    def forward_bag(self, x2d, out=None):
        lib = _lib.load()
        if not x2d.is_cuda:
            raise _lib.RRTHipError("rrt_mil_amd.RRTEncoder runs on MI355X only: move the bag to a "
                                   "'cuda' (HIP) device; there is no CPU fallback")
        if x2d.dtype in (torch.bfloat16, torch.float16):
            x2d = x2d.float()
        if x2d.dtype != torch.float32:
            raise NotImplementedError(f"unsupported bag dtype {x2d.dtype}")
        x2d = x2d.contiguous()
        n, d = x2d.shape
        if d != self.final_dim:
            raise ValueError(f"expected feature dim {self.final_dim}, got {d}")
        y = out if out is not None else torch.empty_like(x2d)
        if self._stochastic():
            return self._forward_bag_stochastic(x2d, y)
        desc, d_ = self._desc, self.__dict__
        mode = desc.compute = self._compute_mode()
        ws = self._workspace(n, x2d.device)
        w = self._weights()
        dev = x2d.device
        ctx = torch.cuda.device(dev) if torch.cuda.current_device() != dev.index else _NULL_CTX
        with ctx:
            stream = torch.cuda.current_stream(dev).cuda_stream
            lowp = mode != _lib.COMPUTE_F32
            key = (ws.data_ptr(), mode, w.version, stream) if lowp else None
            desc.weights16_valid = int(lowp and key == d_.get("_w16_key"))
            desc.solo = int(d_.get("solo", True))
            rc = lib.rrt_encoder_forward_f32(C.byref(desc), C.byref(w), x2d.data_ptr(), y.data_ptr(), n,
                                             ws.data_ptr(), ws.numel(), stream)
            desc.weights16_valid = 0
            d_["_w16_key"] = key if rc == 0 else None
        if rc:
            _lib.check(rc, "rrt_encoder_forward_f32")
        return y

    def forward_batch(self, x3d):
        lib = _lib.load()
        if not x3d.is_cuda:
            raise _lib.RRTHipError("rrt_mil_amd.RRTEncoder runs on MI355X only; there is no CPU fallback")
        x3d = x3d.float().contiguous()
        b, n, d = x3d.shape
        if d != self.final_dim:
            raise ValueError(f"expected feature dim {self.final_dim}, got {d}")
        desc = self._desc
        desc.compute = self._compute_mode()
        need = C.c_size_t()
        _lib.check(lib.rrt_encoder_batch_workspace_size(C.byref(desc), b, n, C.byref(need)), "rrt_encoder_batch_workspace_size")
        ws = torch.empty(need.value, dtype=torch.uint8, device=x3d.device)
        y = torch.empty_like(x3d)
        w = self._weights()
        with torch.cuda.device(x3d.device):
            desc.weights16_valid = 0
            rc = lib.rrt_encoder_forward_batch_f32(C.byref(desc), C.byref(w), x3d.data_ptr(), y.data_ptr(), b, n,
                                                   ws.data_ptr(), ws.numel(), torch.cuda.current_stream(x3d.device).cuda_stream)
        _lib.check(rc, "rrt_encoder_forward_batch_f32")
        return y

    def _stochastic(self):
        return self.training and (self.drop_out > 0 or any(l.drop_path_p > 0 for l in self._trans_layers()))

    def _trans_layers(self):
        layers = list(self.layers.children())
        if self._desc.cr_msa:
            layers.append(self.cr_msa)
        return layers

    def _branch_scales(self):
        if not self.training or not any(l.drop_path_p > 0 for l in self._trans_layers()):
            return None
        n = _lib.RRT_MAX_RMSA_LAYERS + 1
        arr = (C.c_float * (2 * n))(*([1.0] * (2 * n)))
        layers = list(self.layers.children())
        slots = [(i, l) for i, l in enumerate(layers)] + ([(len(layers), self.cr_msa)] if self._desc.cr_msa else [])
        fixed = getattr(self, "drop_path_draws", None)
        k = 0
        for part in (0, 1):
            for idx, layer in slots:
                if part == 1 and not layer.ffn:
                    continue
                keep = 1.0 - layer.drop_path_p
                if fixed is not None:
                    m = float(fixed[k])
                else:
                    m = (1.0 / keep if keep > 0 else 1.0) if float(torch.rand(())) < keep else 0.0
                arr[part * n + idx] = m
                k += 1
        return arr

    def _forward_bag_stochastic(self, x2d, y):
        lib = _lib.load()
        self._desc.compute = self._compute_mode()
        stash_b, ws_b = C.c_size_t(), C.c_size_t()
        _lib.check(lib.rrt_encoder_train_sizes(C.byref(self._desc), x2d.shape[0], C.byref(stash_b), C.byref(ws_b)),
                   "rrt_encoder_train_sizes")
        stash = torch.empty(stash_b.value, dtype=torch.uint8, device=x2d.device)
        w = self._weights()
        drop_p = float(self.drop_out)
        with torch.cuda.device(x2d.device):
            rc = lib.rrt_encoder_forward_train_f32(C.byref(self._desc), C.byref(w), x2d.data_ptr(), y.data_ptr(),
                                                   x2d.shape[0], stash.data_ptr(), stash.numel(), drop_p,
                                                   self._next_drop_seed() if drop_p > 0 else 0, self._branch_scales(),
                                                   torch.cuda.current_stream(x2d.device).cuda_stream)
        _lib.check(rc, "rrt_encoder_forward_train_f32")
        return y

    def _executor(self, n_streams, max_tokens, device):
        key = (n_streams, device)
        ex = getattr(self, "_ex", None)
        self._desc.weights16_valid, self._desc.solo = 0, 0
        if ex is not None and self._ex_key == key and bytes(self._ex_desc) == bytes(self._desc):
            return ex
        self._drop_executor()
        lib = _lib.load()
        h = C.c_void_p()
        with torch.cuda.device(device):
            if os.environ.get("RRT_EXEC_OWN_STREAMS") == "1":
                _lib.check(lib.rrt_executor_create(C.byref(self._desc), n_streams, max_tokens, C.byref(h)),
                           "rrt_executor_create")
            else:
                pool = _BAG_STREAMS.setdefault(device, [])
                off = int(os.environ.get("RRT_EXEC_POOL_OFFSET", "0"))
                while len(pool) < n_streams + off:
                    pool.append(torch.cuda.Stream(device))
                hs = [pool[off + n_streams - 1].cuda_stream] + [st.cuda_stream for st in pool[off:off + n_streams - 1]]
                arr = (C.c_void_p * n_streams)(*hs)
                _lib.check(lib.rrt_executor_create_on_streams(C.byref(self._desc), n_streams, arr, max_tokens, C.byref(h)),
                           "rrt_executor_create_on_streams")
        self._ex, self._ex_key, self._ex_desc = h, key, _lib.EncoderDesc.from_buffer_copy(self._desc)
        return h

    def _drop_executor(self):
        ex = getattr(self, "_ex", None)
        if ex is not None:
            _lib.load().rrt_executor_destroy(ex)
            self._ex = None

    def __del__(self):
        try:
            self._drop_executor()
        except Exception:
            pass

    @torch.no_grad()
    def forward_bags(self, bags, streams=4, outs=None):
        lib = _lib.load()
        n_bags = len(bags)
        if not n_bags:
            return []
        if self._stochastic():
            return [self.forward_bag(b[0]).unsqueeze(0) if b.dim() == 3 else self.forward_bag(b) for b in bags]
        dev = bags[0].device
        D, f32 = self.final_dim, torch.float32
        xs = bags
        for b in bags:
            nd = b.dim()
            if (b.dtype is not f32 or b.device != dev or not b.is_contiguous() or b.size(-1) != D
                    or not (nd == 2 or (nd == 3 and b.size(0) == 1))):
                xs = None
                break
        if xs is None:
            xs = []
            for b in bags:
                if not b.is_cuda or b.device != dev:
                    raise _lib.RRTHipError("forward_bags: every bag must be on the same HIP device (no CPU fallback)")
                x2 = b[0] if b.dim() == 3 and b.size(0) == 1 else b
                if x2.dim() != 2 or x2.size(1) != D:
                    raise ValueError(f"forward_bags: expected (N, {D}) or (1, N, {D}) bags, got {tuple(b.shape)}")
                if x2.dtype in (torch.bfloat16, torch.float16):
                    x2 = x2.float()
                if x2.dtype != f32:
                    raise NotImplementedError(f"unsupported bag dtype {x2.dtype}")
                xs.append(x2.contiguous())
        elif not dev.type == "cuda":
            raise _lib.RRTHipError("forward_bags: every bag must be on the same HIP device (no CPU fallback)")
        if outs is None:
            ys = [torch.empty_like(x) for x in xs]
        else:
            ys = outs
            if len(ys) != n_bags:
# ... 99 lines not shown
```

rrt-mil_amd/mil.py:

```python
import ctypes as C

import torch
import torch.nn.functional as F
from torch import nn

from . import _lib
from .encoder import RRTEncoder, initialize_weights


def _act(name):
    return {"gelu": nn.GELU, "relu": nn.ReLU, "tanh": nn.Tanh}.get(name)


class _LibLinear(torch.autograd.Function):

    @staticmethod
    def forward(ctx, x2d, weight, bias, compute):
        lib = _lib.load()
        x2d = x2d.float().contiguous()
        M, K = x2d.shape
        N = weight.shape[0]
        y = torch.empty((M, N), dtype=torch.float32, device=x2d.device)
        with torch.cuda.device(x2d.device):
            st = torch.cuda.current_stream(x2d.device).cuda_stream
# ... 164 lines not shown
    def forward(self, x, return_attn=False, no_norm=False, **kwargs):
        x, attn = self.attention(x, no_norm)
        return (x.squeeze(1), attn.squeeze(1)) if return_attn else x.squeeze(1)


class RRTMIL(nn.Module):
    def __init__(self, input_dim=1024, mlp_dim=512, act='relu', n_classes=2, dropout=0.25, pos_pos=0,
                 pos='none', peg_k=7, attn='rmsa', pool='attn', region_num=8, n_layers=2, n_heads=8,
                 drop_path=0., da_act='relu', trans_dropout=0.1, ffn=False, ffn_act='gelu', mlp_ratio=4.,
                 da_gated=False, da_bias=False, da_dropout=False, trans_dim=64, epeg=True,
                 min_region_num=0, qkv_bias=True, **kwargs):
        super().__init__()
        if pool != 'attn':
            raise NotImplementedError("pool='attn' only (the reference's avg-pool branch pools the wrong axis)")
        emb = [nn.Linear(input_dim, 512)]
        if act.lower() == 'relu':
            emb.append(nn.ReLU())
        elif act.lower() == 'gelu':
            emb.append(nn.GELU())
        self.dp = nn.Dropout(dropout) if dropout > 0. else nn.Identity()
        self.patch_to_emb = nn.Sequential(*emb)
        self.online_encoder = RRTEncoder(
            mlp_dim=mlp_dim, pos_pos=pos_pos, pos=pos, peg_k=peg_k, attn=attn, region_num=region_num,
            n_layers=n_layers, n_heads=n_heads, drop_path=drop_path, drop_out=trans_dropout, ffn=ffn,
            ffn_act=ffn_act, mlp_ratio=mlp_ratio, trans_dim=trans_dim, epeg=epeg,
            min_region_num=min_region_num, qkv_bias=qkv_bias, **kwargs)
        self.pool_fn = DAttention(self.online_encoder.final_dim, da_act, gated=da_gated, bias=da_bias,
                                  dropout=da_dropout)
        self.predictor = nn.Linear(self.online_encoder.final_dim, n_classes)
        if self.patch_to_emb[0].out_features != self.online_encoder.final_dim:
            raise ValueError(f"patch_to_emb emits 512 features but the encoder was built with mlp_dim="
                             f"{self.online_encoder.final_dim} (the reference fails on this combination too)")
        self.apply(initialize_weights)

        self._act_name = act.lower() if act.lower() in ("relu", "gelu") else "none"
        self._da_act = da_act
        self._ws = None

    def __getstate__(self):
        st = dict(self.__dict__)
        for k in ("_ws", "_slots", "_w16_key"):
            st.pop(k, None)
        return st

    def __setstate__(self, st):
        self.__dict__.update(st)
        self.__dict__.setdefault("_ws", None)

    def _mil_desc(self, input_dim, solo=True):
        enc = self.online_encoder
        d = _lib.MilDesc()
        C.memmove(C.byref(d.enc), C.byref(enc._desc), C.sizeof(_lib.EncoderDesc))
        d.enc.compute = enc._compute_mode()
        d.enc.solo = int(bool(solo))
        d.input_dim = input_dim
        d.emb_act = _lib.ACT_BY_NAME.get(self._act_name, _lib.ACT_NONE)
        d.n_classes = self.predictor.out_features
        att = self.pool_fn.attention
        d.pool_hidden = att.D
        d.pool_act = _lib.ACT_BY_NAME.get(self._da_act, _lib.ACT_NONE)
        d.pool_gated = int(self.pool_fn.gated)
        return d

    def _mil_weights(self):
        enc, p = self.online_encoder, RRTEncoder._ptr
        w = _lib.MilWeights()
        w.enc = enc._weights()
        lin = self.patch_to_emb[0]
        w.emb_w, w.emb_b = p(lin.weight), p(lin.bias)
        att = self.pool_fn.attention
        if self.pool_fn.gated:
            a, b, c = att.attention_a[0], att.attention_b[0], att.attention_c
            w.pool_b_w, w.pool_b_b = p(b.weight), p(b.bias)
        else:
            a, c = att.attention[0], att.attention[-1]
        w.pool_a_w, w.pool_a_b = p(a.weight), p(a.bias)
        w.pool_c_w, w.pool_c_b = p(c.weight), p(c.bias)
        w.pred_w, w.pred_b = p(self.predictor.weight), p(self.predictor.bias)
        return w

    @torch.no_grad()
    def forward_bags(self, bags, streams=4, return_attn=False, no_norm=False):
        if not bags:
            return []
        if self.training and (isinstance(self.dp, nn.Dropout) or self.online_encoder._stochastic()):
            return [self(b if b.dim() == 3 else b.unsqueeze(0), return_attn=return_attn, no_norm=no_norm) for b in bags]
        from .encoder import _BAG_STREAMS
        dev = bags[0].device
        if not bags[0].is_cuda:
            raise _lib.RRTHipError("rrt_mil_amd.RRTMIL runs on MI355X only; there is no CPU fallback")
        S = max(1, min(int(streams), 4, len(bags)))
        pool = _BAG_STREAMS.setdefault(dev, [])
        while len(pool) < S:
            pool.append(torch.cuda.Stream(dev))
        slots = self.__dict__.setdefault("_slots", {})
        cur = torch.cuda.current_stream(dev)
        order = sorted(range(len(bags)), key=lambda i: -bags[i].shape[-2])
        load, outs = [0] * S, [None] * len(bags)
        for st in pool[:S]:
            st.wait_stream(cur)
        ws_was, key_was = self._ws, self.__dict__.get("_w16_key")
        try:
            for i in order:
                s_ = min(range(S), key=lambda t: load[t])
                load[s_] += bags[i].shape[-2]
                b = bags[i]
                x2 = b[0] if b.dim() == 3 else b
                self._ws, self.__dict__["_w16_key"] = slots.get((dev, s_), (None, None))
                with torch.cuda.stream(pool[s_]):
                    o = self.forward_bag(x2, return_attn=return_attn, no_norm=no_norm, solo=(S == 1))
                slots[(dev, s_)] = (self._ws, self.__dict__.get("_w16_key"))
                for t_ in (o if return_attn else (o,)):
                    t_.record_stream(cur)
                if b.dim() == 3:
                    o = tuple(t.unsqueeze(0) for t in o) if return_attn else o.unsqueeze(0)
                outs[i] = o
        finally:
            self._ws, self.__dict__["_w16_key"] = ws_was, key_was
            for st in pool[:S]:
                st.synchronize()
        return outs

    def forward_bag(self, x2d, return_attn=False, no_norm=False, solo=True):
        lib = _lib.load()
        if not x2d.is_cuda:
            raise _lib.RRTHipError("rrt_mil_amd.RRTMIL runs on MI355X only: move the bag to a 'cuda' (HIP) "
                                   "device; there is no CPU fallback")
        if self.training and (isinstance(self.dp, nn.Dropout) or self.online_encoder._stochastic()):
            raise NotImplementedError("forward_bag is the one-call inference entry (no dropout inside); in train() "
                                      "call the module itself: forward() applies the dropouts and records a graph")
        n, in_dim = x2d.shape
        if in_dim != self.patch_to_emb[0].in_features:
            raise ValueError(f"expected feature dim {self.patch_to_emb[0].in_features}, got {in_dim}")
        d = self._mil_desc(in_dim, solo=solo)
        if x2d.dtype in (torch.bfloat16, torch.float16):
            want = {torch.bfloat16: _lib.COMPUTE_BF16, torch.float16: _lib.COMPUTE_F16}[x2d.dtype]
            if d.enc.compute == want and in_dim % 64 == 0:
                d.input16 = want
            else:
                x2d = x2d.float()
        elif x2d.dtype != torch.float32:
            raise NotImplementedError(f"unsupported bag dtype {x2d.dtype}")
        x2d = x2d.contiguous()
        w = self._mil_weights()
        need = C.c_size_t()
        _lib.check(lib.rrt_mil_workspace_size(C.byref(d), n, C.byref(need)), "rrt_mil_workspace_size")
        if self._ws is None or self._ws.device != x2d.device or self._ws.numel() < need.value:
            self._ws = torch.empty(need.value, dtype=torch.uint8, device=x2d.device)
        logits = torch.empty(d.n_classes, dtype=torch.float32, device=x2d.device)
        attn = torch.empty(n, dtype=torch.float32, device=x2d.device) if return_attn else None
        with torch.cuda.device(x2d.device):
            stream = torch.cuda.current_stream(x2d.device).cuda_stream
            key = (self._ws.data_ptr(), d.enc.compute, w.enc.version, stream, n)
            lowp = d.enc.compute != _lib.COMPUTE_F32
            d.enc.weights16_valid = int(lowp and key == getattr(self, "_w16_key", None))
            rc = lib.rrt_mil_forward_f32(C.byref(d), C.byref(w), x2d.data_ptr(), logits.data_ptr(),
                                         attn.data_ptr() if return_attn else None, int(bool(no_norm)), None, n,
                                         self._ws.data_ptr(), self._ws.numel(), stream)
            self._w16_key = key if rc == 0 and lowp else None
        _lib.check(rc, "rrt_mil_forward_f32")
        return (logits, attn) if return_attn else logits

    def forward(self, x, return_attn=False, no_norm=False):
        if torch.is_grad_enabled() and (x.requires_grad or any(p.requires_grad for p in self.parameters())):
            return self._forward_layers(x, return_attn, no_norm)
        with torch.no_grad():
            if self.training and (isinstance(self.dp, nn.Dropout) or self.online_encoder._stochastic()
                                  or any(isinstance(m, nn.Dropout) for m in self.pool_fn.modules())):
                return self._forward_layers(x, return_attn, no_norm)
            return self._forward_infer(x, return_attn, no_norm)

    def _forward_infer(self, x, return_attn=False, no_norm=False):
        if x.dim() == 3 and x.size(0) == 1 and x.is_cuda:
            out = self.forward_bag(x[0], return_attn=return_attn, no_norm=no_norm)
            if return_attn:
                return out[0].unsqueeze(0), out[1].unsqueeze(0)
            return out.unsqueeze(0)
        return self._forward_layers(x, return_attn, no_norm)

    def _forward_layers(self, x, return_attn=False, no_norm=False):
        enc = self.online_encoder
        if x.is_cuda:
            compute = enc._compute_mode()
            compute = _lib.COMPUTE_F32 if compute == _lib.COMPUTE_F32X3 else compute
            h = lib_linear(self.patch_to_emb[0], x, compute)
            for m in list(self.patch_to_emb)[1:]:
                h = m(h)
            x = self.dp(h.float())
        else:
            x = self.dp(self.patch_to_emb(x))
        x = enc(x)
        x, a = self._pool(x, no_norm)
        logits = self.predictor(x)
        return (logits, a) if return_attn else logits

    def _pool(self, x, no_norm):
        att = self.pool_fn.attention
        if not x.is_cuda:
            return self.pool_fn(x, return_attn=True, no_norm=no_norm)
        compute = self.online_encoder._compute_mode()
        compute = _lib.COMPUTE_F32 if compute == _lib.COMPUTE_F32X3 else compute

        def seq(mods, t):
            t = lib_linear(mods[0], t, compute)
            for m in list(mods)[1:]:
                t = m(t)
            return t
        if self.pool_fn.gated:
            ha, hb, lin_c = seq(att.attention_a, x), seq(att.attention_b, x), att.attention_c
        else:
            mods = list(att.attention)
            ha, hb, lin_c = seq(mods[:-1], x), None, mods[-1]
        out = lib_attn_pool(x, ha, hb, lin_c)
        if out is not None:
            pooled, a, a_raw = out
            return pooled, (a_raw if no_norm else a)
        s = lin_c(ha.mul(hb) if hb is not None else ha).transpose(-1, -2)
        a_raw = s.clone()
        a = F.softmax(s, dim=-1)
        pooled = torch.matmul(a, x).squeeze(1)
        return pooled, (a_raw if no_norm else a).squeeze(1)
```

Baseline: 5420.

## Fold LayerNorm into the fused RMSA QKV GEMM and skip partition pass

```diff
diff --git a/include/rrt_hip.h b/include/rrt_hip.h
--- a/include/rrt_hip.h
+++ b/include/rrt_hip.h
@@ -97,6 +97,8 @@
 #define RRT_PLAN_CRMSA_PARTS 16
 #define RRT_PLAN_ATTN_HD    32
 int rrt_encoder_plan(const rrt_encoder_desc *desc, int64_t n_tokens, int32_t *flags);
+#define RRT_PLAN_LN_FOLD    64
+int rrt_encoder_plan_ext(const rrt_encoder_desc *desc, int64_t n_tokens, int32_t *flags);
 
 int rrt_encoder_forward_f32(const rrt_encoder_desc *desc, const rrt_encoder_weights *w,
                             const float *x, float *y, int64_t n_tokens,
@@ -168,6 +170,11 @@
 int rrt_crmsa_combine_parts_f32(const float *x1, const float *part, const float *gamma, const float *beta,
                                 const float *phi, float *wdisp, float *rep, int64_t n_tokens, int32_t dim, int32_t k,
                                 const rrt_grid *g8, void *stream);
+int rrt_rmsa_fused_lnfold_supported(int32_t dim, int32_t heads, int32_t epeg_k, const rrt_grid *g);
+int rrt_rmsa_fused_lnfold_f32(const float *x, const float *ln_w, const float *ln_b, const float *qkv_w, const float *qkv_b,
+                              const float *pe_w, const float *proj_w, const float *proj_b, float *out, float *o_scratch,
+                              int32_t *counters, float *fold, float *qkv_stash, int32_t dim, int32_t heads,
+                              int32_t epeg_k, const rrt_grid *g, void *stream);
 int rrt_device_error(int32_t clear);
 int rrt_debug_rmsa_fused_proj_f32(const float *u, const float *qkv_w, const float *qkv_b, const float *pe_w,
                                   const float *proj_w, const float *proj_b, const float *resid, float *out,
diff --git a/rrt-mil_amd/_lib.py b/rrt-mil_amd/_lib.py
--- a/rrt-mil_amd/_lib.py
+++ b/rrt-mil_amd/_lib.py
@@ -77,6 +77,7 @@
     "rrt_region_grid": (C.c_int, [C.c_int64, C.c_int32, C.c_int32, C.c_int32, C.c_float, C.POINTER(Grid)]),
     "rrt_encoder_workspace_size": (C.c_int, [C.POINTER(EncoderDesc), C.c_int64, C.POINTER(C.c_size_t)]),
     "rrt_encoder_plan": (C.c_int, [C.POINTER(EncoderDesc), C.c_int64, C.POINTER(C.c_int32)]),
+    "rrt_encoder_plan_ext": (C.c_int, [C.POINTER(EncoderDesc), C.c_int64, C.POINTER(C.c_int32)]),
     "rrt_encoder_forward_f32": (C.c_int, [C.POINTER(EncoderDesc), C.POINTER(EncoderWeights), C.c_void_p,
                                           C.c_void_p, C.c_int64, C.c_void_p, C.c_size_t, C.c_void_p]),
     "rrt_encoder_forward_events_f32": (C.c_int, [C.POINTER(EncoderDesc), C.POINTER(EncoderWeights), C.c_void_p,
@@ -106,6 +107,8 @@
     "rrt_rmsa_fused_proj_f32": (C.c_int, [C.c_void_p] * 10 + [C.c_int32] * 3 + [C.c_void_p] * 2),
     "rrt_device_error": (C.c_int, [C.c_int32]),
     "rrt_rmsa_fused_proj_stats_f32": (C.c_int, [C.c_void_p] * 12 + [C.c_int32, C.c_void_p] + [C.c_int32] * 3 + [C.c_void_p] * 2),
+    "rrt_rmsa_fused_lnfold_supported": (C.c_int, [C.c_int32] * 3 + [C.POINTER(Grid)]),
+    "rrt_rmsa_fused_lnfold_f32": (C.c_int, [C.c_void_p] * 13 + [C.c_int32] * 3 + [C.POINTER(Grid), C.c_void_p]),
     "rrt_crmsa_combine_parts_f32": (C.c_int, [C.c_void_p] * 7 + [C.c_int64, C.c_int32, C.c_int32, C.POINTER(Grid), C.c_void_p]),
     "rrt_debug_rmsa_fused_proj_f32": (C.c_int, [C.c_void_p] * 10 + [C.c_int32] * 3 + [C.c_void_p] + [C.c_int32] * 3 + [C.c_void_p]),
     "rrt_cast16": (C.c_int, [C.c_void_p, C.c_void_p, C.c_int64, C.c_int32, C.c_void_p]),
@@ -177,6 +180,7 @@
 EPEG_ATTN, EPEG_VALUE_BF, EPEG_VALUE_AF = 0, 1, 2
 
 PLAN_FUSED, PLAN_FUSED_PROJ, PLAN_FUSED16, PLAN_FUSED_X3, PLAN_CRMSA_PARTS, PLAN_ATTN_HD = 1, 2, 4, 8, 16, 32
+PLAN_LN_FOLD = 64
 EV_START, EV_LN_PARTITION, EV_QKV, EV_ATTN, EV_PROJ, EV_CR_COMBINE, EV_CR_INNER, EV_END, EV_COUNT = range(9)
 
 _lib = None
diff --git a/rrt-mil_amd/csrc/api.hip b/rrt-mil_amd/csrc/api.hip
--- a/rrt-mil_amd/csrc/api.hip
+++ b/rrt-mil_amd/csrc/api.hip
@@ -125,6 +125,11 @@
   return RRT_OK;
 }
 
+bool ln_fold_images_wanted(const rrt_encoder_desc& d, bool want_x3, bool epeg_variant) {
+  return d.n_rmsa_layers > 0 && d.compute == RRT_COMPUTE_F32 && !want_x3 && !epeg_variant && d.n_heads > 0 &&
+         d.dim == d.n_heads * 64 && (!d.epeg || d.epeg_k <= 63) && rmsa_fused_lnfold_enabled();
+}
+
 hipError_t inner_attention(const float* u, int n_regions, int P, const rrt_attn_weights& w, int dim,
                            int heads, int epeg_k, float* qkv, float* o, int prec, bool solo, hipStream_t st) {
   const int M = n_regions * P;
@@ -219,6 +224,12 @@
 }
 
 int rrt_encoder_plan(const rrt_encoder_desc* desc, int64_t n_tokens, int32_t* flags) {
+  const int rc = rrt_encoder_plan_ext(desc, n_tokens, flags);
+  if (flags) *flags &= ~RRT_PLAN_LN_FOLD;
+  return rc;
+}
+
+int rrt_encoder_plan_ext(const rrt_encoder_desc* desc, int64_t n_tokens, int32_t* flags) {
   if (!flags) return RRT_E_INVALID;
   *flags = 0;
   int rc = check_desc(desc, n_tokens);
@@ -246,6 +257,9 @@
     *flags = RRT_PLAN_FUSED;
     if (compute == RRT_COMPUTE_F32 && rmsa_fused_proj_supported(gd.rs * gd.rs, gd.P, D, desc->n_heads, ek, compute)) {
       *flags |= RRT_PLAN_FUSED_PROJ;
+      if (ln_fold_images_wanted(*desc, want_x3, epeg_variant) &&
+          rmsa_fused_lnfold_supported(gd.rs * gd.rs, gd.P, D, desc->n_heads, ek, compute))
+        *flags |= RRT_PLAN_LN_FOLD;
       rrt_grid g8{};
       if (rrt_region_grid(n_tokens, 8, 0, 0, 0.f, &g8) == RRT_OK && desc->solo != 0 && desc->crmsa_k <= 4 && desc->cr_msa &&
           !desc->crmsa_mlp && !desc->ffn && D % 64 == 0 &&
@@ -397,6 +411,18 @@
       jobs.src[jobs.count] = lw.proj_w; jobs.dst[jobs.count] = base + (size_t)6 * D * D; jobs.n4[jobs.count++] = (size_t)D * D / 4;
     }
     if (!desc->weights16_valid) RRT_TRY(launch_cast_split(jobs, st));
+  }
+  const bool ln_fold_images = ln_fold_images_wanted(*desc, want_x3, epeg_variant);
+  if (ln_fold_images) {
+    LnFoldJobs jobs{};
+    for (int li = 0; li < desc->n_rmsa_layers; ++li) {
+      const rrt_attn_weights& lw = w->rmsa[li];
+      if (!lw.norm_w || !lw.norm_b || !lw.qkv_w) return RRT_E_INVALID;
+      jobs.w[li] = lw.qkv_w; jobs.b[li] = lw.qkv_b; jobs.gamma[li] = lw.norm_w; jobs.beta[li] = lw.norm_b;
+      jobs.dst[li] = (float*)ws.w16 + (size_t)li * 4 * D * D;
+    }
+    jobs.count = desc->n_rmsa_layers;
+    if (!desc->weights16_valid) RRT_TRY(launch_ln_fold(jobs, D, st));
   }
   bool parts_done = false;
   for (int li = 0; li < desc->n_rmsa_layers; ++li) {
@@ -498,8 +524,13 @@
                        rmsa_fused_supported(gd.P, D, desc->n_heads, ek) &&
                        crmsa_parts_wanted(*desc, ws, to_dev(g8), rmsa_out != nullptr);
     if (parts && (!w->crmsa.norm_w || !w->crmsa.norm_b || !w->phi)) return RRT_E_INVALID;
-    RRT_TRY(launch_ln_partition(xin, lw.norm_w, lw.norm_b, ws.uo, D, gd, st, merged ? ws.proj_cnt : nullptr,
-                                merged ? gd.rs * gd.rs : 0));
+    const bool ln_fold = merged && ln_fold_images && rmsa_out == nullptr &&
+                         rmsa_fused_lnfold_supported(gd.rs * gd.rs, gd.P, D, desc->n_heads, ek, desc->compute);
+    if (ln_fold)
+      RRT_TRY(hipMemsetAsync(ws.proj_cnt, 0, (size_t)gd.rs * gd.rs * sizeof(int), st));
+    else
+      RRT_TRY(launch_ln_partition(xin, lw.norm_w, lw.norm_b, ws.uo, D, gd, st, merged ? ws.proj_cnt : nullptr,
+                                  merged ? gd.rs * gd.rs : 0));
     if (epeg_variant) {
       if (!lw.pe_w) return RRT_E_INVALID;
       const int nreg = gd.rs * gd.rs;
@@ -557,8 +588,10 @@
         pj.k = desc->crmsa_k;
         parts_done = true;
       }
-      RRT_TRY(launch_rmsa_fused(ws.uo, lw.qkv_w, lw.qkv_b, desc->epeg ? lw.pe_w : nullptr, ws.qkv,
-                                gd.rs * gd.rs, gd.P, D, desc->n_heads, ek, desc->compute, st, nullptr, &pj));
+      pj.ln_fold = ln_fold;
+      RRT_TRY(launch_rmsa_fused(ln_fold ? xin : ws.uo, ln_fold ? (const float*)ws.w16 + (size_t)li * 4 * D * D : lw.qkv_w, lw.qkv_b,
+                                desc->epeg ? lw.pe_w : nullptr, ws.qkv, gd.rs * gd.rs, gd.P, D, desc->n_heads, ek, desc->compute,
+                                st, nullptr, &pj));
       if (gt) { RRT_TRY(hipEventRecord(gt->done, st)); gt->armed = true; }
       if (li == 0) { RRT_MARK(RRT_EV_QKV); RRT_MARK(RRT_EV_ATTN); RRT_MARK(RRT_EV_PROJ); }
       xin = xout;
@@ -996,6 +1029,44 @@
   if (!ln2_gamma || !phi || !part || crmsa_k < 1 || crmsa_k > RRT_MAX_CRMSA_K) return RRT_E_INVALID;
   return fused_proj_stage(u, qkv_w, qkv_b, pe_w, proj_w, proj_b, resid, out, o_scratch, counters, dim, heads, epeg_k, g, 0, 0, 0,
                           ln2_gamma, phi, crmsa_k, part, stream);
+}
+
+int rrt_rmsa_fused_lnfold_supported(int32_t dim, int32_t heads, int32_t epeg_k, const rrt_grid* g) {
+  if (!g || dim <= 0 || heads <= 0) return 0;
+  const GridDev gd = to_dev(*g);
+  return rmsa_fused_lnfold_supported(gd.rs * gd.rs, gd.P, dim, heads, epeg_k, RRT_COMPUTE_F32) && rmsa_fused_supported_rows(gd.Np, dim);
+}
+
+int rrt_rmsa_fused_lnfold_f32(const float* x, const float* ln_w, const float* ln_b, const float* qkv_w, const float* qkv_b,
+                              const float* pe_w, const float* proj_w, const float* proj_b, float* out, float* o_scratch,
+                              int32_t* counters, float* fold, float* qkv_stash, int32_t dim, int32_t heads, int32_t epeg_k,
+                              const rrt_grid* g, void* stream) {
+  if (!x || !ln_w || !ln_b || !qkv_w || !proj_w || !out || !o_scratch || !counters || !fold || !g || dim <= 0 || heads <= 0 ||
+      out == x)
+    return RRT_E_INVALID;
+  if (handover_err_peek(false)) return RRT_E_HANDOVER;
+  const GridDev gd = to_dev(*g);
+  const int ek = pe_w ? epeg_k : 0, R = gd.rs * gd.rs;
+  if (!rmsa_fused_lnfold_supported(R, gd.P, dim, heads, ek, RRT_COMPUTE_F32) || !rmsa_fused_supported_rows(gd.Np, dim))
+    return unsupported("rmsa_fused_lnfold: needs what rmsa_fused_proj needs, regions of <= 176 tokens and a build with the "
+                       "folded form enabled");
+  hipStream_t st = (hipStream_t)stream;
+  hipError_t e = hipMemsetAsync(counters, 0, (size_t)R * sizeof(int32_t), st);
+  if (e != hipSuccess) return (int)e;
+  LnFoldJobs jobs{};
+  jobs.w[0] = qkv_w; jobs.b[0] = qkv_b; jobs.gamma[0] = ln_w; jobs.beta[0] = ln_b; jobs.dst[0] = fold;
+  jobs.count = 1;
+  e = launch_ln_fold(jobs, dim, st);
+  if (e != hipSuccess) return (int)e;
+  FusedProj pj{};
+  pj.Wp = proj_w;
+  pj.bias = proj_b;
+  pj.resid = x;
+  pj.out = out;
+  pj.cnt = counters;
+  pj.g = gd;
+  pj.ln_fold = 1;
+  return (int)launch_rmsa_fused(x, fold, qkv_b, pe_w, o_scratch, R, gd.P, dim, heads, ek, RRT_COMPUTE_F32, st, qkv_stash, &pj);
 }
 
 int rrt_crmsa_combine_parts_f32(const float* x1, const float* part, const float* gamma, const float* beta, const float* phi,
diff --git a/rrt-mil_amd/csrc/cast16.hip b/rrt-mil_amd/csrc/cast16.hip
--- a/rrt-mil_amd/csrc/cast16.hip
+++ b/rrt-mil_amd/csrc/cast16.hip
@@ -172,6 +172,42 @@
   }
 }
 
+__global__ __launch_bounds__(256) void ln_fold_kernel(LnFoldJobs jobs, int D) {
+  const int j = blockIdx.y;
+  const int lane = threadIdx.x & 63;
+  const int r = blockIdx.x * 4 + (threadIdx.x >> 6);
+  if (r >= 3 * D) return;
+  const float* w = jobs.w[j] + (size_t)r * D;
+  const float* gamma = jobs.gamma[j];
+  const float* beta = jobs.beta[j];
+  float* dst = jobs.dst[j];
+  double s = 0.0, t = 0.0;
+  for (int c = lane * 4; c < D; c += 256) {
+    const float4 v = *(const float4*)(w + c), g = *(const float4*)(gamma + c), bt = *(const float4*)(beta + c);
+    const float4 o = make_float4(v.x * g.x, v.y * g.y, v.z * g.z, v.w * g.w);
+    *(float4*)(dst + (size_t)r * D + c) = o;
+    s += ((double)o.x + (double)o.y) + ((double)o.z + (double)o.w);
+    t += ((double)v.x * bt.x + (double)v.y * bt.y) + ((double)v.z * bt.z + (double)v.w * bt.w);
+  }
+#pragma unroll
+  for (int sh = 32; sh >= 1; sh >>= 1) {
+    s += __shfl_xor(s, sh);
+    t += __shfl_xor(t, sh);
+  }
+  if (lane == 0) {
+    float* fold = dst + (size_t)3 * D * D;
+    fold[r] = (float)s;
+    fold[3 * D + r] = (float)((jobs.b[j] ? (double)jobs.b[j][r] : 0.0) + t);
+  }
+}
+
+}
+
+hipError_t launch_ln_fold(const LnFoldJobs& jobs, int D, hipStream_t st) {
+  if (jobs.count <= 0) return hipSuccess;
+  if (D <= 0 || D % 4) return hipErrorInvalidValue;
+  ln_fold_kernel<<<dim3((3 * D + 3) / 4, jobs.count), 256, 0, st>>>(jobs, D);
+  return hipGetLastError();
 }
 
 hipError_t launch_cast_split(const Cast16Jobs& jobs, hipStream_t st) {
diff --git a/rrt-mil_amd/csrc/internal.h b/rrt-mil_amd/csrc/internal.h
--- a/rrt-mil_amd/csrc/internal.h
+++ b/rrt-mil_amd/csrc/internal.h
@@ -116,10 +116,23 @@
   const float* phi;
   int k;
   int n_slabs;
+  int ln_fold;
 };
 int* handover_err_device();
 int handover_err_peek(bool clear);
 bool rmsa_fused_proj_supported(int n_regions, int P, int D, int heads, int epeg_k, int prec);
+bool rmsa_fused_lnfold_enabled();
+bool rmsa_fused_lnfold_supported(int n_regions, int P, int D, int heads, int epeg_k, int prec);
+constexpr size_t ln_fold_floats(size_t D) { return 3 * D * D + 6 * D; }
+struct LnFoldJobs {
+  const float* w[RRT_MAX_RMSA_LAYERS];
+  const float* b[RRT_MAX_RMSA_LAYERS];
+  const float* gamma[RRT_MAX_RMSA_LAYERS];
+  const float* beta[RRT_MAX_RMSA_LAYERS];
+  float* dst[RRT_MAX_RMSA_LAYERS];
+  int count;
+};
+hipError_t launch_ln_fold(const LnFoldJobs& jobs, int D, hipStream_t st);
 hipError_t launch_rmsa_fused(const float* U, const float* Wqkv, const float* bqkv, const float* pe_w,
                              float* O, int n_regions, int P, int D, int heads, int epeg_k, int prec,
                              hipStream_t st, float* stash = nullptr,
diff --git a/rrt-mil_amd/csrc/rmsa_fused.hip b/rrt-mil_amd/csrc/rmsa_fused.hip
--- a/rrt-mil_amd/csrc/rmsa_fused.hip
+++ b/rrt-mil_amd/csrc/rmsa_fused.hip
@@ -348,7 +348,7 @@
   }
 }
 
-template <int MT, int PREC, bool PROJ, int KM = 0>
+template <int MT, int PREC, bool PROJ, int KM = 0, bool LNF = false>
 __global__ __launch_bounds__(512, 1) void rmsa_fused_kernel(const float* __restrict__ U,
                                                             const float* __restrict__ Wqkv,
                                                             const float* __restrict__ bqkv,
@@ -357,6 +357,7 @@
                                                             int D, int heads_rt, int epeg_k, float q_scale,
                                                             float* __restrict__ stash, FusedProj pj) {
   static_assert(!PROJ || PREC == PREC_F32, "the projection phase is fp32 only");
+  static_assert(!LNF || (PROJ && MT <= 11), "the folded LayerNorm rides on the pipelined fp32 loader of the merged launch");
   constexpr int BM = 16 * MT;
   constexpr int STAGE = (BM + BN) * BK;
   constexpr int TILE = BM * HD;
@@ -398,9 +399,20 @@
   if (has_item) {
   float* const taps = (float*)(smem + LDS_MAIN);
   float* const bias_l = taps + 128;
+  [[maybe_unused]] float* const lns_l = bias_l + BN;
+  [[maybe_unused]] float* const b0_l = lns_l + BN;
+  [[maybe_unused]] float2* const stat_l = (float2*)(b0_l + BN);
   if (tid >= 128 && tid < 128 + BN) {
     const int n = tid - 128;
-    bias_l[n] = bqkv ? bqkv[(n >> 6) * D + head * HD + (n & 63)] : 0.f;
+    const int c = (n >> 6) * D + head * HD + (n & 63);
+    if constexpr (LNF) {
+      const float* const fold = Wqkv + (size_t)3 * D * D;
+      lns_l[n] = fold[c];
+      bias_l[n] = fold[3 * D + c];
+      b0_l[n] = bqkv ? bqkv[c] : 0.f;
+    } else {
+      bias_l[n] = bqkv ? bqkv[c] : 0.f;
+    }
   }
   if (tid < 128) {
     const int t = tid - TAP_OFF;
@@ -413,12 +425,27 @@
   if (wave >= 4) {
     const int lw = wave - 4;
     unsigned aoff[LA], boff[LB];
+    [[maybe_unused]] unsigned padm = 0;
+    [[maybe_unused]] int tbase = 0;
+    if constexpr (LNF) {
+      const int ri = fdiv(reg, pj.g.rs, pj.g.inv_rs), rj = reg - ri * pj.g.rs;
+      tbase = ri * pj.g.s * pj.g.H + rj * pj.g.s;
+    }
 #pragma unroll
     for (int qi = 0; qi < LA; ++qi) {
       int S = (qi * 4 + lw) * 64 + lane;
       int row = S >> 3, p = S & 7;
-      int gr = row0 + row;
-      gr = gr < n_rows ? gr : n_rows - 1;
+      int gr;
+      if constexpr (LNF) {
+        const int pi = fdiv(row, pj.g.s, pj.g.inv_s), pjj = row - pi * pj.g.s;
+        const int t = tbase + pi * pj.g.H + pjj;
+        const bool pad = row >= P || t >= pj.g.L;
+        padm |= pad ? 1u << qi : 0u;
+        gr = pad ? pj.g.L - 1 : t;
+      } else {
+        gr = row0 + row;
+        gr = gr < n_rows ? gr : n_rows - 1;
+      }
       aoff[qi] = (unsigned)gr * (unsigned)D * 4u + (unsigned)((p ^ ((row >> 1) & 7)) << 4);
     }
 #pragma unroll
@@ -434,16 +461,55 @@
         if (qi * 4 + lw < NA) dma16s(U + kt * BK, aoff[qi], buf + (qi * 4 + lw) * 1024);
 #pragma unroll
       for (int qi = 0; qi < LB; ++qi) dma16s(Wqkv + kt * BK, boff[qi], buf + BM * BK * 4 + (qi * 4 + lw) * 1024);
+    };
+    [[maybe_unused]] float piv[LA] = {}, sd[LA] = {}, sq[LA] = {};
+    [[maybe_unused]] auto stats = [&](const float* buf, const bool first) {
+      float4 v[LA];
+#pragma unroll
+      for (int qi = 0; qi < LA; ++qi)
+        if (qi * 4 + lw < NA) v[qi] = *(const float4*)(buf + ((qi * 4 + lw) * 64 + lane) * 4);
+#pragma unroll
+      for (int qi = 0; qi < LA; ++qi)
+        if (qi * 4 + lw < NA) {
+          if (first) { piv[qi] = v[qi].x; sd[qi] = 0.f; sq[qi] = 0.f; }
+          const float a = v[qi].x - piv[qi], b = v[qi].y - piv[qi], c = v[qi].z - piv[qi], d = v[qi].w - piv[qi];
+          sd[qi] += (a + b) + (c + d);
+          sq[qi] += (a * a + b * b) + (c * c + d * d);
+        }
     };
     stage(0, lds_b);
     if constexpr (PIPE) {
       wait_vm0();
       __syncthreads();
       if (nk > 1) stage(1, lds_b + STAGE * 4);
+      if constexpr (LNF) stats(lds, true);
       for (int kt = 0; kt < nk; ++kt) {
         wait_vm0();
         __syncthreads();
         if (kt + 2 < nk) stage(kt + 2, lds_b + (kt & 1) * STAGE * 4);
+        if constexpr (LNF) if (kt + 1 < nk) stats(lds + ((kt + 1) & 1) * STAGE, false);
+      }
+      if constexpr (LNF) {
+        const float n = (float)(4 * nk);
+#pragma unroll
+        for (int qi = 0; qi < LA; ++qi)
+          if (qi * 4 + lw < NA) {
+            float cnt = n;
+            float mean = piv[qi] + sd[qi] / n;
+            float m2 = fmaxf(sq[qi] - sd[qi] * sd[qi] / n, 0.f);
+#pragma unroll
+            for (int sh = 1; sh < 8; sh <<= 1) {
+              const float om = __shfl_xor(mean, sh), o2 = __shfl_xor(m2, sh);
+              const float dl = om - mean;
+              m2 = (m2 + o2) + dl * dl * (0.5f * cnt);
+              mean = 0.5f * (mean + om);
+              cnt *= 2.0f;
+            }
+            const float rstd = 1.0f / sqrtf(m2 * (1.0f / (float)D) + LN_EPS);
+            const bool pad = (padm >> qi) & 1u;
+            if ((lane & 7) == 0)
+              stat_l[((qi * 4 + lw) * 64 + lane) >> 3] = pad ? make_float2(0.f, 0.f) : make_float2(rstd, -rstd * mean);
+          }
       }
     } else {
       for (int kt = 0; kt < nk; ++kt) {
@@ -597,12 +663,27 @@
       const float4 b = *(const float4*)(bias_l + n);
       const float sc = c == 0 ? q_scale : 1.0f;
       float* dstm = c == 0 ? Qs : (c == 1 ? Ks : Vs);
+      [[maybe_unused]] float4 s4, b0;
+      if constexpr (LNF) {
+        s4 = *(const float4*)(lns_l + n);
+        b0 = *(const float4*)(b0_l + n);
+      }
 #pragma unroll
       for (int i = 0; i < MT; ++i) {
         const int m = i * 16 + lr;
         const int slot = (d >> 2) ^ (m & 15);
-        float4 v = make_float4((acc[i][j][0] + b.x) * sc, (acc[i][j][1] + b.y) * sc,
-                               (acc[i][j][2] + b.z) * sc, (acc[i][j][3] + b.w) * sc);
+        float4 v;
+        if constexpr (LNF) {
+          const float2 st = stat_l[m];
+          const bool pad = st.x == 0.f;
+          v = make_float4((pad ? b0.x : st.x * acc[i][j][0] + (st.y * s4.x + b.x)) * sc,
+                          (pad ? b0.y : st.x * acc[i][j][1] + (st.y * s4.y + b.y)) * sc,
+                          (pad ? b0.z : st.x * acc[i][j][2] + (st.y * s4.z + b.z)) * sc,
+                          (pad ? b0.w : st.x * acc[i][j][3] + (st.y * s4.w + b.w)) * sc);
+        } else {
+          v = make_float4((acc[i][j][0] + b.x) * sc, (acc[i][j][1] + b.y) * sc,
+                          (acc[i][j][2] + b.z) * sc, (acc[i][j][3] + b.w) * sc);
+        }
         *(float4*)(dstm + m * HD + (slot << 2)) = v;
       }
     }
@@ -1021,8 +1102,11 @@
                      const FusedProj* proj) {
   constexpr int BM = 16 * MT;
   constexpr size_t STG = (size_t)2 * (BM + BN) * BK * 4, QKV = (size_t)3 * BM * HD * 4;
-  constexpr size_t LDS = (STG > QKV ? STG : QKV) + (MT == 9 ? 1280 + MT * 32 * 4 + 16 * HD * 4 : 2064);
+  constexpr size_t XTRA = MT == 9 ? 1280 + MT * 32 * 4 + 16 * HD * 4 : 2064;
+  constexpr size_t LDS = (STG > QKV ? STG : QKV) + XTRA;
   static_assert(LDS <= 160 * 1024, "LDS budget");
+  constexpr size_t XTRA_LNF = 1280 + 2 * BN * 4 + BM * 8;
+  [[maybe_unused]] constexpr size_t LDS_LNF = (STG > QKV ? STG : QKV) + (XTRA > XTRA_LNF ? XTRA : XTRA_LNF);
   const float q_scale = 1.0f / sqrtf((float)HD);
   if constexpr (PREC == PREC_F32) {
     if (proj != nullptr) {
@@ -1035,15 +1119,26 @@
         return hipErrorInvalidValue;
       if (pj.spin_limit <= 0) pj.spin_limit = 1 << 22;
       if (pj.err == nullptr) pj.err = handover_err_device();
-#define RRT_LAUNCH_PROJ(KM_)                                                                                    \
+#define RRT_LAUNCH_PROJ_(KM_, LNF_, LDS_)                                                                       \
   do {                                                                                                           \
-    auto kern = rmsa_fused_kernel<MT, PREC_F32, true, KM_>;                                                      \
+    auto kern = rmsa_fused_kernel<MT, PREC_F32, true, KM_, LNF_>;                                                \
     static OncePerDevice once;                                                                                   \
     if (once.first())                                                                                            \
-      (void)hipFuncSetAttribute((const void*)kern, hipFuncAttributeMaxDynamicSharedMemorySize, (int)LDS);        \
-    kern<<<dim3(pj.n_items + pj.lag), dim3(512), LDS, st>>>(U, Wqkv, bqkv, pe_w, O, n_regions * P, P, D, heads,  \
-                                                            pe_w ? epeg_k : 0, q_scale, nullptr, pj);            \
+      (void)hipFuncSetAttribute((const void*)kern, hipFuncAttributeMaxDynamicSharedMemorySize, (int)(LDS_));     \
+    kern<<<dim3(pj.n_items + pj.lag), dim3(512), LDS_, st>>>(U, Wqkv, bqkv, pe_w, O, n_regions * P, P, D, heads, \
+                                                             pe_w ? epeg_k : 0, q_scale, stash, pj);             \
   } while (0)
+#define RRT_LAUNCH_PROJ(KM_) RRT_LAUNCH_PROJ_(KM_, false, LDS)
+      if constexpr (MT >= 6 && MT <= 11) {
+        if (pj.ln_fold) {
+          static_assert(LDS_LNF <= 160 * 1024, "LDS budget");
+          if (pj.part != nullptr && pj.k <= 4) RRT_LAUNCH_PROJ_(4, true, LDS_LNF);
+          else if (pj.part != nullptr) RRT_LAUNCH_PROJ_(8, true, LDS_LNF);
+          else RRT_LAUNCH_PROJ_(0, true, LDS_LNF);
+          return hipGetLastError();
+        }
+      }
+      if (pj.ln_fold || stash != nullptr) return hipErrorInvalidValue;
       if constexpr (MT >= 6) {
         if (pj.part != nullptr && pj.k <= 4) RRT_LAUNCH_PROJ(4);
         else if (pj.part != nullptr) RRT_LAUNCH_PROJ(8);
@@ -1053,6 +1148,7 @@
         RRT_LAUNCH_PROJ(0);
       }
 #undef RRT_LAUNCH_PROJ
+#undef RRT_LAUNCH_PROJ_
       return hipGetLastError();
     }
   }
@@ -1118,11 +1214,24 @@
   return D % 4 == 0 && P > 64 && n_items >= 2 * lag && lag >= 8 * heads;
 }
 
+bool rmsa_fused_lnfold_enabled() {
+#ifdef RRT_NO_LN_FOLD
+  return false;
+#else
+  static const bool off = rrt_tune_env("RRT_NO_LN_FOLD") != nullptr;
+  return !off;
+#endif
+}
+bool rmsa_fused_lnfold_supported(int n_regions, int P, int D, int heads, int epeg_k, int prec) {
+  return rmsa_fused_lnfold_enabled() && P <= 176 && rmsa_fused_proj_supported(n_regions, P, D, heads, epeg_k, prec);
+}
+
 hipError_t launch_rmsa_fused(const float* U, const float* Wqkv, const float* bqkv, const float* pe_w,
                              float* O, int n_regions, int P, int D, int heads, int epeg_k, int prec,
                              hipStream_t st, float* stash, const FusedProj* proj) {
-  if (proj != nullptr && (stash != nullptr || !rmsa_fused_proj_supported(n_regions, P, D, heads, epeg_k, prec)))
+  if (proj != nullptr && ((stash != nullptr && !proj->ln_fold) || !rmsa_fused_proj_supported(n_regions, P, D, heads, epeg_k, prec)))
     return hipErrorInvalidValue;
+  if (proj != nullptr && proj->ln_fold && !rmsa_fused_lnfold_supported(n_regions, P, D, heads, epeg_k, prec)) return hipErrorInvalidValue;
   if (proj != nullptr && proj->lag > 0 && (proj->lag < 8 * heads || proj->lag > n_regions * heads)) return hipErrorInvalidValue;
 #define RRT_FUSED(MT_)                                                                              \
   switch (prec) {                                                                                   \
diff --git a/rrt-mil_amd/encoder.py b/rrt-mil_amd/encoder.py
--- a/rrt-mil_amd/encoder.py
+++ b/rrt-mil_amd/encoder.py
@@ -479,9 +479,8 @@
         ctx = torch.cuda.device(dev) if torch.cuda.current_device() != dev.index else _NULL_CTX
         with ctx:
             stream = torch.cuda.current_stream(dev).cuda_stream
-            lowp = mode != _lib.COMPUTE_F32
-            key = (ws.data_ptr(), mode, w.version, stream) if lowp else None
-            desc.weights16_valid = int(lowp and key == d_.get("_w16_key"))
+            key = (ws.data_ptr(), mode, w.version, stream)
+            desc.weights16_valid = int(key == d_.get("_w16_key"))
             desc.solo = int(d_.get("solo", True))
             rc = lib.rrt_encoder_forward_f32(C.byref(desc), C.byref(w), x2d.data_ptr(), y.data_ptr(), n,
                                              ws.data_ptr(), ws.numel(), stream)
diff --git a/rrt-mil_amd/mil.py b/rrt-mil_amd/mil.py
--- a/rrt-mil_amd/mil.py
+++ b/rrt-mil_amd/mil.py
@@ -340,12 +340,11 @@
         with torch.cuda.device(x2d.device):
             stream = torch.cuda.current_stream(x2d.device).cuda_stream
             key = (self._ws.data_ptr(), d.enc.compute, w.enc.version, stream, n)
-            lowp = d.enc.compute != _lib.COMPUTE_F32
-            d.enc.weights16_valid = int(lowp and key == getattr(self, "_w16_key", None))
+            d.enc.weights16_valid = int(key == getattr(self, "_w16_key", None))
             rc = lib.rrt_mil_forward_f32(C.byref(d), C.byref(w), x2d.data_ptr(), logits.data_ptr(),
                                          attn.data_ptr() if return_attn else None, int(bool(no_norm)), None, n,
                                          self._ws.data_ptr(), self._ws.numel(), stream)
-            self._w16_key = key if rc == 0 and lowp else None
+            self._w16_key = key if rc == 0 else None
         _lib.check(rc, "rrt_mil_forward_f32")
         return (logits, attn) if return_attn else logits
 
```

Result: slower. 4933 (-9.0%).
